# CPJKU/beat_this

Hardware: AMD Instinct MI355X
Metric: audio-seconds processed/sec (higher is better)
Workload: dtype f32 activations, f16x3 products (3 x f16 MFMA on hi+lo operand halves, f32 accumulate); main-layer attention P.V: 2 x, probabilities as fp16 hi parts

## Files before the change

### beat_this_amd/csrc/attn2.hip

```cpp
#include <cstdlib>

#include "common.h"
#include "kernels.h"

namespace {

constexpr int KB = 4;
constexpr int BLK_BYTES = 2048;
constexpr int TILE_BYTES = KB * BLK_BYTES;
constexpr int SMEM_BYTES = 2 * 2 * TILE_BYTES + 16;

typedef const __attribute__((address_space(1))) void* gptr_t;
typedef __attribute__((address_space(3))) void* lptr_t;

DEVI int lane_id_fresh() {
  int z;
  asm volatile("s_mov_b32 %0, 0" : "=s"(z));
  return __builtin_amdgcn_mbcnt_hi(~0u, __builtin_amdgcn_mbcnt_lo(~0u, z));
}
DEVI unsigned pk2(float a, float b) {
  const hfx2 t = {(hf)a, (hf)b};
  return __builtin_bit_cast(unsigned, t);
}
DEVI void zero16(f32x16& a) {
// ... 613 lines not shown
    const float scale = okq ? gatev / l_tot[j] : 0.f;
#pragma unroll
    for (int k = 0; k < 2; ++k) {
      const unsigned x0 = pk2(st[j].acc[8 * k] * scale, st[j].acc[8 * k + 1] * scale);
      const unsigned x1 = pk2(st[j].acc[8 * k + 2] * scale, st[j].acc[8 * k + 3] * scale);
      const unsigned y0 = pk2(st[j].acc[8 * k + 4] * scale, st[j].acc[8 * k + 5] * scale);
      const unsigned y1 = pk2(st[j].acc[8 * k + 6] * scale, st[j].acc[8 * k + 7] * scale);
      auto r0 = __builtin_amdgcn_permlane32_swap(x0, y0, false, false);
      auto r1 = __builtin_amdgcn_permlane32_swap(x1, y1, false, false);
      if (okq) *reinterpret_cast<u32x4*>(op + 16 * k) = u32x4{r0[0], r1[0], r0[1], r1[1]};
    }
  }
}
#endif


constexpr int BLKX_BYTES = 2 * BLK_BYTES;
constexpr float P_SHIFT_X = 3.f;

struct QStateX {
  hfx8 q0, q1, q0l, q1l;
  f32x16 acc;
  float l;
  f32x4 l4;
  float m;
  f32x16 negm;
};
struct KFragX { hfx8 k0, k1, k0l, k1l; };
struct VFragX { hfx8 v0, v1, v0l, v1l; };
DEVI KFragX ld_kx(const char* kb, int g, int lr) {
  KFragX f;
  f.k0 = *reinterpret_cast<const hfx8*>(kb + ((2 * g) * 32 + lr) * 16);
  f.k1 = *reinterpret_cast<const hfx8*>(kb + ((2 * g + 1) * 32 + lr) * 16);
  f.k0l = *reinterpret_cast<const hfx8*>(kb + BLK_BYTES + ((2 * g) * 32 + lr) * 16);
  f.k1l = *reinterpret_cast<const hfx8*>(kb + BLK_BYTES + ((2 * g + 1) * 32 + lr) * 16);
  return f;
}
DEVI VFragX ld_vx(const char* vb, int lane) {
  VFragX f;
  f.v0 = *reinterpret_cast<const hfx8*>(vb + lane * 16);
  f.v1 = *reinterpret_cast<const hfx8*>(vb + 1024 + lane * 16);
  f.v0l = *reinterpret_cast<const hfx8*>(vb + BLK_BYTES + lane * 16);
  f.v1l = *reinterpret_cast<const hfx8*>(vb + BLK_BYTES + 1024 + lane * 16);
  return f;
}
DEVI void split8(const f32x16& p, int s, u32x4& whi, u32x4& wlo) {
  unsigned h[4], l[4];
#pragma unroll
  for (int j = 0; j < 4; j += 2)
    split_hl4(p[8 * s + 2 * j], p[8 * s + 2 * j + 1], p[8 * s + 2 * j + 2], p[8 * s + 2 * j + 3], h[j], l[j], h[j + 1], l[j + 1]);
  whi = u32x4{h[0], h[1], h[2], h[3]};
  wlo = u32x4{l[0], l[1], l[2], l[3]};
}
template <bool INIT, int QB>
DEVI void score_x(const KFragX& kf, const QStateX (&st)[QB], f32x16 (&sc)[QB]) {
#pragma unroll
  for (int j = 0; j < QB; ++j) {
    if constexpr (INIT) sc[j] = st[j].negm; else zero16(sc[j]);
    sc[j] = MFMA32_H(kf.k0l, st[j].q0, sc[j]);
  }
#pragma unroll
  for (int j = 0; j < QB; ++j) sc[j] = MFMA32_H(kf.k1l, st[j].q1, sc[j]);
#pragma unroll
  for (int j = 0; j < QB; ++j) sc[j] = MFMA32_H(kf.k0, st[j].q0l, sc[j]);
#pragma unroll
  for (int j = 0; j < QB; ++j) sc[j] = MFMA32_H(kf.k1, st[j].q1l, sc[j]);
#pragma unroll
  for (int j = 0; j < QB; ++j) sc[j] = MFMA32_H(kf.k0, st[j].q0, sc[j]);
#pragma unroll
  for (int j = 0; j < QB; ++j) sc[j] = MFMA32_H(kf.k1, st[j].q1, sc[j]);
}
DEVI unsigned cvt_pk_rn(float a, float b) {
  unsigned w;
  asm("s_nop 0\n\tv_cvt_pk_f16_f32 %0, %1, %2" : "=v"(w) : "v"(a), "v"(b));
  return w;
}
template <bool SAFE, bool MASK, int QB, bool PRESUB = (QB == 1), bool P16 = false>
DEVI void finish_x(f32x16 (&sc)[QB], const VFragX& vf, int g, QStateX (&st)[QB], int key0, int L) {
#pragma unroll
  for (int j = 0; j < QB; ++j) {
    if constexpr (SAFE) {
      if constexpr (MASK) {
#pragma unroll
        for (int r = 0; r < 16; ++r)
          if (key0 + crow(r, g) >= L) sc[j][r] = -1e30f;
      }
      float bm = sc[j][0];
#pragma unroll
      for (int r = 1; r < 16; ++r) bm = fmaxf(bm, sc[j][r]);
      bm = fmaxf(bm, __shfl_xor(bm, 32));
      const float m_new = fmaxf(st[j].m, bm);
      const float alpha = __builtin_amdgcn_exp2f(st[j].m - m_new);
      st[j].m = m_new;
      st[j].l *= alpha;
      if constexpr (P16) st[j].l4 *= alpha;
#pragma unroll
      for (int r = 0; r < 16; ++r) st[j].acc[r] *= alpha;
#pragma unroll
      for (int r = 0; r < 16; ++r) sc[j][r] = __builtin_amdgcn_exp2f(sc[j][r] - m_new);
    } else {
#pragma unroll
      for (int r = 0; r < 16; ++r) sc[j][r] = __builtin_amdgcn_exp2f(PRESUB ? sc[j][r] : sc[j][r] + st[j].negm[0]);
      if constexpr (MASK) {
#pragma unroll
        for (int r = 0; r < 16; ++r)
          if (key0 + crow(r, g) >= L) sc[j][r] = 0.f;
      }
    }
    if constexpr (!P16) {
      const float a = (sc[j][0] + sc[j][1]) + (sc[j][2] + sc[j][3]), b = (sc[j][4] + sc[j][5]) + (sc[j][6] + sc[j][7]);
      const float c = (sc[j][8] + sc[j][9]) + (sc[j][10] + sc[j][11]), d = (sc[j][12] + sc[j][13]) + (sc[j][14] + sc[j][15]);
      st[j].l += (a + b) + (c + d);
    }
  }
  if constexpr (P16) {
    u32x4 w0[QB], w1[QB];
#pragma unroll
    for (int j = 0; j < QB; ++j) {
#pragma unroll
      for (int i = 0; i < 4; ++i) {
        w0[j][i] = cvt_pk_rn(sc[j][2 * i], sc[j][2 * i + 1]);
        w1[j][i] = cvt_pk_rn(sc[j][8 + 2 * i], sc[j][8 + 2 * i + 1]);
      }
      rowsum8(st[j].l4, w0[j]);
      rowsum8(st[j].l4, w1[j]);
    }
#pragma unroll
    for (int j = 0; j < QB; ++j) st[j].acc = MFMA32_H(vf.v0l, __builtin_bit_cast(hfx8, w0[j]), st[j].acc);
#pragma unroll
    for (int j = 0; j < QB; ++j) st[j].acc = MFMA32_H(vf.v1l, __builtin_bit_cast(hfx8, w1[j]), st[j].acc);
#pragma unroll
    for (int j = 0; j < QB; ++j) st[j].acc = MFMA32_H(vf.v0, __builtin_bit_cast(hfx8, w0[j]), st[j].acc);
#pragma unroll
    for (int j = 0; j < QB; ++j) st[j].acc = MFMA32_H(vf.v1, __builtin_bit_cast(hfx8, w1[j]), st[j].acc);
    return;
  }
  u32x4 h0[QB], l0[QB], h1[QB], l1[QB];
#pragma unroll
  for (int j = 0; j < QB; ++j) {
    split8(sc[j], 0, h0[j], l0[j]);
    split8(sc[j], 1, h1[j], l1[j]);
  }
#pragma unroll
  for (int j = 0; j < QB; ++j) st[j].acc = MFMA32_H(vf.v0l, __builtin_bit_cast(hfx8, h0[j]), st[j].acc);
#pragma unroll
  for (int j = 0; j < QB; ++j) st[j].acc = MFMA32_H(vf.v1l, __builtin_bit_cast(hfx8, h1[j]), st[j].acc);
#pragma unroll
  for (int j = 0; j < QB; ++j) st[j].acc = MFMA32_H(vf.v0, __builtin_bit_cast(hfx8, l0[j]), st[j].acc);
#pragma unroll
  for (int j = 0; j < QB; ++j) st[j].acc = MFMA32_H(vf.v1, __builtin_bit_cast(hfx8, l1[j]), st[j].acc);
#pragma unroll
  for (int j = 0; j < QB; ++j) st[j].acc = MFMA32_H(vf.v0, __builtin_bit_cast(hfx8, h0[j]), st[j].acc);
#pragma unroll
  for (int j = 0; j < QB; ++j) st[j].acc = MFMA32_H(vf.v1, __builtin_bit_cast(hfx8, h1[j]), st[j].acc);
}

template <int KBX>
DEVI void stage_tile_x(rsrc_t rk, rsrc_t rv, int tile, char* smem, int buf, int tid, int wave) {
  constexpr int TILEX_BYTES = KBX * BLKX_BYTES;
  char* kd = smem + buf * 2 * TILEX_BYTES + wave * 1024;
  char* vd = kd + TILEX_BYTES;
  const int so = tile * TILEX_BYTES;
  static_assert(TILEX_BYTES % 4096 == 0, "stage_tile_x copies 4 KB pieces");
#pragma unroll
  for (int i = 0; i < KBX; ++i) __builtin_amdgcn_raw_ptr_buffer_load_lds(rk, (lptr_t)(kd + i * 4096), 16, tid * 16, so + i * 4096, 0, 0);
#pragma unroll
  for (int i = 0; i < KBX; ++i) __builtin_amdgcn_raw_ptr_buffer_load_lds(rv, (lptr_t)(vd + i * 4096), 16, tid * 16, so + i * 4096, 0, 0);
}

template <bool SAFE, int QB, int KBX, bool P16 = false>
DEVI void attn_tiles_x(rsrc_t rk, rsrc_t rv, char* smem, int tid, int wave, int lane, int g, int lr, QStateX (&st)[QB], int L,
                       int nblk, int t0, bool next_staged) {
  constexpr int TILEX_BYTES = KBX * BLKX_BYTES;
  const int ntiles = (nblk + KBX - 1) / KBX;
  const bool partial = (L & 31) != 0;
  for (int t = t0; t < ntiles; ++t) {
    if (t + 1 < ntiles && !(t == t0 && next_staged)) stage_tile_x<KBX>(rk, rv, t + 1, smem, (t + 1) & 1, tid, wave);
    const char* kb = smem + (t & 1) * 2 * TILEX_BYTES;
    const char* vb = kb + TILEX_BYTES;
    const int nb = min(KBX, nblk - t * KBX);
    for (int c = 0; c < nb; ++c) {
      const int blk = t * KBX + c;
      const KFragX kf = ld_kx(kb + c * BLKX_BYTES, g, lr);
      const VFragX vf = ld_vx(vb + c * BLKX_BYTES, lane);
      f32x16 sc[QB];
      score_x<!SAFE && QB == 1, QB>(kf, st, sc);
      if (partial && blk == nblk - 1) finish_x<SAFE, true, QB, (QB == 1), P16>(sc, vf, g, st, blk * 32, L);
      else finish_x<SAFE, false, QB, (QB == 1), P16>(sc, vf, g, st, blk * 32, L);
    }
    __syncthreads();
  }
}

template <int QB>
DEVI void diag_max_x(const char* kseq, const int (&qblk)[QB], int g, int lr, const QStateX (&st)[QB], int L, float (&dmax)[QB]) {
  KFragX kd[QB];
#pragma unroll
  for (int j = 0; j < QB; ++j) kd[j] = ld_kx(kseq + (long)qblk[j] * BLKX_BYTES, g, lr);
  asm volatile("s_waitcnt vmcnt(0)" ::: "memory");
  __builtin_amdgcn_sched_barrier(0);
#pragma unroll
  for (int j = 0; j < QB; ++j) {
    f32x16 sd;
    zero16(sd);
    sd = MFMA32_H(kd[j].k0l, st[j].q0, sd);
    sd = MFMA32_H(kd[j].k1l, st[j].q1, sd);
    sd = MFMA32_H(kd[j].k0, st[j].q0l, sd);
    sd = MFMA32_H(kd[j].k1, st[j].q1l, sd);
    sd = MFMA32_H(kd[j].k0, st[j].q0, sd);
    sd = MFMA32_H(kd[j].k1, st[j].q1, sd);
    float m = -1e30f;
#pragma unroll
    for (int r = 0; r < 16; ++r) m = fmaxf(m, (32 * qblk[j] + crow(r, g) < L) ? sd[r] : -1e30f);
    dmax[j] = m;
  }
}
template <int QB>
DEVI void ref_max_x(const char* smem, int g, int lr, QStateX (&st)[QB], int L, int nblk, const float (&dmax)[QB]) {
  float bm[QB];
#pragma unroll
  for (int j = 0; j < QB; ++j) bm[j] = dmax[j];
  const int nref = min(2, nblk);
  for (int c = 0; c < nref; ++c) {
    const KFragX kf = ld_kx(smem + c * BLKX_BYTES, g, lr);
    f32x16 s0[QB];
    score_x<false, QB>(kf, st, s0);
#pragma unroll
    for (int j = 0; j < QB; ++j)
#pragma unroll
      for (int r = 0; r < 16; ++r) bm[j] = fmaxf(bm[j], (32 * c + crow(r, g) < L) ? s0[j][r] : -1e30f);
  }
#pragma unroll
  for (int j = 0; j < QB; ++j) {
    const float m = ceilf(fmaxf(bm[j], __shfl_xor(bm[j], 32)));
#pragma unroll
    for (int r = 0; r < 16; ++r) st[j].negm[r] = -m - P_SHIFT_X;
  }
}

template <int QB, int KBX, bool P16 = false>
DEVI void attn_fast_x(rsrc_t rk, rsrc_t rv, char* smem, int tid, int wave, int lane, int g, int lr, QStateX (&st)[QB], int L,
                      int nblk, const float (&dmax)[QB]) {
  constexpr int TILEX_BYTES = KBX * BLKX_BYTES;
  static_assert(KBX % 2 == 0, "two score buffers alternate over the blocks of a tile");
  const int ntiles = (nblk + KBX - 1) / KBX;
  const bool partial = (L & 31) != 0;
  int nfull = nblk / KBX;
  if (partial && nfull * KBX == nblk) --nfull;
  stage_tile_x<KBX>(rk, rv, 0, smem, 0, tid, wave);
  __syncthreads();
  if (ntiles > 1) stage_tile_x<KBX>(rk, rv, 1, smem, 1, tid, wave);
#pragma unroll
  for (int j = 0; j < QB; ++j) {
    zero16(st[j].acc);
    st[j].l = 0.f;
    st[j].l4 = f32x4{0.f, 0.f, 0.f, 0.f};
    st[j].m = -1e30f;
  }
  constexpr bool PIPE = QB == 1;
  f32x16 s2[PIPE ? 2 : 1][QB];
  ref_max_x<QB>(smem, g, lr, st, L, nblk, dmax);
  KFragX kf = ld_kx(smem, g, lr);
  if (QB == 1 && nfull > 0) score_x<true, QB>(kf, st, s2[0]);
  else if (QB != 1) score_x<false, QB>(kf, st, s2[0]);
  for (int t = 0; t < nfull; ++t) {
    const char* kb = smem + (t & 1) * 2 * TILEX_BYTES;
    const char* vb = kb + TILEX_BYTES;
    const char* kb_next = smem + ((t + 1) & 1) * 2 * TILEX_BYTES;
#pragma unroll
    for (int c = 0; c < KBX; ++c) {
      const VFragX vf = ld_vx(vb + c * BLKX_BYTES, lane);
      const int cur = PIPE ? (c & 1) : 0, nxt = PIPE ? ((c + 1) & 1) : 0;
      bool have_next = true;
      if (c + 1 < KBX) {
        kf = ld_kx(kb + (c + 1) * BLKX_BYTES, g, lr);
      } else {
        __syncthreads();
        if (t + 2 < ntiles) stage_tile_x<KBX>(rk, rv, t + 2, smem, t & 1, tid, wave);
        have_next = t + 1 < nfull;
        if (have_next) kf = ld_kx(kb_next, g, lr);
      }
      if (PIPE && have_next) score_x<true, QB>(kf, st, s2[nxt]);
      finish_x<false, false, QB, (QB == 1), P16>(s2[cur], vf, g, st, 0, L);
      if (!PIPE && have_next) score_x<false, QB>(kf, st, s2[0]);
    }
  }
// ... 90 lines not shown
  const unsigned seq_bytes = (unsigned)p.nbp * BLKX_BYTES;
  const rsrc_t rk = __builtin_amdgcn_make_buffer_rsrc(const_cast<char*>(kseq), 0, seq_bytes, 0x00020000);
  const rsrc_t rv = __builtin_amdgcn_make_buffer_rsrc(const_cast<char*>(vseq), 0, seq_bytes, 0x00020000);
  float dmax[QB];
  diag_max_x<QB>(kseq, qbi, g, lr, st, L, dmax);
  attn_fast_x<QB, KBX, P16>(rk, rv, smem, tid, wave, lane, g, lr, st, L, nblk, dmax);
  auto lane_sum = [&](int j) { return P16 ? st[j].l4[0] : st[j].l; };
  float l_tot[QB];
  bool bad[QB];
#pragma unroll
  for (int j = 0; j < QB; ++j) {
    l_tot[j] = lane_sum(j) + __shfl_xor(lane_sum(j), 32);
    const bool valid = qb0 + j < nblk && (qb0 + j) * 32 + lr < L;
    bad[j] = valid && !(l_tot[j] < 65504.f);
    const unsigned long long bw = __ballot(bad[j]);
    if (lane == 0 && qb0 + j < nblk) p.fix_mask[(long)sh * p.nbp + qb0 + j] = (int)(unsigned)bw;
  }
#ifdef BT_DEV
  if (p.status && tid == 0) atomicAdd(p.status + 2, 1);
#endif

  float amax = 0.f;
#pragma unroll
  for (int j = 0; j < QB; ++j) {
    const int qi = (qb0 + j) * 32 + lr;
    store_rows_x<OUT>(p, st[j], l_tot[j], qi, qb0 + j < nblk && qi < L && !bad[j], sh, g, amax);
  }
  if (OUT == 0 && p.status && __any(!(amax <= (p.out_f32 == 2 ? HL8_ACT_MAX : 65504.f))) && lane == 0) atomicOr(p.status, 1);
}


#include "attn_x3_loop.inc"

template <int OUT, bool P16>
__global__ __launch_bounds__(256, 2) void attn_frag_x3q2_kernel(const AttnFragP p, int nqt, int sh_total) {
  constexpr int QB = 2, KBX = ATTN_X3Q2_KBX, NBUF = ATTN_X3Q2_NBUF;
  constexpr int TILEX_BYTES = KBX * BLKX_BYTES, BUF_BYTES = 2 * TILEX_BYTES;
  static_assert(KBX == 2 && NBUF == 4 && BUF_BYTES == 16384, "the generated loop is written for four 16 KB ring buffers");
  __shared__ __attribute__((aligned(16))) char smem[NBUF * BUF_BYTES + 16];
  const int bid = blockIdx.x;
  const int idx = bid >> 3;
  const int sh = (idx / nqt) * 8 + (bid & 7);
  const int qt = idx % nqt;
  if (sh >= sh_total) return;
  const int tid = threadIdx.x, lane = tid & 63, wave = __builtin_amdgcn_readfirstlane(tid >> 6);
  const int g = lane >> 5, lr = lane & 31;
  const int L = p.L;
  const int nblk = (L + 31) >> 5;
  const long seq_off = (long)sh * p.nbp * BLKX_BYTES;
  const char* kseq = reinterpret_cast<const char*>(p.k) + seq_off;
  const char* vseq = reinterpret_cast<const char*>(p.v) + seq_off;
  QStateX st[QB];
  const int qb0 = (qt * 4 + wave) * QB;
  auto load_q = [&]() {
    const int ln = lane_id_fresh(), gg = ln >> 5, ll = ln & 31;
#pragma unroll
    for (int j = 0; j < QB; ++j) {
      const int qbc = min(qb0 + j, nblk - 1);
      const char* qblk = reinterpret_cast<const char*>(p.q) + seq_off + (long)qbc * BLKX_BYTES;
      st[j].q0 = *reinterpret_cast<const hfx8*>(qblk + ((2 * gg) * 32 + ll) * 16);
      st[j].q1 = *reinterpret_cast<const hfx8*>(qblk + ((2 * gg + 1) * 32 + ll) * 16);
      st[j].q0l = *reinterpret_cast<const hfx8*>(qblk + BLK_BYTES + ((2 * gg) * 32 + ll) * 16);
      st[j].q1l = *reinterpret_cast<const hfx8*>(qblk + BLK_BYTES + ((2 * gg + 1) * 32 + ll) * 16);
    }
    asm volatile("s_waitcnt vmcnt(0)" ::: "memory");
    __builtin_amdgcn_sched_barrier(0);
  };
  load_q();
  float dmax[QB];
  {
    const int qbi[QB] = {min(qb0, nblk - 1), min(qb0 + 1, nblk - 1)};
    diag_max_x<QB>(kseq, qbi, g, lr, st, L, dmax);
  }
  const unsigned seq_bytes = (unsigned)p.nbp * BLKX_BYTES;
  const rsrc_t rk = __builtin_amdgcn_make_buffer_rsrc(const_cast<char*>(kseq), 0, seq_bytes, 0x00020000);
  const rsrc_t rv = __builtin_amdgcn_make_buffer_rsrc(const_cast<char*>(vseq), 0, seq_bytes, 0x00020000);
  const int ntiles = (nblk + KBX - 1) / KBX;
  const bool partial = (L & 31) != 0;
  int nfull = nblk / KBX;
  if (partial && nfull * KBX == nblk) --nfull;
  nfull = __builtin_amdgcn_readfirstlane(nfull);
  auto stage_ring = [&](int tile) {
    char* kd = smem + (tile & (NBUF - 1)) * BUF_BYTES + wave * 1024;
    const int so = tile * TILEX_BYTES;
#pragma unroll
    for (int i = 0; i < KBX; ++i) __builtin_amdgcn_raw_ptr_buffer_load_lds(rk, (lptr_t)(kd + i * 4096), 16, tid * 16, so + i * 4096, 0, 0);
#pragma unroll
    for (int i = 0; i < KBX; ++i) __builtin_amdgcn_raw_ptr_buffer_load_lds(rv, (lptr_t)(kd + TILEX_BYTES + i * 4096), 16, tid * 16, so + i * 4096, 0, 0);
  };
  auto fast_pass = [&]() {
#pragma unroll
    for (int j = 0; j < QB; ++j) {
      zero16(st[j].acc);
      st[j].l = 0.f;
      st[j].l4 = f32x4{0.f, 0.f, 0.f, 0.f};
    }
    const float nm0 = st[0].negm[0], nm1 = st[1].negm[0];
    if (nfull > 0) {
    const unsigned long long ka = (unsigned long long)kseq, va = (unsigned long long)vseq;
    const u32x4 dk = {(unsigned)__builtin_amdgcn_readfirstlane((int)(unsigned)ka), (unsigned)__builtin_amdgcn_readfirstlane((int)(unsigned)((ka >> 32) & 0xffffu)),
                      (unsigned)__builtin_amdgcn_readfirstlane((int)seq_bytes), 0x00020000u};
    const u32x4 dv = {(unsigned)__builtin_amdgcn_readfirstlane((int)(unsigned)va), (unsigned)__builtin_amdgcn_readfirstlane((int)(unsigned)((va >> 32) & 0xffffu)),
                      (unsigned)__builtin_amdgcn_readfirstlane((int)seq_bytes), 0x00020000u};
    const int ln = lane_id_fresh();
    const unsigned lds0 = (unsigned)(unsigned long long)(lptr_t)smem;
    const unsigned klane = lds0 + ((2 * (ln >> 5)) * 32 + (ln & 31)) * 16, vlane = lds0 + ln * 16, dmaoff = (wave * 64 + ln) * 16;
    const unsigned m0base = (unsigned)__builtin_amdgcn_readfirstlane((int)(lds0 + wave * 1024));
    const float m1 = -1.0f;
    int t = 0, soff = 3 * TILEX_BYTES;
    if constexpr (P16)
      asm volatile(ATTN_X3Q2P_ASM
                   : "+v"(st[0].acc), "+v"(st[1].acc), "+v"(st[0].l4), "+v"(st[1].l4), "+s"(t), "+s"(soff)
                   : "v"(st[0].q0), "v"(st[0].q1), "v"(st[0].q0l), "v"(st[0].q1l), "v"(st[1].q0), "v"(st[1].q1), "v"(st[1].q0l), "v"(st[1].q1l),
                     "v"(st[0].negm), "v"(st[1].negm), "v"(klane), "v"(vlane), "v"(dmaoff), "s"(dk), "s"(dv), "s"(m0base), "s"(m1), "s"(nfull)
                   : ATTN_X3Q2P_CLOBBERS);
    else
      asm volatile(ATTN_X3Q2_ASM
                   : "+v"(st[0].acc), "+v"(st[1].acc), "+v"(st[0].l), "+v"(st[1].l), "+s"(t), "+s"(soff)
                   : "v"(st[0].q0), "v"(st[0].q1), "v"(st[0].q0l), "v"(st[0].q1l), "v"(st[1].q0), "v"(st[1].q1), "v"(st[1].q0l), "v"(st[1].q1l),
                     "v"(st[0].negm), "v"(st[1].negm), "v"(klane), "v"(vlane), "v"(dmaoff), "s"(dk), "s"(dv), "s"(m0base), "s"(m1), "s"(nfull)
                   : ATTN_X3Q2_CLOBBERS);
    }
    asm volatile("s_waitcnt vmcnt(0)" ::: "memory");
    __syncthreads();
    if (nfull < ntiles) {
      load_q();
#pragma unroll
      for (int r = 0; r < 16; ++r) {
        st[0].negm[r] = nm0;
        st[1].negm[r] = nm1;
      }
      const int lane2 = lane_id_fresh(), g2 = lane2 >> 5, lr2 = lane2 & 31;
      const char* kb = smem + (nfull & (NBUF - 1)) * BUF_BYTES;
      const char* vb = kb + TILEX_BYTES;
      const int nb = nblk - nfull * KBX;
      for (int c = 0; c < nb; ++c) {
        const int blk = nfull * KBX + c;
        const KFragX kf = ld_kx(kb + c * BLKX_BYTES, g2, lr2);
        const VFragX vf = ld_vx(vb + c * BLKX_BYTES, lane2);
        f32x16 sc[QB];
        score_x<true, QB>(kf, st, sc);
        if (partial && blk == nblk - 1) finish_x<false, true, QB, true, P16>(sc, vf, g2, st, blk * 32, L);
        else finish_x<false, false, QB, true, P16>(sc, vf, g2, st, blk * 32, L);
      }
      __syncthreads();
    }
  };
  stage_ring(0);
  stage_ring(1);
  stage_ring(2);
  asm volatile("s_waitcnt vmcnt(8)" ::: "memory");
  __syncthreads();
  ref_max_x<QB>(smem, g, lr, st, L, nblk, dmax);
  fast_pass();
  auto lane_sum = [&](int j) { return P16 ? st[j].l4[0] : st[j].l; };
  const int laneE = lane_id_fresh(), gE = laneE >> 5, lrE = laneE & 31;
  float l_tot[QB];
  bool bad[QB];
#pragma unroll
  for (int j = 0; j < QB; ++j) {
    l_tot[j] = lane_sum(j) + __shfl_xor(lane_sum(j), 32);
    const bool valid = qb0 + j < nblk && (qb0 + j) * 32 + lrE < L;
    bad[j] = valid && !(l_tot[j] < 65504.f);
    const unsigned long long bw = __ballot(bad[j]);
    if (laneE == 0 && qb0 + j < nblk) p.fix_mask[(long)sh * p.nbp + qb0 + j] = (int)(unsigned)bw;
  }
#ifdef BT_DEV
  if (p.status && tid == 0) atomicAdd(p.status + 2, 1);
#endif

  const int seq = sh / p.heads, head = sh - seq * p.heads;
  float amax = 0.f;
#pragma unroll
  for (int j = 0; j < QB; ++j) {
    const int qi = (qb0 + j) * 32 + lrE;
    const bool okq = qb0 + j < nblk && qi < L && !bad[j];
    const float gatev = okq ? p.gates[(long)sh * p.nbp * 32 + qi] : 0.f;
    const long orow = okq ? (long)(seq / p.o_div) * p.o_outer + (long)(seq % p.o_div) * p.o_inner + (long)qi * p.o_tok : 0;
    const float scale = okq ? gatev / l_tot[j] : 0.f;
    if constexpr (OUT == 1) {
      float* op = reinterpret_cast<float*>(p.out) + orow * p.inner + head * 32 + 4 * gE;
      if (okq) {
#pragma unroll
        for (int a = 0; a < 4; ++a)
          *reinterpret_cast<f32x4*>(op + 8 * a) = f32x4{st[j].acc[4 * a] * scale, st[j].acc[4 * a + 1] * scale,
                                                         st[j].acc[4 * a + 2] * scale, st[j].acc[4 * a + 3] * scale};
      }
    } else {
      hf* op = reinterpret_cast<hf*>(p.out) + orow * 2 * p.inner + head * 64 + 8 * gE;
#pragma unroll
      for (int k = 0; k < 2; ++k) {
        unsigned xh[2], xl[2], yh[2], yl[2];
#pragma unroll
        for (int i = 0; i < 2; ++i) {
          const float a0 = st[j].acc[8 * k + 2 * i] * scale, a1 = st[j].acc[8 * k + 2 * i + 1] * scale;
          const float b0 = st[j].acc[8 * k + 4 + 2 * i] * scale, b1 = st[j].acc[8 * k + 4 + 2 * i + 1] * scale;
          split_hl4(a0, a1, b0, b1, xh[i], xl[i], yh[i], yl[i]);
          amax = fmaxf(amax, fmaxf(fmaxf(fabsf(a0), fabsf(a1)), fmaxf(fabsf(b0), fabsf(b1))));
        }
        auto h0 = __builtin_amdgcn_permlane32_swap(xh[0], yh[0], false, false);
        auto h1 = __builtin_amdgcn_permlane32_swap(xh[1], yh[1], false, false);
        if (p.out_f32 == 2) {
          const float s0 = st[j].acc[8 * k] * scale, s1 = st[j].acc[8 * k + 1] * scale, s2 = st[j].acc[8 * k + 2] * scale, s3 = st[j].acc[8 * k + 3] * scale;
          const float t0 = st[j].acc[8 * k + 4] * scale, t1 = st[j].acc[8 * k + 5] * scale, t2 = st[j].acc[8 * k + 6] * scale, t3 = st[j].acc[8 * k + 7] * scale;
          auto b8 = __builtin_amdgcn_permlane32_swap(pk4_f8(s0, s1, s2, s3), pk4_f8(t0, t1, t2, t3), false, false);
          auto c8 = __builtin_amdgcn_permlane32_swap(lo4_f8(s0, s1, s2, s3, xh[0], xh[1]), lo4_f8(t0, t1, t2, t3, yh[0], yh[1]), false, false);
          if (okq) {
            *reinterpret_cast<u32x4*>(op + 16 * k) = u32x4{h0[0], h1[0], h0[1], h1[1]};
            char* gb = reinterpret_cast<char*>(op) - 16 * gE;
            *reinterpret_cast<u32x2*>(gb + 64 + 16 * k + 8 * gE) = u32x2{b8[0], b8[1]};
            *reinterpret_cast<u32x2*>(gb + 96 + 16 * k + 8 * gE) = u32x2{c8[0], c8[1]};
          }
        } else {
        auto l0 = __builtin_amdgcn_permlane32_swap(xl[0], yl[0], false, false);
        auto l1 = __builtin_amdgcn_permlane32_swap(xl[1], yl[1], false, false);
        if (okq) {
          *reinterpret_cast<u32x4*>(op + 16 * k) = u32x4{h0[0], h1[0], h0[1], h1[1]};
          *reinterpret_cast<u32x4*>(op + 32 + 16 * k) = u32x4{l0[0], l1[0], l0[1], l1[1]};
        }
        }
      }
    }
  }
  if (OUT == 0 && p.status && __any(!(amax <= (p.out_f32 == 2 ? HL8_ACT_MAX : 65504.f))) && laneE == 0) atomicOr(p.status, 1);
}


// ... 241 lines not shown
```

### beat_this_amd/csrc/attn_x3_loop.inc

```
#ifndef BT_X3Q2_ABL
#define BT_X3Q2_ABL 0
#endif
#if BT_X3Q2_ABL == 0
#define ATTN_X3Q2_ASM \
  "s_nop 4\n\t" \
  "s_and_b32 s88, %4, 3\n\t" \
  "s_lshl_b32 s88, s88, 14\n\t" \
  "v_add_u32_e32 v121, s88, %16\n\t" \
  "ds_read_b128 v[176:179], v121 offset:0\n\t" \
  "ds_read_b128 v[180:183], v121 offset:512\n\t" \
  "ds_read_b128 v[184:187], v121 offset:2048\n\t" \
  "ds_read_b128 v[188:191], v121 offset:2560\n\t" \
  "v_add_u32_e32 v122, s88, %17\n\t" \
  "ds_read_b128 v[144:147], v122 offset:8192\n\t" \
  "ds_read_b128 v[148:151], v122 offset:9216\n\t" \
  "ds_read_b128 v[152:155], v122 offset:10240\n\t" \
  "ds_read_b128 v[156:159], v122 offset:11264\n\t" \
  "ds_read_b128 v[128:131], v122 offset:8192\n\t" \
  "ds_read_b128 v[132:135], v122 offset:9216\n\t" \
  "ds_read_b128 v[136:139], v122 offset:10240\n\t" \
  "ds_read_b128 v[140:143], v122 offset:11264\n\t" \
  "v_mov_b32_e32 v200, 0\n\t" \
  "v_mov_b32_e32 v192, 0\n\t" \
  "v_mov_b32_e32 v201, 0\n\t" \
// ... 2656 lines not shown
  "ds_read_b128 v[148:151], v124 offset:9216\n\t" \
  "v_exp_f32_e32 v232, v232\n\t" \
  "v_exp_f32_e32 v233, v233\n\t" \
  "v_exp_f32_e32 v234, v234\n\t" \
  "v_exp_f32_e32 v235, v235\n\t" \
  "ds_read_b128 v[152:155], v124 offset:10240\n\t" \
  "v_mfma_f32_32x32x16_f16 %0, v[140:143], v[220:223], %0\n\t" \
  "v_exp_f32_e32 v236, v236\n\t" \
  "v_exp_f32_e32 v237, v237\n\t" \
  "v_exp_f32_e32 v238, v238\n\t" \
  "v_exp_f32_e32 v239, v239\n\t" \
  "ds_read_b128 v[156:159], v124 offset:11264\n\t" \
  "v_mfma_f32_4x4x4_16b_f16 %2, v[126:127], v[218:219], %2\n\t" \
  "v_mfma_f32_32x32x16_f16 v[240:255], v[176:179], %8, v[240:255]\n\t" \
  "v_mfma_f32_32x32x16_f16 v[240:255], v[180:183], %9, v[240:255]\n\t" \
  "v_cvt_pk_f16_f32 v200, v224, v225\n\t" \
  "v_cvt_pk_f16_f32 v201, v226, v227\n\t" \
  "v_cvt_pk_f16_f32 v202, v228, v229\n\t" \
  "v_cvt_pk_f16_f32 v203, v230, v231\n\t" \
  "v_mfma_f32_32x32x16_f16 %0, v[128:131], v[216:219], %0\n\t" \
  "v_cvt_pk_f16_f32 v204, v232, v233\n\t" \
  "v_cvt_pk_f16_f32 v205, v234, v235\n\t" \
  "v_mfma_f32_4x4x4_16b_f16 %2, v[126:127], v[220:221], %2\n\t" \
  "v_mfma_f32_32x32x16_f16 v[240:255], v[176:179], %6, v[240:255]\n\t" \
  "v_mfma_f32_32x32x16_f16 v[240:255], v[180:183], %7, v[240:255]\n\t" \
  "v_cvt_pk_f16_f32 v206, v236, v237\n\t" \
  "v_cvt_pk_f16_f32 v207, v238, v239\n\t" \
  "v_mfma_f32_32x32x16_f16 %0, v[132:135], v[220:223], %0\n\t" \
  "v_mfma_f32_4x4x4_16b_f16 %2, v[126:127], v[222:223], %2\n\t" \
  "s_add_u32 %5, %5, 8192\n\t" \
  "s_add_u32 %4, %4, 1\n\t" \
  "s_cmp_lt_i32 %4, %23\n\t" \
  "s_cbranch_scc1 Lloop%=\n\t" \
  "v_mfma_f32_32x32x16_f16 %1, v[136:139], v[200:203], %1\n\t" \
  "v_mfma_f32_4x4x4_16b_f16 %3, v[126:127], v[200:201], %3\n\t" \
  "s_nop 7\n\t" \
  "s_nop 3\n\t" \
  "v_mfma_f32_32x32x16_f16 %1, v[140:143], v[204:207], %1\n\t" \
  "v_mfma_f32_4x4x4_16b_f16 %3, v[126:127], v[202:203], %3\n\t" \
  "s_nop 7\n\t" \
  "s_nop 3\n\t" \
  "v_mfma_f32_32x32x16_f16 %1, v[128:131], v[200:203], %1\n\t" \
  "v_mfma_f32_4x4x4_16b_f16 %3, v[126:127], v[204:205], %3\n\t" \
  "s_nop 7\n\t" \
  "s_nop 3\n\t" \
  "v_mfma_f32_32x32x16_f16 %1, v[132:135], v[204:207], %1\n\t" \
  "v_mfma_f32_4x4x4_16b_f16 %3, v[126:127], v[206:207], %3\n\t" \
  "s_nop 7\n\t" \
  "s_nop 3\n\t" \
  "s_waitcnt lgkmcnt(0)\n\t" \
  "s_nop 7\n\t" \
  "s_nop 7\n\t" \
  ""
#define ATTN_X3Q2_CLOBBERS "v116", "v117", "v118", "v119", "v120", "v121", "v122", "v123", "v124", "v128", "v129", "v130", "v131", "v132", "v133", "v134", "v135", "v136", "v137", "v138", "v139", "v140", "v141", "v142", "v143", "v144", "v145", "v146", "v147", "v148", "v149", "v150", "v151", "v152", "v153", "v154", "v155", "v156", "v157", "v158", "v159", "v160", "v161", "v162", "v163", "v164", "v165", "v166", "v167", "v168", "v169", "v170", "v171", "v172", "v173", "v174", "v175", "v176", "v177", "v178", "v179", "v180", "v181", "v182", "v183", "v184", "v185", "v186", "v187", "v188", "v189", "v190", "v191", "v192", "v193", "v194", "v195", "v196", "v197", "v198", "v199", "v200", "v201", "v202", "v203", "v204", "v205", "v206", "v207", "v208", "v209", "v210", "v211", "v212", "v213", "v214", "v215", "v216", "v217", "v218", "v219", "v220", "v221", "v222", "v223", "v224", "v225", "v226", "v227", "v228", "v229", "v230", "v231", "v232", "v233", "v234", "v235", "v236", "v237", "v238", "v239", "v240", "v241", "v242", "v243", "v244", "v245", "v246", "v247", "v248", "v249", "v250", "v251", "v252", "v253", "v254", "v255", "s88", "s89", "s90", "s91", "s92", "s93", "s94", "s95", "scc", "memory"
#define ATTN_X3Q2P_CLOBBERS "v121", "v122", "v123", "v124", "v126", "v127", "v128", "v129", "v130", "v131", "v132", "v133", "v134", "v135", "v136", "v137", "v138", "v139", "v140", "v141", "v142", "v143", "v144", "v145", "v146", "v147", "v148", "v149", "v150", "v151", "v152", "v153", "v154", "v155", "v156", "v157", "v158", "v159", "v160", "v161", "v162", "v163", "v164", "v165", "v166", "v167", "v168", "v169", "v170", "v171", "v172", "v173", "v174", "v175", "v176", "v177", "v178", "v179", "v180", "v181", "v182", "v183", "v184", "v185", "v186", "v187", "v188", "v189", "v190", "v191", "v200", "v201", "v202", "v203", "v204", "v205", "v206", "v207", "v216", "v217", "v218", "v219", "v220", "v221", "v222", "v223", "v224", "v225", "v226", "v227", "v228", "v229", "v230", "v231", "v232", "v233", "v234", "v235", "v236", "v237", "v238", "v239", "v240", "v241", "v242", "v243", "v244", "v245", "v246", "v247", "v248", "v249", "v250", "v251", "v252", "v253", "v254", "v255", "s88", "s89", "s90", "s91", "s92", "s93", "s94", "s95", "scc", "memory"
#define ATTN_X3Q2_KBX 2
#define ATTN_X3Q2_NBUF 4
```

### beat_this_amd/csrc/engine.hip

```cpp
#include <algorithm>
#include <cmath>
#include <cstddef>
#include <cstdio>
#include <cstring>
#include <mutex>
#include <string>
#include <vector>

#include "../../include/beat_this_amd.h"
#include "common.h"
#include "kernels.h"


static thread_local std::string g_err;
static int bt_set_error(int code, const std::string& msg) {
  g_err = msg;
  return code;
}
int bt_set_error_external(int code, const char* msg) { return bt_set_error(code, msg); }

namespace prof {
struct Rec { int cat; hipEvent_t a, b; };
struct State { bool on = false; std::vector<Rec> recs; };
struct Scope {
// ... 111 lines not shown
  g.W = x3 ? d.conv_w_x3[blk] : d.conv_w[blk][BT_PREC_HALF];
  g.epi = G3_RESID; g.no_resid = 1; g.gelu = 1; g.bias = d.conv_b[blk]; g.ldx = 2 * C;
  g.conv_C2 = 2 * C; g.conv_T = T; g.conv_F = F / 2; g.x3 = x3; g.status = ws.status;
  g.x = out_half ? nullptr : out; g.xb = out_half ? (void*)out : nullptr;
  return g;
}

GemmP linear_params(const bt_model_desc& d, int wp, const float* in, float* out, void* xb, float* ssq_out, int B, int T) {
  GemmP g;
  memset(&g, 0, sizeof g);
  g.A = in; g.lda = 1024; g.W = d.lin_w[wp]; g.M = B * T; g.N = d.transformer_dim; g.K = 1024;
  g.epi = GEMM_EPI_STORE; g.flags = GEMM_F_A_F32 | GEMM_F_BIAS | GEMM_F_OUT_F32;
  g.bias = d.lin_b; g.out = out; g.ldo = d.transformer_dim; g.xb = xb; g.ssq_out = ssq_out;
  return g;
}

Gemm3P linear3_params(const bt_model_desc& d, const Workspace& ws, int B, int T, bool x3, bool out_f8) {
  const int D = d.transformer_dim;
  Gemm3P g;
  memset(&g, 0, sizeof g);
  g.A = front_x(ws, 3); g.lda = 1024; g.M = B * T; g.K = 1024; g.W = x3 ? d.lin_w_x3 : d.lin_w[BT_PREC_HALF]; g.N = D;
  g.epi = G3_RESID; g.no_resid = 1; g.bias = d.lin_b; g.x = ws.xm; g.ldx = D; g.xb = ws.xmb; g.ssq_out = ws.ssq[0];
  g.x3 = x3 ? 1 | (out_f8 ? G3_X3_OUT_F8 : 0) : 0; g.status = ws.status;
  return g;
}

HeadP head_params(const bt_model_desc& d, const float* x, const float* w, int prenorm, float* beat, float* downbeat, int M,
                  int* status) {
  HeadP p;
  p.x = x; p.w = w; p.b0 = d.head_b[0]; p.b1 = d.head_b[1];
  p.beat = beat; p.downbeat = downbeat; p.M = M; p.D = d.transformer_dim; p.sum_head = d.sum_head; p.prenorm = prenorm;
  p.status = status;
  return p;
}

template <class P>
void attn_rows(P& a, int B, int T, int F) {
  a.n_seq = B * F; a.L = T; a.o_div = F; a.o_outer = (long)T * F; a.o_inner = F > 1 ? 1 : 0; a.o_tok = F;
}

struct PairRoute {
  bool ff_fused;
  bool outff;
  bool split;
  bool time_frag;
};

struct FragLayer {
  bool qkv8;
  bool out8;
  bool ff8;
  bool next8;
  bool tail;
};

enum { LAYERS_GENERIC, LAYERS_FRAG_HALF, LAYERS_FRAG_X3 };

struct Route {
  bool x3;
  int fp;
  int gp, wp;
  int x3_attn, x3_attn_front;
  bool half_shadow;
  int layers;
  struct Block { PairRoute freq, time; bool conv3; } blk[3];
  bool lin3, lin_f8;
  struct Layer { PairRoute pair; FragLayer frag; } layer[BT_MAX_LAYERS];
};

Route plan_route(const bt_engine& e, int B, int T, int prec, int first, const Workspace& ws) {
  const bt_model_desc& d = e.d;
  const int D = d.transformer_dim;
  Route r;
  r.x3 = prec == BT_PREC_F32X3;
  r.fp = r.x3 ? BT_PREC_F32 : prec;
  r.gp = prec;
  r.wp = r.x3 ? BT_PREC_HALF : prec;
  r.x3_attn = r.x3 ? 4 | ((e.x3_attn_p16 == 1 || e.x3_attn_p16 == 2) ? BT_X3_P16 : 0) : 0;
  r.x3_attn_front = r.x3 ? 4 | (e.x3_attn_p16 >= 2 ? BT_X3_P16 : 0) : 0;
  auto pair = [&](const bt_pair_weights& w) {
    PairRoute p;
    p.ff_fused = w.dim <= 128 && w.w_ff_frag[r.fp];
    p.outff = p.ff_fused && w.w_outff_frag[r.fp] && w.w_attnff_frag[r.fp];
    p.split = r.x3 && w.w_outff_frag_x3 && w.w_attnff_frag_x3;
    p.time_frag = r.x3 ? p.outff && p.split && w.w_qkv_frag_x3 : p.ff_fused && r.fp == BT_PREC_HALF && w.w_qkv_frag;
    return p;
  };

  r.half_shadow = prec == BT_PREC_HALF && D >= 128 && D % 64 == 0;
  const long wide = (long)B * T * d.ff_mult * D;
  bool frag_x3 = r.x3 && D >= 128 && D % 128 == 0 && wide * 4 < 0x7fffffffL;
  for (int l = 0; frag_x3 && l < d.n_layers; ++l)
    frag_x3 = d.layers[l].w_qkvg_x3 && d.layers[l].w_out_x3 && d.layers[l].w_ff1_x3 && d.layers[l].w_ff2_x3;
  const bool frag_half = r.half_shadow && D % 128 == 0 && wide * 2 < 0x7fffffffL;
  r.layers = frag_x3 ? LAYERS_FRAG_X3 : frag_half ? LAYERS_FRAG_HALF : LAYERS_GENERIC;

  const bool lin3_fits = (frag_half || (frag_x3 && d.lin_w_x3)) && gemm3_supported(linear3_params(d, ws, B, T, frag_x3, false));
  for (int blk = 0; blk < 3; ++blk) {
    Route::Block& rb = r.blk[blk];
    rb.freq = pair(d.front[blk][0]);
    rb.time = pair(d.front[blk][1]);
    const Gemm3P cg = conv3_params(d, ws, blk, B, T, frag_x3, blk == 2 && lin3_fits);
    rb.conv3 = d.partial_transformers && rb.time.outff && (frag_x3 ? rb.time.split : frag_half) && cg.N >= 128 && cg.W &&
               gemm3_supported(cg);
  }
  r.lin3 = lin3_fits && (!frag_x3 || r.blk[2].conv3);
  r.lin_f8 = r.lin3 && frag_x3 && e.x3_gemm_fp8 >= 2 && d.n_layers > 0 && d.layers[0].w_qkvg_f8;

  for (int l = 0; l < d.n_layers; ++l) {
    const bt_pair_weights& w = d.layers[l];
    FragLayer& f = r.layer[l].frag;
    r.layer[l].pair = pair(w);
    f.qkv8 = l == 0 ? first == 0 && r.lin_f8 : r.layer[l - 1].frag.next8;
    f.out8 = frag_x3 && e.x3_gemm_fp8 >= 2 && w.w_out_f8;
    f.ff8 = frag_x3 && e.x3_gemm_fp8 >= 1 && w.w_ff1_f8 && w.w_ff2_f8;
    f.next8 = frag_x3 && e.x3_gemm_fp8 >= 2 && l + 1 < d.n_layers && d.layers[l + 1].w_qkvg_f8 && w.w_ff2_f8;
    f.tail = frag_half && w.w_tail_frag && layer_tail_supported(D, d.ff_mult * D);
  }
  return r;
}

#define CHECK_RC(what)                                                         \
  if (_rc != 0) {                                                              \
    char buf[160];                                                             \
    snprintf(buf, sizeof buf, "%s failed (code %d: %s)", what, _rc,            \
             _rc > 0 ? hipGetErrorString((hipError_t)_rc) : "bad arguments");  \
    return bt_set_error(_rc > 0 ? BT_ERR_HIP : BT_ERR_ARG, buf);               \
  }
#define LAUNCH(expr, what) \
  do { int _rc = (expr); CHECK_RC(what) } while (0)
#define LAUNCH_CAT(cat, st, expr, what) \
  do { int _rc; { prof::Scope _ps(pf, cat, st); _rc = (expr); } CHECK_RC(what) } while (0)


int check_rows(long M) {
  return M > 0x7fffffffL ? bt_set_error(BT_ERR_ARG, "batch too large for one forward call") : BT_OK;
}

int out_proj(prof::State* pf, const bt_pair_weights& pw, const Route& r, float* x, void* xs, const Workspace& ws, long M,
             hipStream_t s) {
  const int C = pw.dim;
  GemmP g;
  memset(&g, 0, sizeof g);
  g.A = ws.ao; g.lda = C; g.W = pw.w_out[r.wp]; g.M = (int)M; g.N = C; g.K = C;
  g.epi = GEMM_EPI_RESID; g.flags = 0; g.x = x; g.ldx = C; g.xb = xs;
  LAUNCH_CAT(CAT_OUT, s, launch_gemm(g, r.gp, s), "out-proj gemm");
  return BT_OK;
}

int qkv_attn(prof::State* pf, const bt_pair_weights& pw, const Route& r, const float* rope, float* x, void* xs,
             const Workspace& ws, int B, int T, int F, hipStream_t s) {
  const int C = pw.dim, H = pw.heads;
  GemmP g;
  memset(&g, 0, sizeof g);
  g.A = xs ? xs : (const void*)x; g.lda = C; g.W = pw.w_qkvg[r.wp]; g.M = B * T * F; g.N = 3 * C + H; g.K = C;
  g.epi = GEMM_EPI_QKV; g.flags = GEMM_F_RMS | (xs ? 0 : GEMM_F_A_F32) | (F > 1 ? GEMM_F_ROWMAP : 0);
  g.bias = pw.b_gates; g.out = ws.qkv; g.ldo = 3 * C; g.gates = ws.gates; g.inner = C; g.heads = H;
  g.rope = rope; g.map_T = T; g.map_F = F; g.pdiv = F; g.pmod = T;
  LAUNCH_CAT(CAT_QKV, s, launch_gemm(g, r.gp, s), "qkv gemm");
  AttnP a;
  memset(&a, 0, sizeof a);
  a.qkv = ws.qkv; a.ld = 3 * C; a.gates = ws.gates; a.out = ws.ao; a.heads = H; a.inner = C;
  attn_rows(a, B, T, F);
  LAUNCH_CAT(CAT_ATTN_FLASH, s, launch_attn_flash(a, r.gp, s), F > 1 ? "time attention" : "attention");
  return BT_OK;
}

int ff_half(prof::State* pf, const bt_pair_weights& pw, const PairRoute& pr, const Route& r, float* x, void* xs,
            const Workspace& ws, long M, int ff_mult, hipStream_t s) {
  const int C = pw.dim, HID = ff_mult * C;
  if (pr.ff_fused) {
    FusedFFP ff;
    ff.x = x; ff.M = M; ff.C = C; ff.wfrag = pw.w_ff_frag[r.fp]; ff.b1 = pw.b_ff1; ff.b2 = pw.b_ff2; ff.xb = xs;
    LAUNCH_CAT(CAT_FF_FUSED, s, launch_ff_fused(ff, r.fp, s), "fused feed-forward");
    return BT_OK;
  }
  GemmP g;
  memset(&g, 0, sizeof g);
  g.A = xs ? xs : (const void*)x; g.lda = C; g.W = pw.w_ff1[r.wp]; g.M = (int)M; g.N = HID; g.K = C;
  g.epi = GEMM_EPI_STORE; g.flags = GEMM_F_RMS | (xs ? 0 : GEMM_F_A_F32) | GEMM_F_BIAS | GEMM_F_GELU;
  g.bias = pw.b_ff1; g.out = ws.hid; g.ldo = HID;
  LAUNCH_CAT(CAT_FF1, s, launch_gemm(g, r.gp, s), "ff1 gemm");
  memset(&g, 0, sizeof g);
  g.A = ws.hid; g.lda = HID; g.W = pw.w_ff2[r.wp]; g.M = (int)M; g.N = C; g.K = HID;
  g.epi = GEMM_EPI_RESID; g.flags = GEMM_F_BIAS; g.bias = pw.b_ff2; g.x = x; g.ldx = C; g.xb = xs;
  LAUNCH_CAT(CAT_FF2, s, launch_gemm(g, r.gp, s), "ff2 gemm");
  return BT_OK;
}

int generic_layer(prof::State* pf, const bt_pair_weights& pw, const PairRoute& pr, const Route& r, const float* rope, float* x,
                  void* xs, const Workspace& ws, int B, int T, int ff_mult, bool attn, bool ff, hipStream_t s) {
  const long M = (long)B * T;
  if (int rc = check_rows(M)) return rc;
  if (attn) {
    if (int rc = qkv_attn(pf, pw, r, rope, x, xs, ws, B, T, 1, s)) return rc;
    if (int rc = out_proj(pf, pw, r, x, xs, ws, M, s)) return rc;
  }
  return ff ? ff_half(pf, pw, pr, r, x, xs, ws, M, ff_mult, s) : BT_OK;
}

int freq_half(prof::State* pf, const bt_pair_weights& pw, const PairRoute& pr, const Route& r, const float* rope, float* x,
              int B, int T, int F, hipStream_t s) {
  const long M = (long)B * T * F;
  if (int rc = check_rows(M)) return rc;
  if (!pr.outff) return bt_set_error(BT_ERR_ARG, "frequency-direction half needs bt_pair_weights.w_attnff_frag");
  FusedAttnFFP f;
  f.x = x; f.M = M; f.C = pw.dim; f.b_gates = pw.b_gates; f.rope = rope;
  f.wfrag = pr.split ? pw.w_attnff_frag_x3 : pw.w_attnff_frag[r.fp]; f.b1 = pw.b_ff1; f.b2 = pw.b_ff2;
  LAUNCH_CAT(CAT_ATTN_FREQ_FUSED, s, launch_attnff_fused(f, pr.split ? BT_PREC_F32X3 : r.fp, s),
             "fused frequency attention + feed-forward");
  return BT_OK;
}

int time_half(prof::State* pf, const bt_pair_weights& pw, const PairRoute& pr, const Route& r, const float* rope, float* x,
              const Workspace& ws, int B, int T, int F, void* shadow, hipStream_t s) {
  const long M = (long)B * T * F;
  if (int rc = check_rows(M)) return rc;
  if (pr.time_frag) {
    QkvFrontP qp;
    memset(&qp, 0, sizeof qp);
    qp.x = x; qp.B = B; qp.T = T; qp.F = F; qp.C = pw.dim; qp.wfrag = r.x3 ? pw.w_qkv_frag_x3 : pw.w_qkv_frag;
    qp.b_gates = pw.b_gates; qp.rope = rope;
    qp.q = ws.qf; qp.k = ws.kf; qp.v = ws.vf; qp.gates = ws.gates_h; qp.nbp = ws.nbp;
    qp.x3 = r.x3; qp.status = ws.status;
    LAUNCH_CAT(CAT_QKV, s, launch_qkv_front(qp, s), "frontend qkv projection");
    AttnFragP a;
    memset(&a, 0, sizeof a);
    a.q = ws.qf; a.k = ws.kf; a.v = ws.vf; a.gates = ws.gates_h; a.out = ws.ao; a.heads = pw.heads; a.inner = pw.dim;
    a.nbp = ws.nbp; attn_rows(a, B, T, F);
    a.x3 = r.x3_attn_front; a.out_f32 = 1; a.status = ws.status; a.fix_mask = ws.fix_mask;
    LAUNCH_CAT(CAT_ATTN_FLASH, s, launch_attn_frag(a, s), "time attention");
  } else if (int rc = qkv_attn(pf, pw, r, rope, x, nullptr, ws, B, T, F, s)) {
    return rc;
  }
  if (pr.outff) {
    FusedOutFFP f;
    f.x = x; f.M = M; f.C = pw.dim; f.ao = ws.ao; f.wfrag = pr.split ? pw.w_outff_frag_x3 : pw.w_outff_frag[r.fp];
    f.b1 = pw.b_ff1; f.b2 = pw.b_ff2; f.xb = shadow; f.abl = 0;
    LAUNCH_CAT(CAT_FF_FUSED, s, launch_outff_fused(f, pr.split ? BT_PREC_F32X3 : r.fp, s), "fused out-projection + feed-forward");
    return BT_OK;
  }
  if (int rc = out_proj(pf, pw, r, x, nullptr, ws, M, s)) return rc;
  return ff_half(pf, pw, pr, r, x, nullptr, ws, M, 4, s);
}

int frag_layer(prof::State* pf, const bt_pair_weights& pw, const FragLayer& f, const Route& r, const float* rope,
               const Workspace& ws, int B, int T, int ff_mult, hipStream_t s) {
  const int D = pw.dim, H = pw.heads, HID = ff_mult * D;
  const int M = B * T;
  const int parts = D / 64;
  int* status = r.x3 ? ws.status : nullptr;
  auto w = [&](const void* const* half, const void* hl32, const void* hl8, bool f8) { return !r.x3 ? half[BT_PREC_HALF] : f8 ? hl8 : hl32; };
  Gemm3P g;
  memset(&g, 0, sizeof g);
  g.A = ws.xmb; g.lda = D; g.M = M; g.K = D; g.W = w(pw.w_qkvg, pw.w_qkvg_x3, pw.w_qkvg_f8, f.qkv8); g.N = 3 * D + H; g.epi = G3_QKV;
  g.ssq_in = ws.ssq[0]; g.ssq_parts = parts; g.x3 = r.x3 | (f.qkv8 ? G3_X3_F8 : 0); g.status = status;
  g.n_seq = B; g.L = T; g.nblk = (T + 31) / 32; g.nbp = ws.nbp; g.heads = H; g.inner = D; g.rope = rope;
  g.qf = ws.qf; g.kf = ws.kf; g.vf = ws.vf; g.gates = ws.gates_h; g.b_gates = pw.b_gates;
  LAUNCH_CAT(CAT_QKV, s, launch_gemm3(g, s), r.x3 ? "qkv gemm (hi + lo)" : "qkv gemm");
  AttnFragP a;
  memset(&a, 0, sizeof a);
  a.q = ws.qf; a.k = ws.kf; a.v = ws.vf; a.gates = ws.gates_h; a.out = ws.ao; a.heads = H; a.inner = D; a.nbp = ws.nbp;
  attn_rows(a, B, T, 1);
  a.x3 = r.x3_attn; a.out_f32 = f.out8 ? 2 : 0; a.status = status; a.fix_mask = ws.fix_mask;
  LAUNCH_CAT(CAT_ATTN_FLASH, s, launch_attn_frag(a, s), r.x3 ? "attention (hi + lo)" : "attention");
  if (f.tail) {
    LayerTailP t;
    t.x = ws.xm; t.M = M; t.C = D; t.hidden = HID; t.ao = ws.ao; t.wfrag = pw.w_tail_frag; t.b1 = pw.b_ff1; t.b2 = pw.b_ff2;
    t.xb = ws.xmb; t.ssq_out = ws.ssq[0];
    LAUNCH_CAT(CAT_LAYER_TAIL, s, launch_layer_tail(t, s), "layer tail (out-projection + feed-forward)");
    return BT_OK;
  }
  memset(&g, 0, sizeof g);
  g.A = ws.ao; g.lda = D; g.M = M; g.K = D; g.W = w(pw.w_out, pw.w_out_x3, pw.w_out_f8, f.out8); g.N = D; g.epi = G3_RESID;
  g.x3 = r.x3 | (f.out8 ? G3_X3_F8 : 0) | (f.ff8 ? G3_X3_OUT_F8 : 0); g.status = status;
  g.x = ws.xm; g.ldx = D; g.xb = ws.xmb; g.ssq_out = ws.ssq[1];
  LAUNCH_CAT(CAT_OUT, s, launch_gemm3(g, s), r.x3 ? "out-proj gemm (hi + lo)" : "out-proj gemm");
  memset(&g, 0, sizeof g);
  g.A = ws.xmb; g.lda = D; g.M = M; g.K = D; g.W = w(pw.w_ff1, pw.w_ff1_x3, pw.w_ff1_f8, f.ff8); g.N = HID; g.epi = G3_FF1;
  g.x3 = r.x3 | (f.ff8 ? G3_X3_F8 | G3_X3_OUT_F8 : 0); g.status = status;
  g.bias = pw.b_ff1; g.ssq_in = ws.ssq[1]; g.ssq_parts = parts; g.out = ws.hid; g.ldo = HID;
  LAUNCH_CAT(CAT_FF1, s, launch_gemm3(g, s), r.x3 ? "ff1 gemm (hi + lo)" : "ff1 gemm");
  memset(&g, 0, sizeof g);
  g.A = ws.hid; g.lda = HID; g.M = M; g.K = HID; g.W = w(pw.w_ff2, pw.w_ff2_x3, pw.w_ff2_f8, f.ff8); g.N = D; g.epi = G3_RESID;
  g.x3 = r.x3 | (f.ff8 ? G3_X3_F8 : 0) | (f.next8 ? G3_X3_OUT_F8 : 0); g.status = status;
  g.bias = pw.b_ff2; g.x = ws.xm; g.ldx = D; g.xb = ws.xmb; g.ssq_out = ws.ssq[0];
  LAUNCH_CAT(CAT_FF2, s, launch_gemm3(g, s), r.x3 ? "ff2 gemm (hi + lo)" : "ff2 gemm");
  return BT_OK;
}

int frontend(prof::State* pf, const bt_model_desc& d, const Route& r, const float* spect, const Workspace& ws, int B, int T,
             hipStream_t s) {
  const StemP sp = stem_params(d, spect, front_x(ws, 0), B, T);
  LAUNCH_CAT(CAT_STEM, s, launch_stem(sp, s), "stem");
  for (int blk = 0; blk < 3; ++blk) {
    const Route::Block& rb = r.blk[blk];
    float* x = front_x(ws, blk);
    if (d.partial_transformers) {
      if (int rc = freq_half(pf, d.front[blk][0], rb.freq, r, d.rope, x, B, T, 32 >> blk, s)) return rc;
      if (int rc = time_half(pf, d.front[blk][1], rb.time, r, d.rope, x, ws, B, T, 32 >> blk, rb.conv3 ? ws.hid : nullptr, s))
        return rc;
    }
    if (rb.conv3) {
      const Gemm3P g = conv3_params(d, ws, blk, B, T, r.layers == LAYERS_FRAG_X3, blk == 2 && r.lin3);
      LAUNCH_CAT(CAT_CONV, s, launch_gemm3(g, s), "frontend conv gemm");
    } else {
      const GemmP g = conv_params(d, blk, r.wp, x, front_x(ws, blk + 1), B, T, !(blk == 2 && r.lin3));
      LAUNCH_CAT(CAT_CONV, s, launch_gemm(g, r.gp, s), "frontend conv gemm");
    }
  }
  if (r.lin3) {
    const Gemm3P g = linear3_params(d, ws, B, T, r.layers == LAYERS_FRAG_X3, r.lin_f8);
    LAUNCH_CAT(CAT_LINEAR, s, launch_gemm3(g, s), "frontend linear gemm");
    return BT_OK;
  }
  const GemmP g = linear_params(d, r.wp, front_x(ws, 3), ws.xm, r.half_shadow ? ws.xmb : nullptr,
                                r.layers == LAYERS_FRAG_HALF ? ws.ssq[0] : nullptr, B, T);
  LAUNCH_CAT(CAT_LINEAR, s, launch_gemm(g, r.gp, s), "frontend linear gemm");
  if (r.layers == LAYERS_FRAG_X3)
    LAUNCH_CAT(CAT_LINEAR, s, launch_shadow_ssq(ws.xm, ws.xmb, ws.ssq[0], (long)B * T, d.transformer_dim, s, 1), "hl32 shadow of the residual stream");
  return BT_OK;
}

}

extern "C" {

const char* bt_last_error(void) { return g_err.c_str(); }
int bt_version(void) { return BT_ABI_VERSION; }
int bt_half_is_bf16(void) { return BT_HALF_IS_BF16; }
void bt_struct_sizes(int32_t* out) {
  out[0] = (int32_t)sizeof(bt_pair_weights); out[1] = (int32_t)sizeof(bt_model_desc);
  out[2] = (int32_t)sizeof(bt_logmel_tables); out[3] = (int32_t)sizeof(bt_gemm_args);
  out[4] = (int32_t)sizeof(bt_attn_args); out[5] = (int32_t)offsetof(bt_model_desc, layers);
  out[6] = (int32_t)offsetof(bt_model_desc, rope);
  out[7] = (int32_t)sizeof(bt_attn_frag_args);
  out[8] = (int32_t)sizeof(bt_gemm3_args);
}

int bt_engine_create(const bt_model_desc* desc, bt_engine** out) {
  if (!desc || !out) return bt_set_error(BT_ERR_ARG, "null argument");
  if (desc->transformer_dim % 32 || desc->transformer_dim < 32 || desc->transformer_dim > 1024 ||
      desc->n_layers < 0 || desc->n_layers > BT_MAX_LAYERS || desc->ff_mult < 1 || desc->ff_mult > 16)
    return bt_set_error(BT_ERR_ARG, "unsupported transformer_dim / n_layers / ff_mult");
  bt_engine* e = new bt_engine;
  e->d = *desc;
  *out = e;
  return BT_OK;
}
static void drop_graphs(bt_engine* e) {
  for (auto& g : e->graphs) (void)hipGraphExecDestroy(g.exec);
  e->graphs.clear();
  e->warm.clear();
// ... 8 lines not shown

int bt_engine_set_option(bt_engine* e, int option, int value) {
  if (!e) return bt_set_error(BT_ERR_ARG, "null argument");
  std::lock_guard<std::mutex> lock(e->mu);
  if (option == BT_OPT_X3_ATTN_P16 && value >= 0 && value <= 3) { if (e->x3_attn_p16 != value) drop_graphs(e); e->x3_attn_p16 = value; return BT_OK; }
  if (option == BT_OPT_X3_GEMM_FP8 && value >= 0 && value <= 2) { if (e->x3_gemm_fp8 != value) drop_graphs(e); e->x3_gemm_fp8 = value; return BT_OK; }
  if (option == BT_OPT_WS_GUARD && value >= 0 && value % 256 == 0) { if (e->ws_guard != value) drop_graphs(e); e->ws_guard = value; return BT_OK; }
  return bt_set_error(BT_ERR_ARG, "unknown engine option / value");
}
int bt_engine_get_option(const bt_engine* e, int option, int* value) {
  if (!e || !value) return bt_set_error(BT_ERR_ARG, "null argument");
  if (option == BT_OPT_X3_ATTN_P16) { *value = e->x3_attn_p16; return BT_OK; }
  if (option == BT_OPT_X3_GEMM_FP8) { *value = e->x3_gemm_fp8; return BT_OK; }
  if (option == BT_OPT_WS_GUARD) { *value = e->ws_guard; return BT_OK; }
  return bt_set_error(BT_ERR_ARG, "unknown engine option");
}

size_t bt_workspace_bytes(const bt_engine* e, int B, int T, int prec) {
  if (!e || B <= 0 || T <= 0) return 0;
  return carve(nullptr, B, T, e->d.transformer_dim, e->d.ff_mult, prec, (size_t)e->ws_guard).total;
}

int bt_workspace_regions(const bt_engine* e, int B, int T, int prec, int64_t* begin_end, int max) {
  if (!e || B <= 0 || T <= 0 || max < 0 || (max > 0 && !begin_end)) return bt_set_error(BT_ERR_ARG, "bad argument to bt_workspace_regions");
  if (prec != BT_PREC_F32 && prec != BT_PREC_HALF && prec != BT_PREC_F32X3) return bt_set_error(BT_ERR_ARG, "unknown precision");
  std::vector<int64_t> r;
  carve(nullptr, B, T, e->d.transformer_dim, e->d.ff_mult, prec, (size_t)e->ws_guard, &r);
  const int n = (int)(r.size() / 2);
  for (int i = 0; i < std::min(n, max); ++i) { begin_end[2 * i] = r[2 * i]; begin_end[2 * i + 1] = r[2 * i + 1]; }
  return n;
}

int bt_forward(bt_engine* e, void* stream, int prec, const float* d_spect, int B, int T, void* d_ws, size_t ws_bytes,
               float* d_beat, float* d_downbeat) {
  return bt_forward_stages(e, stream, prec, 0, 2, d_spect, B, T, d_ws, ws_bytes, nullptr, d_beat, d_downbeat);
}

int bt_forward_stages(bt_engine* e, void* stream, int prec, int first, int last, const float* d_spect, int B, int T, void* d_ws,
                      size_t ws_bytes, float* d_out, float* d_beat, float* d_downbeat) {
  if (!e || !d_spect || !d_ws) return bt_set_error(BT_ERR_ARG, "null argument");
  if (first < 0 || last > 2 || first > last) return bt_set_error(BT_ERR_ARG, "stages: need 0 <= first <= last <= 2");
  if (last == 2 ? (!d_beat || !d_downbeat) : !d_out) return bt_set_error(BT_ERR_ARG, "null output");
  const int max_T = e->d.rope_len > 0 ? e->d.rope_len : 1536;
  if (B <= 0 || T <= 0 || T > max_T)
    return bt_set_error(BT_ERR_ARG, "need B >= 1 and 1 <= T <= " + std::to_string(max_T) + " (bt_model_desc.rope_len: rows of the rotary table)");
  if (prec != BT_PREC_F32 && prec != BT_PREC_HALF && prec != BT_PREC_F32X3)
    return bt_set_error(BT_ERR_ARG, "unknown precision");
  const bt_model_desc& d = e->d;
  prof::State* pf = &e->prof;
  const int D = d.transformer_dim;
  const Workspace ws = carve((char*)d_ws, B, T, D, d.ff_mult, prec, (size_t)e->ws_guard);
  if (ws.total > ws_bytes) return bt_set_error(BT_ERR_WORKSPACE, "workspace too small");
  if (prec == BT_PREC_F32X3 && BT_HALF_IS_BF16) return bt_set_error(BT_ERR_ARG, "BT_PREC_F32X3 needs an IEEE fp16 build");
  const Route r = plan_route(*e, B, T, prec, first, ws);
  hipStream_t s = (hipStream_t)stream;
  if (r.x3) LAUNCH(launch_clear_words(ws.status, 1, s), "clearing the range flag");
  int* status = r.x3 ? ws.status : nullptr;

  const size_t xm_bytes = (size_t)B * T * D * 4;
  if (first == 2) {
    if (!d.head_w_raw) return bt_set_error(BT_ERR_ARG, "stage entry at task_heads needs head_w_raw");
    const HeadP hp = head_params(d, d_spect, d.head_w_raw, 1, d_beat, d_downbeat, B * T, nullptr);
    LAUNCH_CAT(CAT_HEAD, s, launch_head(hp, s), "head");
    return BT_OK;
  }
  if (first == 1) {
    if (hipMemcpyAsync(ws.xm, d_spect, xm_bytes, hipMemcpyDeviceToDevice, s) != hipSuccess)
      return bt_set_error(BT_ERR_HIP, "copy of the stage input");
    if (r.half_shadow)
      LAUNCH_CAT(CAT_LINEAR, s, launch_shadow_ssq(ws.xm, ws.xmb, r.layers == LAYERS_FRAG_HALF ? ws.ssq[0] : nullptr, (long)B * T, D, s), "stage entry");
    if (r.layers == LAYERS_FRAG_X3) LAUNCH_CAT(CAT_LINEAR, s, launch_shadow_ssq(ws.xm, ws.xmb, ws.ssq[0], (long)B * T, D, s, 1), "stage entry");
  }
  if (first == 0)
    if (int rc = frontend(pf, d, r, d_spect, ws, B, T, s)) return rc;
  if (last == 0) {
    if (hipMemcpyAsync(d_out, ws.xm, xm_bytes, hipMemcpyDeviceToDevice, s) != hipSuccess)
      return bt_set_error(BT_ERR_HIP, "copy of the stage output");
    if (r.x3) LAUNCH_CAT(CAT_HEAD, s, launch_finite_rows(ws.xm, (long)B * T, D, ws.status, s), "range check of the stage output");
    return BT_OK;
  }
  for (int l = 0; l < d.n_layers; ++l) {
    const Route::Layer& rl = r.layer[l];
    const int rc = r.layers == LAYERS_GENERIC
                       ? generic_layer(pf, d.layers[l], rl.pair, r, d.rope, ws.xm, r.half_shadow ? ws.xmb : nullptr, ws, B, T,
                                       d.ff_mult, true, true, s)
                       : frag_layer(pf, d.layers[l], rl.frag, r, d.rope, ws, B, T, d.ff_mult, s);
    if (rc) return rc;
  }
  if (last == 1) {
    if (!d.norm_out_g) return bt_set_error(BT_ERR_ARG, "stage exit after transformer_blocks needs norm_out_g");
    LAUNCH_CAT(CAT_HEAD, s, launch_norm_out(ws.xm, d.norm_out_g, d_out, (long)B * T, D, s, status), "final norm");
    return BT_OK;
  }
  const HeadP hp = head_params(d, ws.xm, d.head_w, 0, d_beat, d_downbeat, B * T, status);
  LAUNCH_CAT(CAT_HEAD, s, launch_head(hp, s), "head");
  return BT_OK;
}

int bt_forward_unit(bt_engine* e, void* stream, int prec, int unit, int index, const float* d_in, float* d_out, int B, int T,
                    void* d_ws, size_t ws_bytes) {
  if (!e || !d_in || !d_out || !d_ws) return bt_set_error(BT_ERR_ARG, "null argument");
  const bt_model_desc& d = e->d;
  const int max_T = d.rope_len > 0 ? d.rope_len : 1536;
  if (B <= 0 || T <= 0 || T > max_T) return bt_set_error(BT_ERR_ARG, "need B >= 1 and 1 <= T <= bt_model_desc.rope_len");
  if (prec == BT_PREC_F32X3) prec = BT_PREC_F32;
  if (prec != BT_PREC_F32 && prec != BT_PREC_HALF) return bt_set_error(BT_ERR_ARG, "unknown precision");
  prof::State* pf = &e->prof;
  const int D = d.transformer_dim;
  const Workspace ws = carve((char*)d_ws, B, T, D, d.ff_mult, prec, (size_t)e->ws_guard);
  if (ws.total > ws_bytes) return bt_set_error(BT_ERR_WORKSPACE, "workspace too small");
  const Route r = plan_route(*e, B, T, prec, 0, ws);
  hipStream_t s = (hipStream_t)stream;
  const bool block_unit = unit == BT_UNIT_PARTIAL || unit == BT_UNIT_CONV;
  const bool layer_unit = unit == BT_UNIT_ATTN || unit == BT_UNIT_FF;
  const bool leaf_unit = unit == BT_UNIT_FRONT_ATTN || unit == BT_UNIT_FRONT_FF;
  if (leaf_unit && (index < 0 || index > 5 || !d.partial_transformers)) return bt_set_error(BT_ERR_ARG, "partial-transformer leaf index out of range");
  if (block_unit && (index < 0 || index > 2)) return bt_set_error(BT_ERR_ARG, "frontend block index out of range");
  if (layer_unit && (index < 0 || index >= d.n_layers)) return bt_set_error(BT_ERR_ARG, "layer index out of range");
  auto copy_in = [&](size_t bytes) -> int {
    if (d_in != d_out && hipMemcpyAsync(d_out, d_in, bytes, hipMemcpyDeviceToDevice, s) != hipSuccess)
      return bt_set_error(BT_ERR_HIP, "copy of the unit's input");
    return BT_OK;
  };
  switch (unit) {
    case BT_UNIT_STEM: {
      const StemP sp = stem_params(d, d_in, d_out, B, T);
      LAUNCH_CAT(CAT_STEM, s, launch_stem(sp, s), "stem");
      return BT_OK;
    }
    case BT_UNIT_PARTIAL: {
      if (!d.partial_transformers) return bt_set_error(BT_ERR_ARG, "this model has no partial transformers");
      const Route::Block& rb = r.blk[index];
      if (int rc = copy_in((size_t)B * T * 1024 * 4)) return rc;
      if (int rc = freq_half(pf, d.front[index][0], rb.freq, r, d.rope, d_out, B, T, 32 >> index, s)) return rc;
      return time_half(pf, d.front[index][1], rb.time, r, d.rope, d_out, ws, B, T, 32 >> index, nullptr, s);
    }
    case BT_UNIT_CONV: {
      const GemmP g = conv_params(d, index, r.wp, d_in, d_out, B, T, true);
      LAUNCH_CAT(CAT_CONV, s, launch_gemm(g, r.gp, s), "frontend conv gemm");
      return BT_OK;
    }
    case BT_UNIT_LINEAR: {
      const GemmP g = linear_params(d, r.wp, d_in, d_out, nullptr, nullptr, B, T);
      LAUNCH_CAT(CAT_LINEAR, s, launch_gemm(g, r.gp, s), "frontend linear gemm");
      return BT_OK;
    }
    case BT_UNIT_ATTN:
    case BT_UNIT_FF: {
      if (int rc = copy_in((size_t)B * T * D * 4)) return rc;
      return generic_layer(pf, d.layers[index], r.layer[index].pair, r, d.rope, d_out, nullptr, ws, B, T, d.ff_mult,
                           unit == BT_UNIT_ATTN, unit == BT_UNIT_FF, s);
    }
    case BT_UNIT_FRONT_ATTN:
    case BT_UNIT_FRONT_FF: {
      const bt_pair_weights& pw = d.front[index >> 1][index & 1];
      const Route::Block& rb = r.blk[index >> 1];
      if (int rc = copy_in((size_t)B * T * pw.dim * 4)) return rc;
      return generic_layer(pf, pw, index & 1 ? rb.time : rb.freq, r, d.rope, d_out, nullptr, ws, B, T, 4,
                           unit == BT_UNIT_FRONT_ATTN, unit == BT_UNIT_FRONT_FF, s);
    }
    case BT_UNIT_NORM:
      if (!d.norm_out_g) return bt_set_error(BT_ERR_ARG, "bt_model_desc.norm_out_g is not set");
      LAUNCH_CAT(CAT_HEAD, s, launch_norm_out(d_in, d.norm_out_g, d_out, (long)B * T, D, s), "final norm");
      return BT_OK;
    default:
      return bt_set_error(BT_ERR_ARG, "unknown unit");
  }
}

int bt_split_chunks(void* stream, const float* d_spect, int64_t n_frames, const int32_t* d_starts, int B, int T,
                    float* d_chunks) {
  if (!d_spect || !d_starts || !d_chunks || B <= 0 || T <= 0 || n_frames <= 0)
    return bt_set_error(BT_ERR_ARG, "bad argument to bt_split_chunks");
  LAUNCH(launch_split(d_spect, n_frames, d_starts, nullptr, B, T, d_chunks, (hipStream_t)stream), "split");
  return BT_OK;
}

int bt_split_chunks_batch(void* stream, const float* d_spect, const int32_t* d_chunk_table, int B, int T, float* d_chunks) {
  if (!d_spect || !d_chunk_table || !d_chunks || B <= 0 || T <= 0)
    return bt_set_error(BT_ERR_ARG, "bad argument to bt_split_chunks_batch");
  LAUNCH(launch_split(d_spect, 0, nullptr, d_chunk_table, B, T, d_chunks, (hipStream_t)stream), "split (batch)");
  return BT_OK;
}

int bt_aggregate(void* stream, const float* cb, const float* cd, const int32_t* d_starts, int B, int T, int border,
                 int64_t n_frames, float* d_beat, float* d_downbeat) {
  if (!cb || !cd || !d_starts || !d_beat || !d_downbeat || B <= 0 || T <= 0 || n_frames <= 0 || border < 0)
    return bt_set_error(BT_ERR_ARG, "bad argument to bt_aggregate");
// ... 268 lines not shown
  for (int i = 0; i < n_categories; ++i) { ms_by_category[i] = 0.0; launches_by_category[i] = 0; }
  for (auto& r : e->prof.recs) {
    hipError_t e = hipEventSynchronize(r.b);
    float ms = 0.f;
    if (e == hipSuccess) e = hipEventElapsedTime(&ms, r.a, r.b);
    if (e != hipSuccess) return bt_set_error(BT_ERR_HIP, hipGetErrorString(e));
    ms_by_category[r.cat] += ms;
    launches_by_category[r.cat] += 1;
    (void)hipEventDestroy(r.a); (void)hipEventDestroy(r.b);
  }
  e->prof.recs.clear();
  return BT_OK;
}

int bt_ff_fused(void* stream, int prec, const bt_pair_weights* w, float* d_x, int64_t M) {
  if (!w || !d_x || M <= 0 || w->dim > 128 || !w->w_ff_frag[prec]) return bt_set_error(BT_ERR_ARG, "bad argument to bt_ff_fused");
  FusedFFP ff;
  ff.x = d_x; ff.M = M; ff.C = w->dim; ff.wfrag = w->w_ff_frag[prec]; ff.b1 = w->b_ff1; ff.b2 = w->b_ff2;
  ff.xb = nullptr;
  LAUNCH(launch_ff_fused(ff, prec, (hipStream_t)stream), "fused feed-forward");
  return BT_OK;
}

int bt_gemm(void* stream, int prec, const bt_gemm_args* a) {
  if (!a) return bt_set_error(BT_ERR_ARG, "null argument");
  GemmP g;
  memset(&g, 0, sizeof g);
  g.A = a->A; g.lda = a->lda; g.W = a->W; g.M = a->M; g.N = a->N; g.K = a->K; g.epi = a->epi; g.flags = a->flags;
  g.bias = a->bias; g.out = a->out; g.ldo = a->ldo; g.x = a->x; g.ldx = a->ldx;
  g.conv_C2 = a->conv_C2; g.conv_T = a->conv_T; g.conv_F = a->conv_F;
  g.gates = a->gates; g.inner = a->inner; g.heads = a->heads; g.rope = a->rope;
  g.pdiv = a->pdiv; g.pmod = a->pmod; g.map_T = a->map_T; g.map_F = a->map_F;
  LAUNCH(launch_gemm(g, prec, (hipStream_t)stream), "gemm");
  return BT_OK;
}

int bt_attention(void* stream, int prec, const bt_attn_args* a) {
  if (!a) return bt_set_error(BT_ERR_ARG, "null argument");
  AttnP p;
  memset(&p, 0, sizeof p);
  p.qkv = a->qkv; p.ld = a->ld; p.gates = a->gates; p.out = a->out; p.n_seq = a->n_seq; p.L = a->L;
  p.heads = a->heads; p.inner = a->inner; p.o_div = a->o_div; p.o_outer = a->o_outer; p.o_inner = a->o_inner;
  p.o_tok = a->o_tok;
  LAUNCH(launch_attn_flash(p, prec, (hipStream_t)stream), "attention (flash)");
  return BT_OK;
}

int bt_outff_fused(void* stream, int prec, const bt_pair_weights* w, const void* d_ao, float* d_x, int64_t M, void* d_xb) {
  if (prec != BT_PREC_F32 && prec != BT_PREC_HALF && prec != BT_PREC_F32X3) return bt_set_error(BT_ERR_ARG, "unknown precision");
  const void* wf = !w ? nullptr : prec == BT_PREC_F32X3 ? w->w_outff_frag_x3 : w->w_outff_frag[prec];
  if (!w || !d_ao || !d_x || M <= 0 || w->dim > 128 || !wf) return bt_set_error(BT_ERR_ARG, "bad argument to bt_outff_fused");
  FusedOutFFP f;
  f.x = d_x; f.M = M; f.C = w->dim; f.ao = d_ao; f.wfrag = wf; f.b1 = w->b_ff1; f.b2 = w->b_ff2;
  f.xb = prec == BT_PREC_F32 ? nullptr : d_xb; f.abl = 0;
  LAUNCH(launch_outff_fused(f, prec, (hipStream_t)stream), "fused out-projection + feed-forward");
  return BT_OK;
}

int bt_attnff_fused(void* stream, int prec, const bt_pair_weights* w, const float* d_rope, float* d_x, int64_t M) {
  if (prec != BT_PREC_F32 && prec != BT_PREC_HALF && prec != BT_PREC_F32X3) return bt_set_error(BT_ERR_ARG, "unknown precision");
  const void* wf = !w ? nullptr : prec == BT_PREC_F32X3 ? w->w_attnff_frag_x3 : w->w_attnff_frag[prec];
  if (!w || !d_x || !d_rope || M <= 0 || w->dim > 128 || !wf) return bt_set_error(BT_ERR_ARG, "bad argument to bt_attnff_fused");
  FusedAttnFFP f;
  f.x = d_x; f.M = M; f.C = w->dim; f.b_gates = w->b_gates; f.rope = d_rope; f.wfrag = wf;
  f.b1 = w->b_ff1; f.b2 = w->b_ff2;
  LAUNCH(launch_attnff_fused(f, prec, (hipStream_t)stream), "fused frequency attention + feed-forward");
  return BT_OK;
}

int bt_layer_tail(void* stream, const bt_pair_weights* w, int hidden, const void* d_ao, float* d_x, int64_t M, void* d_xb,
                  float* d_ssq_out) {
  if (!w || !w->w_tail_frag || !d_ao || !d_x || M <= 0 || !layer_tail_supported(w->dim, hidden))
    return bt_set_error(BT_ERR_ARG, "bad argument to bt_layer_tail");
  LayerTailP t;
  t.x = d_x; t.M = M; t.C = w->dim; t.hidden = hidden; t.ao = d_ao; t.wfrag = w->w_tail_frag; t.b1 = w->b_ff1;
  t.b2 = w->b_ff2; t.xb = d_xb; t.ssq_out = d_ssq_out;
  LAUNCH(launch_layer_tail(t, (hipStream_t)stream), "layer tail");
  return BT_OK;
}

int bt_gemm3(void* stream, const bt_gemm3_args* a) {
  if (!a || !a->A || !a->W) return bt_set_error(BT_ERR_ARG, "null argument");
  Gemm3P g;
  memset(&g, 0, sizeof g);
  g.A = a->A; g.lda = a->lda; g.M = a->M; g.K = a->K; g.W = a->W; g.N = a->N; g.epi = a->epi; g.bias = a->bias;
  g.ssq_in = a->ssq_in; g.ssq_parts = a->ssq_parts; g.out = a->out; g.ldo = a->ldo; g.x = a->x; g.ldx = a->ldx;
  g.xb = a->xb; g.ssq_out = a->ssq_out; g.n_seq = a->n_seq; g.L = a->L; g.nblk = (a->L + 31) / 32; g.nbp = a->nbp;
  g.heads = a->heads; g.inner = a->heads * 32; g.rope = a->rope; g.qf = a->qf; g.kf = a->kf; g.vf = a->vf;
  g.gates = a->gates; g.b_gates = a->b_gates;
  g.x3 = a->x3; g.status = a->status;
  g.no_resid = a->no_resid; g.gelu = a->gelu; g.conv_C2 = a->conv_C2; g.conv_T = a->conv_T; g.conv_F = a->conv_F;
  if (!gemm3_supported(g)) return bt_set_error(BT_ERR_ARG, "shape not supported by bt_gemm3");
  LAUNCH(launch_gemm3(g, (hipStream_t)stream), "gemm3");
  return BT_OK;
}

int bt_gemm_mx8(void* stream, const void* d_A, const void* d_SA, const void* d_W, const void* d_SW, float* d_out, int M, int N, int K,
                int64_t ldo) {
  GemmMx8P g;
  g.A = d_A; g.SA = d_SA; g.W = d_W; g.SW = d_SW; g.out = d_out; g.ldo = (long)ldo; g.M = M; g.N = N; g.K = K;
  if (!d_A || !d_SA || !d_W || !d_SW || !d_out || !gemm_mx8_supported(g)) return bt_set_error(BT_ERR_ARG, "bad argument to bt_gemm_mx8");
  LAUNCH(launch_gemm_mx8(g, (hipStream_t)stream), "MX e4m3 gemm");
  return BT_OK;
}

int bt_attn_frag_blocks(int L) { return L > 0 ? attn_frag_blocks(L) : 0; }

// ... 30 lines not shown
```

### beat_this_amd/csrc/fused2.hip

```cpp
#include <cstdlib>
#include <type_traits>

#include "chain.h"
#include "kernels.h"

namespace {


typedef __amdgpu_buffer_rsrc_t rsrc_t;
typedef __attribute__((address_space(3))) void* lptr_t;
DEVI unsigned pk2_hf(float a, float b) {
  const hfx2 t = {(hf)a, (hf)b};
  return __builtin_bit_cast(unsigned, t);
}

#ifdef BT_DEV
__device__ long long* g_f2_dbg = nullptr;
#define F2_DBG g_f2_dbg
#define F2_ABL(p) ((p).abl)
#else
#define F2_DBG ((long long*)nullptr)
#define F2_ABL(p) 0
#endif

template <typename T, int C>
struct WRing {
  static constexpr int KT = C / 32;
  static constexpr int TILE_B = 32 * 32 * (int)sizeof(T);
  static constexpr int STEP_B = 2 * KT * TILE_B;
#ifndef BT_F2_NST_HL128
#define BT_F2_NST_HL128 2
#endif
#ifndef BT_F2_NST_HL64
#define BT_F2_NST_HL64 2
#endif
  static constexpr bool HL = sizeof(T) == 4 && !std::is_same<T, float>::value;
  static constexpr int NST = C == 128 ? (HL ? BT_F2_NST_HL128 : 3) : (HL && C == 64 ? BT_F2_NST_HL64 : 4);
  static constexpr int CH = STEP_B / 4096;
  rsrc_t rs;
  char* lds;
  int tid, wave, total;
  long long t_wait = 0, t_bar = 0;
  bool timing = false;
  DEVI void issue(int s) {
    if (s >= total) return;
    char* dst = lds + (s % NST) * STEP_B + wave * 1024;
#pragma unroll
    for (int i = 0; i < CH; ++i)
      __builtin_amdgcn_raw_ptr_buffer_load_lds(rs, (lptr_t)(dst + i * 4096), 16, tid * 16, s * STEP_B + i * 4096, 0, 0);
  }
  DEVI void prologue() {
#pragma unroll
    for (int s = 0; s < NST - 1; ++s) issue(s);
  }
  DEVI const char* acquire(int s) {
    const int ahead = min(NST - 2, total - 1 - s);
    long long q0 = 0, q1 = 0;
    if (timing) q0 = clock64();
    if (ahead >= 2) asm volatile("s_waitcnt vmcnt(%0) lgkmcnt(0)" ::"n"(2 * CH) : "memory");
    else if (ahead == 1) asm volatile("s_waitcnt vmcnt(%0) lgkmcnt(0)" ::"n"(CH) : "memory");
    else asm volatile("s_waitcnt vmcnt(0) lgkmcnt(0)" ::: "memory");
    if (timing) q1 = clock64();
    __builtin_amdgcn_s_barrier();
    if (timing) { const long long q2 = clock64(); t_wait += q1 - q0; t_bar += q2 - q1; }
    issue(s + NST - 1);
    return lds + (s % NST) * STEP_B;
  }
};

template <typename T, int C>
DEVI void ff_tail(WRing<T, C>& ws, int step0, float (&xn)[C / 32][16], const float* b1s, const float* b2,
                  float* xrow, hf* xbrow, bool ok, int lane, int g) {
  constexpr int KT = C / 32, HB = 4 * C / 32;
  constexpr int TILE_B = WRing<T, C>::TILE_B;
  float ss = 0.f;
#pragma unroll
  for (int kt = 0; kt < KT; ++kt)
#pragma unroll
    for (int r = 0; r < 16; ++r) ss = fmaf(xn[kt][r], xn[kt][r], ss);
  ss += __shfl_xor(ss, 32);
  constexpr float PW = OpScale<T>::PW;
  const float scale = sqrtf((float)C) / fmaxf(sqrtf(ss), 1e-12f) * PW;
  Frag<T> xf[KT];
#pragma unroll
  for (int kt = 0; kt < KT; ++kt) xf[kt] = pack_frag<T>(xn[kt]);
  f32x16 acc2[KT];
#pragma unroll
  for (int mt = 0; mt < KT; ++mt)
#pragma unroll
    for (int r = 0; r < 16; ++r) acc2[mt][r] = xn[mt][r] * (1.f / PW);
#pragma unroll 1
  for (int hb = 0; hb < HB; ++hb) {
    const char* wb = ws.acquire(step0 + hb);
    f32x16 acc1;
    zero16(acc1);
#pragma unroll
    for (int kt = 0; kt < KT; ++kt) mma32(acc1, lds_frag<T>(wb + kt * TILE_B, lane), xf[kt]);
    float h[16];
#pragma unroll
    for (int a = 0; a < 4; ++a) {
      const f32x4 b = *reinterpret_cast<const f32x4*>(b1s + hb * 32 + 8 * a + 4 * g);
#pragma unroll
      for (int j = 0; j < 4; ++j) h[4 * a + j] = gelu_t<T>(fmaf(acc1[4 * a + j], scale, b[j]));
    }
    const Frag<T> hf = pack_frag<T>(h);
#pragma unroll
    for (int mt = 0; mt < KT; ++mt) mma32(acc2[mt], lds_frag<T>(wb + (KT + mt) * TILE_B, lane), hf);
  }
#pragma unroll
  for (int mt = 0; mt < KT; ++mt) {
    f32x4 v[4];
#pragma unroll
    for (int a = 0; a < 4; ++a) {
      const int f0 = mt * 32 + 8 * a + 4 * g;
      const f32x4 b = *reinterpret_cast<const f32x4*>(b2 + f0);
#pragma unroll
      for (int j = 0; j < 4; ++j) v[a][j] = fmaf(acc2[mt][4 * a + j], PW, b[j]);
      if (ok) *reinterpret_cast<f32x4*>(xrow + f0) = v[a];
    }
    if (xbrow) {
      typedef __attribute__((ext_vector_type(4))) unsigned int u32x4;
      if constexpr (std::is_same<T, hl>::value) {
#pragma unroll
        for (int k = 0; k < 2; ++k) {
          unsigned xh[2], xl[2], yh[2], yl[2];
#pragma unroll
          for (int i = 0; i < 2; ++i) {
            split_hl4(v[2 * k][2 * i], v[2 * k][2 * i + 1], v[2 * k + 1][2 * i], v[2 * k + 1][2 * i + 1], xh[i], xl[i], yh[i], yl[i]);
          }
          auto h0 = __builtin_amdgcn_permlane32_swap(xh[0], yh[0], false, false);
          auto h1 = __builtin_amdgcn_permlane32_swap(xh[1], yh[1], false, false);
          auto l0 = __builtin_amdgcn_permlane32_swap(xl[0], yl[0], false, false);
          auto l1 = __builtin_amdgcn_permlane32_swap(xl[1], yl[1], false, false);
          if (ok) {
            *reinterpret_cast<u32x4*>(xbrow + mt * 64 + 16 * k + 8 * g) = u32x4{h0[0], h1[0], h0[1], h1[1]};
            *reinterpret_cast<u32x4*>(xbrow + mt * 64 + 32 + 16 * k + 8 * g) = u32x4{l0[0], l1[0], l0[1], l1[1]};
          }
        }
      } else {
#pragma unroll
      for (int k = 0; k < 2; ++k) {
        const unsigned x0 = pk2_hf(v[2 * k][0], v[2 * k][1]), x1 = pk2_hf(v[2 * k][2], v[2 * k][3]);
        const unsigned y0 = pk2_hf(v[2 * k + 1][0], v[2 * k + 1][1]), y1 = pk2_hf(v[2 * k + 1][2], v[2 * k + 1][3]);
        auto r0 = __builtin_amdgcn_permlane32_swap(x0, y0, false, false);
        auto r1 = __builtin_amdgcn_permlane32_swap(x1, y1, false, false);
        if (ok) *reinterpret_cast<u32x4*>(xbrow + mt * 32 + 16 * k + 8 * g) = u32x4{r0[0], r1[0], r0[1], r1[1]};
      }
      }
    }
  }
}

template <typename T, int C>
__global__ __launch_bounds__(256) void outff_fused_kernel(const FusedOutFFP p) {
  constexpr int KT = C / 32, HB = 4 * C / 32;
  constexpr int TILE_B = WRing<T, C>::TILE_B, STEP_B = WRing<T, C>::STEP_B, NST = WRing<T, C>::NST;
  __shared__ __attribute__((aligned(16))) char wl[NST * STEP_B + 4 * C * 4];
  float* b1s = reinterpret_cast<float*>(wl + NST * STEP_B);
  const int tid = threadIdx.x, lane = tid & 63, wave = __builtin_amdgcn_readfirstlane(tid >> 6);
  const int g = lane >> 5, lr = lane & 31;
  const long tok = ((long)blockIdx.x * 4 + wave) * 32 + lr;
  const bool ok_st = tok < p.M && !(F2_ABL(p) & 2);
  const bool ok = tok < p.M && !(F2_ABL(p) & 1);
  float* xrow = p.x + (tok < p.M ? tok : 0) * C;
  for (int i = tid; i < 4 * C; i += 256) b1s[i] = p.b1[i];

  const T* arow = reinterpret_cast<const T*>(p.ao) + (ok ? tok : 0) * C;
  Frag<T> af[KT];
#pragma unroll
  for (int kt = 0; kt < KT; ++kt) af[kt] = ldg_frag<T>(arow + kt * 32 + 16 * g);
  float xn[KT][16];
#pragma unroll
  for (int mt = 0; mt < KT; ++mt)
#pragma unroll
    for (int a = 0; a < 4; ++a) {
      const f32x4 v = ok ? *reinterpret_cast<const f32x4*>(xrow + mt * 32 + 8 * a + 4 * g) : f32x4{0.f, 0.f, 0.f, 0.f};
#pragma unroll
      for (int j = 0; j < 4; ++j) xn[mt][4 * a + j] = v[j];
    }
  WRing<T, C> ws;
  ws.rs = __builtin_amdgcn_make_buffer_rsrc(const_cast<void*>(p.wfrag), 0, (unsigned)((KT + HB) * STEP_B), 0x00020000);
  ws.lds = wl; ws.tid = tid; ws.wave = wave; ws.total = KT + HB;
  __syncthreads();
  asm volatile("s_waitcnt vmcnt(0)" ::: "memory");
  ws.prologue();
#pragma unroll
  for (int mt = 0; mt < KT; ++mt) {
    const char* wb = ws.acquire(mt);
    f32x16 acc;
    zero16(acc);
#pragma unroll
    for (int kt = 0; kt < KT; ++kt) mma32(acc, lds_frag<T>(wb + kt * TILE_B, lane), af[kt]);
#pragma unroll
    for (int r = 0; r < 16; ++r) xn[mt][r] = fmaf(acc[r], OpScale<T>::PW, xn[mt][r]);
  }
  hf* xbrow = p.xb ? reinterpret_cast<hf*>(p.xb) + tok * C * (std::is_same<T, hl>::value ? 2 : 1) : nullptr;
  ff_tail<T, C>(ws, KT, xn, b1s, p.b2, xrow, xbrow, ok_st, lane, g);
}

template <typename T, int C>
__global__ __launch_bounds__(256) void attnff_fused_kernel(const FusedAttnFFP p) {
  constexpr int KT = C / 32;
  constexpr int H = C / 32;
  constexpr int F = 1024 / C;
  constexpr int HB = 4 * C / 32;
  constexpr int TILE_B = WRing<T, C>::TILE_B, STEP_B = WRing<T, C>::STEP_B, NST = WRing<T, C>::NST;
  __shared__ __attribute__((aligned(16))) char wl[NST * STEP_B + 4 * C * 4];
  float* b1s = reinterpret_cast<float*>(wl + NST * STEP_B);
  const int tid = threadIdx.x, lane = tid & 63, wave = __builtin_amdgcn_readfirstlane(tid >> 6);
  const int g = lane >> 5, lr = lane & 31;
  const long tok = ((long)blockIdx.x * 4 + wave) * 32 + lr;
  const bool ok = tok < p.M;
  float* xrow = p.x + (ok ? tok : 0) * C;
  long long* dbg = F2_DBG;
  const long long t_in = dbg ? clock64() : 0;
  for (int i = tid; i < 4 * C; i += 256) b1s[i] = p.b1[i];

  float ss = 0.f;
  Frag<T> xf[KT];
#pragma unroll
  for (int kt = 0; kt < KT; ++kt) xf[kt] = ldx_frag<T>(xrow + kt * 32 + 16 * g, ok, ss);
  ss += __shfl_xor(ss, 32);
  constexpr float PW = OpScale<T>::PW, PA = OpScale<T>::PA;
  const float scale = sqrtf((float)C) / fmaxf(sqrtf(ss), 1e-12f) * PW;
  float sk[16];
#pragma unroll
  for (int r = 0; r < 16; ++r) sk[r] = __shfl(scale, crow(r, g));
  const int pos = (int)(tok & (F - 1));
  f32x2 cs[8];
#pragma unroll
  for (int a = 0; a < 4; ++a)
#pragma unroll
    for (int b = 0; b < 2; ++b)
      cs[2 * a + b] = *reinterpret_cast<const f32x2*>(p.rope + ((long)pos * 16 + 4 * a + 2 * g + b) * 2);
  float bg[H];
#pragma unroll
  for (int hd = 0; hd < H; ++hd) bg[hd] = p.b_gates[hd];
  WRing<T, C> ws;
  ws.rs = __builtin_amdgcn_make_buffer_rsrc(const_cast<void*>(p.wfrag), 0, (unsigned)((1 + 2 * H + HB) * STEP_B), 0x00020000);
  ws.lds = wl; ws.tid = tid; ws.wave = wave; ws.total = 1 + 2 * H + HB;
  __syncthreads();
  asm volatile("s_waitcnt vmcnt(0)" ::: "memory");
  ws.timing = dbg != nullptr;
  const long long t_ring = dbg ? clock64() : 0;
  ws.prologue();

  float gate[H];
  {
    const char* wb = ws.acquire(0);
    f32x16 ag;
// ... 51 lines not shown
      }
      l += __shfl_xor(l, 32);
    }
    {
      const char* wb = ws.acquire(2 + 2 * hd);
      f32x16 av;
      zero16(av);
#pragma unroll
      for (int kt = 0; kt < KT; ++kt) mma32(av, xf[kt], lds_frag<T>(wb + kt * TILE_B, lane));
      float v[16];
#pragma unroll
      for (int r = 0; r < 16; ++r) v[r] = av[r] * sk[r];
      f32x16 ao;
      zero16(ao);
      mma32(ao, pack_frag<T>(v), pack_frag<T>(pr));
      float gsel = gate[0];
#pragma unroll
      for (int k = 1; k < H; ++k) gsel = hd == k ? gate[k] : gsel;
      const float fin = gsel / l * PA;
      float o[16];
#pragma unroll
      for (int r = 0; r < 16; ++r) o[r] = ao[r] * fin;
      const Frag<T> of = pack_frag<T>(o);
#pragma unroll
      for (int mt = 0; mt < KT; ++mt) mma32(acco[mt], lds_frag<T>(wb + (KT + mt) * TILE_B, lane), of);
    }
  }
  f32x4 xv[KT][4];
#pragma unroll
  for (int mt = 0; mt < KT; ++mt)
#pragma unroll
    for (int a = 0; a < 4; ++a)
      xv[mt][a] = ok ? *reinterpret_cast<const f32x4*>(xrow + mt * 32 + 8 * a + 4 * g) : f32x4{0.f, 0.f, 0.f, 0.f};
  asm volatile("s_waitcnt vmcnt(0)" ::: "memory");
  __builtin_amdgcn_sched_barrier(0);
  float xn[KT][16];
#pragma unroll
  for (int mt = 0; mt < KT; ++mt)
#pragma unroll
    for (int a = 0; a < 4; ++a)
#pragma unroll
      for (int j = 0; j < 4; ++j) xn[mt][4 * a + j] = fmaf(acco[mt][4 * a + j], PW, xv[mt][a][j]);
  const long long t_ff = dbg ? clock64() : 0;
  ff_tail<T, C>(ws, 1 + 2 * H, xn, b1s, p.b2, xrow, nullptr, ok, lane, g);
  if (dbg && lane == 0) {
    long long* d = dbg + ((long)blockIdx.x * 4 + wave) * 6;
    d[0] = t_ring - t_in; d[1] = t_ff - t_ring; d[2] = clock64() - t_ff; d[3] = ws.t_wait; d[4] = ws.t_bar; d[5] = 0;
  }
}

template <typename T>
int launch_outff_t(const FusedOutFFP& p, hipStream_t s) {
  dim3 grid((unsigned)((p.M + 127) / 128)), block(256);
  switch (p.C) {
    case 32: hipLaunchKernelGGL((outff_fused_kernel<T, 32>), grid, block, 0, s, p); break;
    case 64: hipLaunchKernelGGL((outff_fused_kernel<T, 64>), grid, block, 0, s, p); break;
    case 128: hipLaunchKernelGGL((outff_fused_kernel<T, 128>), grid, block, 0, s, p); break;
    default: return -2;
  }
  return (int)hipGetLastError();
}
template <typename T>
int launch_attnff_t(const FusedAttnFFP& p, hipStream_t s) {
  dim3 grid((unsigned)((p.M + 127) / 128)), block(256);
  switch (p.C) {
    case 32: hipLaunchKernelGGL((attnff_fused_kernel<T, 32>), grid, block, 0, s, p); break;
    case 64: hipLaunchKernelGGL((attnff_fused_kernel<T, 64>), grid, block, 0, s, p); break;
    case 128: hipLaunchKernelGGL((attnff_fused_kernel<T, 128>), grid, block, 0, s, p); break;
    default: return -2;
  }
  return (int)hipGetLastError();
}

}

#ifdef BT_DEV
extern "C" int bt_debug_fused2_buffer(void* buf) {
  return (int)hipMemcpyToSymbol(HIP_SYMBOL(g_f2_dbg), &buf, sizeof buf);
}
#endif

int launch_outff_fused(const FusedOutFFP& p0, int prec, hipStream_t s) {
  if (p0.M <= 0) return -2;
  FusedOutFFP p = p0;
  p.abl = 0;
#ifdef BT_DEV
  static const int abl = getenv("BT_F2_ABL") ? atoi(getenv("BT_F2_ABL")) : 0;
  p.abl = abl;
#endif
  if (prec == BT_PREC_F32X3) return BT_HALF_IS_BF16 ? -2 : launch_outff_t<hl>(p, s);
  return prec == BT_PREC_F32 ? launch_outff_t<float>(p, s) : launch_outff_t<hf>(p, s);
}
int launch_attnff_fused(const FusedAttnFFP& p, int prec, hipStream_t s) {
  if (p.M <= 0) return -2;
  if (prec == BT_PREC_F32X3) return BT_HALF_IS_BF16 ? -2 : launch_attnff_t<hl>(p, s);
  return prec == BT_PREC_F32 ? launch_attnff_t<float>(p, s) : launch_attnff_t<hf>(p, s);
}
```

### beat_this_amd/csrc/gemm3.hip

```cpp
#include <cstdlib>

#include "common.h"
#include "kernels.h"

struct G3CfgS { static constexpr int BM = 128, BN = 128, BK = 32, WGM = 2, WGN = 2, NST = 3, OCC = 3; };
struct G3CfgB { static constexpr int BM = 256, BN = 256, BK = 64, WGM = 2, WGN = 4, NST = 2, OCC = 1; };
struct G3CfgT { static constexpr int BM = 192, BN = 256, BK = 64, WGM = 2, WGN = 4, NST = 2, OCC = 1; };
struct G3CfgSX { static constexpr int BM = 128, BN = 128, BK = 64, WGM = 2, WGN = 2, NST = 2, OCC = 2; };
struct G3CfgBX { static constexpr int BM = 256, BN = 256, BK = 64, WGM = 2, WGN = 4, NST = 2, OCC = 1; };
struct G3CfgTX { static constexpr int BM = 192, BN = 256, BK = 64, WGM = 2, WGN = 4, NST = 2, OCC = 1; };
struct G3CfgMX { static constexpr int BM = 256, BN = 128, BK = 32, WGM = 2, WGN = 2, NST = 3, OCC = 2; };
struct G3CfgHX { static constexpr int BM = 64, BN = 128, BK = 64, WGM = 2, WGN = 2, NST = 3, OCC = 2; };

#ifndef X3_NSPLIT
#define X3_NSPLIT 2
#endif

namespace {

typedef G3CfgS CfgS;
typedef G3CfgB CfgB;

constexpr unsigned OOB = 0x80000000u;

// ... 20 lines not shown
#pragma unroll
  for (int k = 0; k < 2; ++k) {
    unsigned x0 = pk2(v[8 * k], v[8 * k + 1]), x1 = pk2(v[8 * k + 2], v[8 * k + 3]);
    unsigned y0 = pk2(v[8 * k + 4], v[8 * k + 5]), y1 = pk2(v[8 * k + 6], v[8 * k + 7]);
    auto r0 = __builtin_amdgcn_permlane32_swap(x0, y0, false, false);
    auto r1 = __builtin_amdgcn_permlane32_swap(x1, y1, false, false);
    piece[k] = u32x4{r0[0], r1[0], r0[1], r1[1]};
  }
}

DEVI void split2(float a, float b, unsigned& whi, unsigned& wlo, float& amax) {
  split_hl(a, b, whi, wlo);
  amax = fmaxf(amax, fmaxf(fabsf(a), fabsf(b)));
}
DEVI void pack_row_hl(const float (&v)[16], u32x4 (&hi)[2], u32x4 (&lo)[2], float& amax) {
#pragma unroll
  for (int k = 0; k < 2; ++k) {
    unsigned xh[2], xl[2], yh[2], yl[2];
    split2(v[8 * k], v[8 * k + 1], xh[0], xl[0], amax);
    split2(v[8 * k + 2], v[8 * k + 3], xh[1], xl[1], amax);
    split2(v[8 * k + 4], v[8 * k + 5], yh[0], yl[0], amax);
    split2(v[8 * k + 6], v[8 * k + 7], yh[1], yl[1], amax);
    auto h0 = __builtin_amdgcn_permlane32_swap(xh[0], yh[0], false, false);
    auto h1 = __builtin_amdgcn_permlane32_swap(xh[1], yh[1], false, false);
    auto l0 = __builtin_amdgcn_permlane32_swap(xl[0], yl[0], false, false);
    auto l1 = __builtin_amdgcn_permlane32_swap(xl[1], yl[1], false, false);
    hi[k] = u32x4{h0[0], h1[0], h0[1], h1[1]};
    lo[k] = u32x4{l0[0], l1[0], l0[1], l1[1]};
  }
}
DEVI void pack_row_f8(const float (&v)[16], u32x4 (&hi)[2], u32x2 (&h8)[2], u32x2 (&l8)[2], float& amax) {
#pragma unroll
  for (int k = 0; k < 2; ++k) {
    unsigned xh[2], xl[2], yh[2], yl[2];
    split2(v[8 * k], v[8 * k + 1], xh[0], xl[0], amax);
    split2(v[8 * k + 2], v[8 * k + 3], xh[1], xl[1], amax);
    split2(v[8 * k + 4], v[8 * k + 5], yh[0], yl[0], amax);
    split2(v[8 * k + 6], v[8 * k + 7], yh[1], yl[1], amax);
    const unsigned x8 = pk4_f8(v[8 * k], v[8 * k + 1], v[8 * k + 2], v[8 * k + 3]);
    const unsigned y8 = pk4_f8(v[8 * k + 4], v[8 * k + 5], v[8 * k + 6], v[8 * k + 7]);
    const unsigned xl8 = lo4_f8(v[8 * k], v[8 * k + 1], v[8 * k + 2], v[8 * k + 3], xh[0], xh[1]);
    const unsigned yl8 = lo4_f8(v[8 * k + 4], v[8 * k + 5], v[8 * k + 6], v[8 * k + 7], yh[0], yh[1]);
    auto h0 = __builtin_amdgcn_permlane32_swap(xh[0], yh[0], false, false);
    auto h1 = __builtin_amdgcn_permlane32_swap(xh[1], yh[1], false, false);
    auto b8 = __builtin_amdgcn_permlane32_swap(x8, y8, false, false);
    auto c8 = __builtin_amdgcn_permlane32_swap(xl8, yl8, false, false);
    hi[k] = u32x4{h0[0], h1[0], h0[1], h1[1]};
    h8[k] = u32x2{b8[0], b8[1]};
    l8[k] = u32x2{c8[0], c8[1]};
  }
}
DEVI void flag_range(int* status, float amax, float limit = 65504.f) {
  if (status && __any(!(amax <= limit)) && (threadIdx.x & 63) == 0) atomicOr(status, 1);
}

template <int EPI, typename CFG, int X3 = 0, int ABL = 0>
__global__ __launch_bounds__(64 * CFG::WGM * CFG::WGN, (CFG::OCC * CFG::WGM * CFG::WGN + 3) / 4)
void gemm3_kernel(const Gemm3P p, int n_tiles, int total_tiles, int per_xcd, int nsplit) {
  constexpr int BM = CFG::BM, BN = CFG::BN, BK = CFG::BK, NST = CFG::NST;
  constexpr int NW = CFG::WGM * CFG::WGN, NT = 64 * NW;
  constexpr int TB = BM / CFG::WGM / 32;
  constexpr int FB = BN / CFG::WGN / 32;
  constexpr int ROWB = BK * 2;
  constexpr int KR = X3 ? BK / 2 : BK;
  constexpr bool HL16 = X3 && BK == 32;
  constexpr int EB = X3 ? 4 : 2;
  constexpr int CPR = ROWB / 16;
  constexpr int RPI = 64 / CPR;
  constexpr int A_BYTES = BM * ROWB, W_BYTES = BN * ROWB, ST_BYTES = A_BYTES + W_BYTES;
  constexpr int APC = A_BYTES / (NT * 16), WPC = W_BYTES / (NT * 16);
  static_assert(EPI != G3_QKV || TB == FB, "the V columns swap the operand roles: square wave tile needed");
  static_assert(BN / CFG::WGN == 64, "ssq partials are per 64 columns = one wave");
  static_assert(!X3 || ROWB == 128 || ROWB == 64, "hl32: a k-step is a whole group (128 B per row) or half of one (64 B)");
  static_assert(X3 != 2 || ROWB == 128, "hl8: a k-step is a whole 32-column group");
  static_assert(NST * ST_BYTES >= NW * 8192, "the epilogues stage 8 KB per wave in the ring's LDS");
  __shared__ __attribute__((aligned(16))) char smem[NST * ST_BYTES];
  const int bid = blockIdx.x;
  int m_tile, n_tile;
  if (nsplit <= 1) {
    const int tile = (bid & 7) * per_xcd + (bid >> 3);
    if (tile >= total_tiles) return;
    m_tile = tile / n_tiles;
    n_tile = tile - m_tile * n_tiles;
  } else {
    const int xcd = bid & 7, slot = bid >> 3;
    const int g = xcd % nsplit, j = xcd / nsplit, per_m = 8 / nsplit, nt = n_tiles / nsplit;
    const int m_local = slot / nt;
    m_tile = m_local * per_m + j;
    n_tile = g * nt + (slot - m_local * nt);
    if ((long)m_tile * n_tiles >= total_tiles) return;
  }
  const int m0 = m_tile * BM, n0 = n_tile * BN;
  const int tid = threadIdx.x, lane = tid & 63, wave = __builtin_amdgcn_readfirstlane(tid >> 6);
  const int g = lane >> 5, lr = lane & 31;
  const int wm = wave / CFG::WGN, wn = wave % CFG::WGN;
  const int nk = p.K / KR;
  auto swz = [](int r) { return ROWB == 64 ? (r >> 2) & 3 : (r >> 1) & 7; };
  const int Lv = p.nblk * 32;

  int kind = 0;
  if constexpr (EPI == G3_QKV) kind = n0 < 3 * p.inner ? n0 / p.inner : 3;
  const bool normal = EPI == G3_QKV && kind == 2;

  const unsigned a_bytes = (unsigned)((long)p.M * p.lda * EB), w_bytes = (unsigned)((long)n_tiles * BN * p.K * EB);
  static_assert(APC >= 1 && WPC >= 1, "tile too small for the workgroup");
  static_assert(APC <= 4 && WPC <= 4, "voffA / voffW hold at most 4 pieces");
  unsigned voffA[4], voffW[4];
  int tapmask[4] = {0, 0, 0, 0};
#pragma unroll
  for (int i = 0; i < APC; ++i) {
    const int r = (i * NW + wave) * RPI + lane / CPR;
    const int c = (lane % CPR) ^ swz(r);
    long row = (long)m0 + r;
    bool ok = row < p.M;
    if constexpr (EPI == G3_QKV) {
      const int seq = (int)(row / Lv), t = (int)(row - (long)seq * Lv);
      ok = seq < p.n_seq && t < p.L;
      row = (long)seq * p.L + t;
    }
#ifdef BT_ABL_HID_WRAP
    if (EPI == G3_RESID && X3 && p.K >= 1024 && p.conv_C2 == 0) row &= BT_ABL_HID_WRAP - 1;
#endif
    voffA[i] = ok ? (unsigned)(row * p.lda * EB + (HL16 ? (c >> 1) * 64 + (c & 1) * 16 : c * 16)) : OOB;
    if constexpr (EPI == G3_RESID) {
      const int t = p.conv_C2 > 0 ? (int)((row / p.conv_F) % p.conv_T) : 1;
      tapmask[i] = ok ? ((t >= 1 ? 1 : 0) | 2 | (t + 1 < p.conv_T ? 4 : 0)) : 0;
    }
  }
#pragma unroll
  for (int i = 0; i < WPC; ++i) {
    const int r = (i * NW + wave) * RPI + lane / CPR;
    const int c = (lane % CPR) ^ swz(r);
    voffW[i] = (unsigned)((long)(n0 + r) * p.K * EB + (HL16 ? (c >> 1) * 64 + (c & 1) * 16 : c * 16));
  }
  const bool conv = EPI == G3_RESID && p.conv_C2 > 0;
  const unsigned tap_bytes = conv ? (unsigned)(p.conv_F * p.conv_C2 * EB) : 0u;
  const int c2_shift = conv ? __builtin_ctz((unsigned)p.conv_C2) : 0;
  const rsrc_t rA = __builtin_amdgcn_make_buffer_rsrc(const_cast<char*>(reinterpret_cast<const char*>(p.A)) - tap_bytes, 0,
                                                      a_bytes + 2 * tap_bytes, 0x00020000);
  const rsrc_t rW = __builtin_amdgcn_make_buffer_rsrc(const_cast<void*>(p.W), 0, w_bytes, 0x00020000);
#define G3_ISSUE(kt, stage)                                                                                          \
  do {                                                                                                                \
    char* st_ = smem + (stage) * ST_BYTES + wave * 1024;                                                              \
    const int so_ = HL16 ? ((kt) >> 1) * 128 + ((kt) & 1) * 32 : (kt) * ROWB;                                         \
    if (conv) {                                                                                                       \
      const int tap_ = ((kt) * KR) >> c2_shift;                                                                       \
      const int kin_ = ((kt) * KR) & (p.conv_C2 - 1);                                                                 \
      const int soa_ = tap_ * (int)tap_bytes + (HL16 ? (kin_ >> 5) * 128 + ((kin_ >> 4) & 1) * 32 : kin_ * EB);      \
      _Pragma("unroll") for (int i_ = 0; i_ < APC; ++i_)                                                              \
          __builtin_amdgcn_raw_ptr_buffer_load_lds(rA, (lptr_t)(st_ + i_ * NW * 1024), 16,                            \
                                                   ((tapmask[i_] >> tap_) & 1) ? voffA[i_] : OOB, soa_, 0, 0);        \
    } else {                                                                                                          \
      _Pragma("unroll") for (int i_ = 0; i_ < APC; ++i_)                                                              \
          __builtin_amdgcn_raw_ptr_buffer_load_lds(rA, (lptr_t)(st_ + i_ * NW * 1024), 16, voffA[i_], so_, 0, 0);     \
    }                                                                                                                 \
// ... 277 lines not shown
    if (p.gelu) {
#pragma unroll
      for (int a = 0; a < FB; ++a)
#pragma unroll
        for (int b = 0; b < TB; ++b)
#pragma unroll
          for (int r = 0; r < 16; ++r) acc[a][b][r] = X3 ? gelu_erf(acc[a][b][r]) : gelu_tanh(acc[a][b][r]);
    }
#pragma unroll
    for (int b = 0; b < TB; ++b) {
      f32x4 xv[8];
#pragma unroll
      for (int ps = 0; ps < 8; ++ps) {
        const unsigned off = off_lane + (unsigned)(32 * b + 4 * ps) * ldx + colq[ps & 3];
        xv[ps] = (32 * b + 4 * ps < rows_left && !p.no_resid && p.x) ? *reinterpret_cast<const f32x4*>(p.x + off)
                                                               : f32x4{0.f, 0.f, 0.f, 0.f};
      }
#pragma unroll
      for (int a = 0; a < FB; ++a)
#pragma unroll
        for (int q = 0; q < 4; ++q)
          *reinterpret_cast<f32x4*>(wst + lr * 256 + (((8 * a + 2 * q + g) ^ (lr & 15)) << 4)) =
              f32x4{acc[a][b][4 * q], acc[a][b][4 * q + 1], acc[a][b][4 * q + 2], acc[a][b][4 * q + 3]};
#pragma unroll
      for (int ps = 0; ps < 8; ++ps) {
        const int r = ps * 4 + r4;
        const unsigned off = off_lane + (unsigned)(32 * b + 4 * ps) * ldx + colq[ps & 3];
        const bool ok = 32 * b + 4 * ps < rows_left;
        f32x4 v = *reinterpret_cast<const f32x4*>(wst + r * 256 + (cp << 4));
#pragma unroll
        for (int i = 0; i < 4; ++i) v[i] += xv[ps][i];
        if (ok) {
          if (p.x) *reinterpret_cast<f32x4*>(p.x + off) = v;
          if constexpr (X3) {
            if (xb) {
              const unsigned f = (unsigned)nb0 + colq[ps & 3];
              unsigned wh[2], wl[2];
              split2(v[0], v[1], wh[0], wl[0], amax);
              split2(v[2], v[3], wh[1], wl[1], amax);
              hf* d = xb + (2u * off - (f & 31u));
              *reinterpret_cast<u32x2*>(d) = u32x2{wh[0], wh[1]};
              if (p.x3 & G3_X3_OUT_F8) {
                char* gb = reinterpret_cast<char*>(d) - (f & 31u);
                *reinterpret_cast<unsigned*>(gb + 64) = pk4_f8(v[0], v[1], v[2], v[3]);
                *reinterpret_cast<unsigned*>(gb + 96) = lo4_f8(v[0], v[1], v[2], v[3], wh[0], wh[1]);
              } else {
                *reinterpret_cast<u32x2*>(d + 32) = u32x2{wl[0], wl[1]};
              }
            }
          } else {
            if (xb) *reinterpret_cast<u32x2*>(xb + off) = u32x2{pk2(v[0], v[1]), pk2(v[2], v[3])};
          }
        }
        float ssq = ok ? fmaf(v[0], v[0], fmaf(v[1], v[1], fmaf(v[2], v[2], v[3] * v[3]))) : 0.f;
#pragma unroll
        for (int o = 8; o > 0; o >>= 1) ssq += __shfl_xor(ssq, o);
        if (p.ssq_out && ok && cp == 0) p.ssq_out[(unsigned)(n0 / 64 + wn) * (unsigned)p.M + (unsigned)(row0 + 32 * b + r)] = ssq;
      }
    }
    }
  } else {
    constexpr int BLK_E = X3 ? 2048 : 1024;
    if (kind < 2) {
      hf* dst = reinterpret_cast<hf*>(kind == 0 ? p.qf : p.kf);
#pragma unroll
      for (int b = 0; b < TB; ++b) {
        if (tseq[b] >= p.n_seq) continue;
        const f32x4 (&cs)[4] = csv[b];
#pragma unroll
        for (int a = 0; a < FB; ++a) {
          const int head = (n0 - kind * p.inner + wn * 64 + a * 32) >> 5;
          hf* blk = dst + (((long)tseq[b] * p.heads + head) * p.nbp + tblk[b]) * BLK_E;
#pragma unroll
          for (int q = 0; q < 4; ++q) {
            const float e0 = acc[a][b][4 * q] * rs[b], o0 = acc[a][b][4 * q + 1] * rs[b];
            const float e1 = acc[a][b][4 * q + 2] * rs[b], o1 = acc[a][b][4 * q + 3] * rs[b];
            const float r0 = e0 * cs[q][0] - o0 * cs[q][1], r1 = o0 * cs[q][0] + e0 * cs[q][1];
            const float r2 = e1 * cs[q][2] - o1 * cs[q][3], r3 = o1 * cs[q][2] + e1 * cs[q][3];
            if constexpr (X3) {
              unsigned wh[2], wl[2];
              split2(r0, r1, wh[0], wl[0], amax);
              split2(r2, r3, wh[1], wl[1], amax);
              ST_STREAM(reinterpret_cast<u32x2*>(blk + (q * 32 + lr) * 8 + 4 * g), (u32x2{wh[0], wh[1]}));
              ST_STREAM(reinterpret_cast<u32x2*>(blk + 1024 + (q * 32 + lr) * 8 + 4 * g), (u32x2{wl[0], wl[1]}));
            } else {
              *reinterpret_cast<u32x2*>(blk + (q * 32 + lr) * 8 + 4 * g) = u32x2{pk2(r0, r1), pk2(r2, r3)};
            }
          }
        }
      }
    } else if (kind == 2) {
      hf* dst = reinterpret_cast<hf*>(p.vf);
#pragma unroll
      for (int a = 0; a < TB; ++a) {
        if (tseq[a] >= p.n_seq) continue;
        float sk[16];
#pragma unroll
        for (int r = 0; r < 16; ++r) sk[r] = __shfl(rs[a], crow(r, g));
#pragma unroll
        for (int b = 0; b < FB; ++b) {
          const int head = (n0 - 2 * p.inner + wn * 64 + b * 32) >> 5;
          hf* blk = dst + (((long)tseq[a] * p.heads + head) * p.nbp + tblk[a]) * BLK_E;
#pragma unroll
          for (int s = 0; s < 2; ++s) {
            unsigned w[4], wl[4] = {0, 0, 0, 0};
#pragma unroll
            for (int i = 0; i < 4; ++i) {
              const float v0 = acc[a][b][8 * s + 2 * i] * sk[8 * s + 2 * i], v1 = acc[a][b][8 * s + 2 * i + 1] * sk[8 * s + 2 * i + 1];
              if constexpr (X3) split2(v0, v1, w[i], wl[i], amax);
              else w[i] = pk2(v0, v1);
// ... 167 lines not shown
```

### beat_this_amd/csrc/kernels.h

```cpp
#pragma once
#include <hip/hip_runtime.h>
#include <stdint.h>

#ifndef BT_PREC_F32
#define BT_PREC_F32 0
#define BT_PREC_HALF 1
#endif
#ifndef BT_PREC_F32X3
#define BT_PREC_F32X3 3
#endif

enum {
  GEMM_EPI_STORE = 0,
  GEMM_EPI_RESID = 1,
  GEMM_EPI_QKV = 2
};
enum {
  GEMM_F_RMS = 1,
  GEMM_F_BIAS = 2,
  GEMM_F_GELU = 4,
  GEMM_F_OUT_F32 = 8,
  GEMM_F_A_F32 = 16,
  GEMM_F_CONV = 32,
  GEMM_F_ROWMAP = 64
// ... 57 lines not shown
  const void* qkv;
  long ld;
  const float* gates;
  void* out;
  int n_seq, L, heads, inner;
  int o_div;
  long o_outer, o_inner, o_tok;
};
int launch_attn_flash(const AttnP& p, int prec, hipStream_t s);

struct AttnFragP {
  const void* q; const void* k; const void* v;
  const float* gates;
  void* out;
  int n_seq, L, heads, inner, nbp;
  int o_div;
  long o_outer, o_inner, o_tok;
  int x3, out_f32;
  int* status;
  int* fix_mask;
};
int attn_frag_blocks(int L);
int launch_attn_frag(const AttnFragP& p, hipStream_t s);

struct QkvFrontP {
  const float* x;
  int B, T, F, C;
  const void* wfrag;
  const float* b_gates;
  const float* rope;
  void* q; void* k; void* v;
  float* gates;
  int nbp;
  int x3;
  int* status;
};
int launch_qkv_front(const QkvFrontP& p, hipStream_t s);

struct FusedFFP {
  float* x; long M; int C;
  const void* wfrag;
  const float* b1; const float* b2;
  void* xb;
};
int launch_ff_fused(const FusedFFP& p, int prec, hipStream_t s);

struct FusedOutFFP {
  float* x; long M; int C;
  const void* ao;
  const void* wfrag;
  const float* b1; const float* b2;
  void* xb;
  int abl;
};
int launch_outff_fused(const FusedOutFFP& p, int prec, hipStream_t s);
struct FusedAttnFFP {
  float* x; long M; int C;
  const float* b_gates; const float* rope;
  const void* wfrag;
  const float* b1; const float* b2;
};
int launch_attnff_fused(const FusedAttnFFP& p, int prec, hipStream_t s);

struct LayerTailP {
  float* x; long M; int C; int hidden;
  const void* ao;
  const void* wfrag;
  const float* b1; const float* b2;
  void* xb;
  float* ssq_out;
};
bool layer_tail_supported(int C, int hidden);
int launch_layer_tail(const LayerTailP& p, hipStream_t s);

struct StemP {
  const float* spect;
  float* x;
  const float* bn1_scale; const float* bn1_shift;
  const float* w;
  const float* bias;
  int B, T;
};
int launch_stem(const StemP& p, hipStream_t s);

struct HeadP {
  const float* x;
  const float* w;
  float b0, b1;
  float* beat; float* downbeat;
  int M, D, sum_head;
  int prenorm;
  int* status;
};
int launch_head(const HeadP& p, hipStream_t s);
int launch_clear_words(int* w, int n, hipStream_t s);
int launch_norm_out(const float* x, const float* gamma, float* y, long M, int D, hipStream_t s, int* status = nullptr);
int launch_finite_rows(const float* x, long M, int D, int* status, hipStream_t s);
int launch_shadow_ssq(const float* x, void* xb, float* ssq, long M, int D, hipStream_t s, int hl32 = 0);

struct bt_span_t { const float* data; long n; long out_off; long n_out; };

int launch_split(const float* spect, long n_frames, const int* starts, const int* table, int B, int T, float* chunks,
                 hipStream_t s, int border = 0);
int launch_aggregate(const float* cb, const float* cd, const int* starts, const int* table, const int* pieces, int n_pieces,
                     int B, int T, int border, long n_frames, float* beat, float* downbeat, hipStream_t s);
int launch_resample(const bt_span_t& one, const bt_span_t* tracks, int n_tracks, long max_n_out, int up, int down,
// ... 16 lines not shown
```

Measured before the change: 63370.

## Skip dead second query block in attention, add gate-tile QKV path and shadow-only outff

When a wave's second query block lies past the sequence end, the attention kernel now runs a one-block variant of the hand-written asm loop and the C++ tail, instead of computing a clamped duplicate block. The QKV GEMM gets a dedicated gate-column tile that computes only the sigmoid gates with f16x3 products. The fused out/FF kernel gains a shadow-only mode that skips the f32 residual store. The GEMM epilogue also skips the sum-of-squares reduction when no output buffer is given. These remove redundant MFMA work and stores, at the cost of more code paths and a large new inline-asm block.

```diff
diff --git a/beat_this_amd/csrc/attn2.hip b/beat_this_amd/csrc/attn2.hip
--- a/beat_this_amd/csrc/attn2.hip
+++ b/beat_this_amd/csrc/attn2.hip
@@ -689,33 +689,33 @@
   whi = u32x4{h[0], h[1], h[2], h[3]};
   wlo = u32x4{l[0], l[1], l[2], l[3]};
 }
-template <bool INIT, int QB>
+template <bool INIT, int QB, int NA = QB>
 DEVI void score_x(const KFragX& kf, const QStateX (&st)[QB], f32x16 (&sc)[QB]) {
 #pragma unroll
-  for (int j = 0; j < QB; ++j) {
+  for (int j = 0; j < NA; ++j) {
     if constexpr (INIT) sc[j] = st[j].negm; else zero16(sc[j]);
     sc[j] = MFMA32_H(kf.k0l, st[j].q0, sc[j]);
   }
 #pragma unroll
-  for (int j = 0; j < QB; ++j) sc[j] = MFMA32_H(kf.k1l, st[j].q1, sc[j]);
-#pragma unroll
-  for (int j = 0; j < QB; ++j) sc[j] = MFMA32_H(kf.k0, st[j].q0l, sc[j]);
-#pragma unroll
-  for (int j = 0; j < QB; ++j) sc[j] = MFMA32_H(kf.k1, st[j].q1l, sc[j]);
-#pragma unroll
-  for (int j = 0; j < QB; ++j) sc[j] = MFMA32_H(kf.k0, st[j].q0, sc[j]);
-#pragma unroll
-  for (int j = 0; j < QB; ++j) sc[j] = MFMA32_H(kf.k1, st[j].q1, sc[j]);
+  for (int j = 0; j < NA; ++j) sc[j] = MFMA32_H(kf.k1l, st[j].q1, sc[j]);
+#pragma unroll
+  for (int j = 0; j < NA; ++j) sc[j] = MFMA32_H(kf.k0, st[j].q0l, sc[j]);
+#pragma unroll
+  for (int j = 0; j < NA; ++j) sc[j] = MFMA32_H(kf.k1, st[j].q1l, sc[j]);
+#pragma unroll
+  for (int j = 0; j < NA; ++j) sc[j] = MFMA32_H(kf.k0, st[j].q0, sc[j]);
+#pragma unroll
+  for (int j = 0; j < NA; ++j) sc[j] = MFMA32_H(kf.k1, st[j].q1, sc[j]);
 }
 DEVI unsigned cvt_pk_rn(float a, float b) {
   unsigned w;
   asm("s_nop 0\n\tv_cvt_pk_f16_f32 %0, %1, %2" : "=v"(w) : "v"(a), "v"(b));
   return w;
 }
-template <bool SAFE, bool MASK, int QB, bool PRESUB = (QB == 1), bool P16 = false>
+template <bool SAFE, bool MASK, int QB, bool PRESUB = (QB == 1), bool P16 = false, int NA = QB>
 DEVI void finish_x(f32x16 (&sc)[QB], const VFragX& vf, int g, QStateX (&st)[QB], int key0, int L) {
 #pragma unroll
-  for (int j = 0; j < QB; ++j) {
+  for (int j = 0; j < NA; ++j) {
     if constexpr (SAFE) {
       if constexpr (MASK) {
 #pragma unroll
@@ -753,7 +753,7 @@
   if constexpr (P16) {
     u32x4 w0[QB], w1[QB];
 #pragma unroll
-    for (int j = 0; j < QB; ++j) {
+    for (int j = 0; j < NA; ++j) {
 #pragma unroll
       for (int i = 0; i < 4; ++i) {
         w0[j][i] = cvt_pk_rn(sc[j][2 * i], sc[j][2 * i + 1]);
@@ -763,33 +763,33 @@
       rowsum8(st[j].l4, w1[j]);
     }
 #pragma unroll
-    for (int j = 0; j < QB; ++j) st[j].acc = MFMA32_H(vf.v0l, __builtin_bit_cast(hfx8, w0[j]), st[j].acc);
-#pragma unroll
-    for (int j = 0; j < QB; ++j) st[j].acc = MFMA32_H(vf.v1l, __builtin_bit_cast(hfx8, w1[j]), st[j].acc);
-#pragma unroll
-    for (int j = 0; j < QB; ++j) st[j].acc = MFMA32_H(vf.v0, __builtin_bit_cast(hfx8, w0[j]), st[j].acc);
-#pragma unroll
-    for (int j = 0; j < QB; ++j) st[j].acc = MFMA32_H(vf.v1, __builtin_bit_cast(hfx8, w1[j]), st[j].acc);
+    for (int j = 0; j < NA; ++j) st[j].acc = MFMA32_H(vf.v0l, __builtin_bit_cast(hfx8, w0[j]), st[j].acc);
+#pragma unroll
+    for (int j = 0; j < NA; ++j) st[j].acc = MFMA32_H(vf.v1l, __builtin_bit_cast(hfx8, w1[j]), st[j].acc);
+#pragma unroll
+    for (int j = 0; j < NA; ++j) st[j].acc = MFMA32_H(vf.v0, __builtin_bit_cast(hfx8, w0[j]), st[j].acc);
+#pragma unroll
+    for (int j = 0; j < NA; ++j) st[j].acc = MFMA32_H(vf.v1, __builtin_bit_cast(hfx8, w1[j]), st[j].acc);
     return;
   }
   u32x4 h0[QB], l0[QB], h1[QB], l1[QB];
 #pragma unroll
-  for (int j = 0; j < QB; ++j) {
+  for (int j = 0; j < NA; ++j) {
     split8(sc[j], 0, h0[j], l0[j]);
     split8(sc[j], 1, h1[j], l1[j]);
   }
 #pragma unroll
-  for (int j = 0; j < QB; ++j) st[j].acc = MFMA32_H(vf.v0l, __builtin_bit_cast(hfx8, h0[j]), st[j].acc);
-#pragma unroll
-  for (int j = 0; j < QB; ++j) st[j].acc = MFMA32_H(vf.v1l, __builtin_bit_cast(hfx8, h1[j]), st[j].acc);
-#pragma unroll
-  for (int j = 0; j < QB; ++j) st[j].acc = MFMA32_H(vf.v0, __builtin_bit_cast(hfx8, l0[j]), st[j].acc);
-#pragma unroll
-  for (int j = 0; j < QB; ++j) st[j].acc = MFMA32_H(vf.v1, __builtin_bit_cast(hfx8, l1[j]), st[j].acc);
-#pragma unroll
-  for (int j = 0; j < QB; ++j) st[j].acc = MFMA32_H(vf.v0, __builtin_bit_cast(hfx8, h0[j]), st[j].acc);
-#pragma unroll
-  for (int j = 0; j < QB; ++j) st[j].acc = MFMA32_H(vf.v1, __builtin_bit_cast(hfx8, h1[j]), st[j].acc);
+  for (int j = 0; j < NA; ++j) st[j].acc = MFMA32_H(vf.v0l, __builtin_bit_cast(hfx8, h0[j]), st[j].acc);
+#pragma unroll
+  for (int j = 0; j < NA; ++j) st[j].acc = MFMA32_H(vf.v1l, __builtin_bit_cast(hfx8, h1[j]), st[j].acc);
+#pragma unroll
+  for (int j = 0; j < NA; ++j) st[j].acc = MFMA32_H(vf.v0, __builtin_bit_cast(hfx8, l0[j]), st[j].acc);
+#pragma unroll
+  for (int j = 0; j < NA; ++j) st[j].acc = MFMA32_H(vf.v1, __builtin_bit_cast(hfx8, l1[j]), st[j].acc);
+#pragma unroll
+  for (int j = 0; j < NA; ++j) st[j].acc = MFMA32_H(vf.v0, __builtin_bit_cast(hfx8, h0[j]), st[j].acc);
+#pragma unroll
+  for (int j = 0; j < NA; ++j) st[j].acc = MFMA32_H(vf.v1, __builtin_bit_cast(hfx8, h1[j]), st[j].acc);
 }
 
 template <int KBX>
@@ -829,15 +829,15 @@
   }
 }
 
-template <int QB>
+template <int QB, int NA = QB>
 DEVI void diag_max_x(const char* kseq, const int (&qblk)[QB], int g, int lr, const QStateX (&st)[QB], int L, float (&dmax)[QB]) {
   KFragX kd[QB];
 #pragma unroll
-  for (int j = 0; j < QB; ++j) kd[j] = ld_kx(kseq + (long)qblk[j] * BLKX_BYTES, g, lr);
+  for (int j = 0; j < NA; ++j) kd[j] = ld_kx(kseq + (long)qblk[j] * BLKX_BYTES, g, lr);
   asm volatile("s_waitcnt vmcnt(0)" ::: "memory");
   __builtin_amdgcn_sched_barrier(0);
 #pragma unroll
-  for (int j = 0; j < QB; ++j) {
+  for (int j = 0; j < NA; ++j) {
     f32x16 sd;
     zero16(sd);
     sd = MFMA32_H(kd[j].k0l, st[j].q0, sd);
@@ -852,23 +852,23 @@
     dmax[j] = m;
   }
 }
-template <int QB>
+template <int QB, int NA = QB>
 DEVI void ref_max_x(const char* smem, int g, int lr, QStateX (&st)[QB], int L, int nblk, const float (&dmax)[QB]) {
   float bm[QB];
 #pragma unroll
-  for (int j = 0; j < QB; ++j) bm[j] = dmax[j];
+  for (int j = 0; j < NA; ++j) bm[j] = dmax[j];
   const int nref = min(2, nblk);
   for (int c = 0; c < nref; ++c) {
     const KFragX kf = ld_kx(smem + c * BLKX_BYTES, g, lr);
     f32x16 s0[QB];
-    score_x<false, QB>(kf, st, s0);
-#pragma unroll
-    for (int j = 0; j < QB; ++j)
+    score_x<false, QB, NA>(kf, st, s0);
+#pragma unroll
+    for (int j = 0; j < NA; ++j)
 #pragma unroll
       for (int r = 0; r < 16; ++r) bm[j] = fmaxf(bm[j], (32 * c + crow(r, g) < L) ? s0[j][r] : -1e30f);
   }
 #pragma unroll
-  for (int j = 0; j < QB; ++j) {
+  for (int j = 0; j < NA; ++j) {
     const float m = ceilf(fmaxf(bm[j], __shfl_xor(bm[j], 32)));
 #pragma unroll
     for (int r = 0; r < 16; ++r) st[j].negm[r] = -m - P_SHIFT_X;
@@ -1065,10 +1065,18 @@
   const char* vseq = reinterpret_cast<const char*>(p.v) + seq_off;
   QStateX st[QB];
   const int qb0 = (qt * 4 + wave) * QB;
+#ifndef BT_X3Q2_ONE
+#define BT_X3Q2_ONE 1
+#endif
+  const bool one = BT_X3Q2_ONE && __builtin_amdgcn_readfirstlane((int)(qb0 + 1 >= nblk)) != 0;
   auto load_q = [&]() {
     const int ln = lane_id_fresh(), gg = ln >> 5, ll = ln & 31;
 #pragma unroll
     for (int j = 0; j < QB; ++j) {
+      if (j == 1 && one) {
+        st[j].q0 = st[j].q1 = st[j].q0l = st[j].q1l = hfx8{0, 0, 0, 0, 0, 0, 0, 0};
+        continue;
+      }
       const int qbc = min(qb0 + j, nblk - 1);
       const char* qblk = reinterpret_cast<const char*>(p.q) + seq_off + (long)qbc * BLKX_BYTES;
       st[j].q0 = *reinterpret_cast<const hfx8*>(qblk + ((2 * gg) * 32 + ll) * 16);
@@ -1083,7 +1091,12 @@
   float dmax[QB];
   {
     const int qbi[QB] = {min(qb0, nblk - 1), min(qb0 + 1, nblk - 1)};
-    diag_max_x<QB>(kseq, qbi, g, lr, st, L, dmax);
+    if (one) {
+      diag_max_x<QB, 1>(kseq, qbi, g, lr, st, L, dmax);
+      dmax[1] = -1e30f;
+    } else {
+      diag_max_x<QB>(kseq, qbi, g, lr, st, L, dmax);
+    }
   }
   const unsigned seq_bytes = (unsigned)p.nbp * BLKX_BYTES;
   const rsrc_t rk = __builtin_amdgcn_make_buffer_rsrc(const_cast<char*>(kseq), 0, seq_bytes, 0x00020000);
@@ -1121,6 +1134,20 @@
     const unsigned m0base = (unsigned)__builtin_amdgcn_readfirstlane((int)(lds0 + wave * 1024));
     const float m1 = -1.0f;
     int t = 0, soff = 3 * TILEX_BYTES;
+    if (one) {
+    if constexpr (P16)
+      asm volatile(ATTN_X3Q2P_ONE_ASM
+                   : "+v"(st[0].acc), "+v"(st[1].acc), "+v"(st[0].l4), "+v"(st[1].l4), "+s"(t), "+s"(soff)
+                   : "v"(st[0].q0), "v"(st[0].q1), "v"(st[0].q0l), "v"(st[0].q1l), "v"(st[1].q0), "v"(st[1].q1), "v"(st[1].q0l), "v"(st[1].q1l),
+                     "v"(st[0].negm), "v"(st[1].negm), "v"(klane), "v"(vlane), "v"(dmaoff), "s"(dk), "s"(dv), "s"(m0base), "s"(m1), "s"(nfull)
+                   : ATTN_X3Q2P_CLOBBERS);
+    else
+      asm volatile(ATTN_X3Q2_ONE_ASM
+                   : "+v"(st[0].acc), "+v"(st[1].acc), "+v"(st[0].l), "+v"(st[1].l), "+s"(t), "+s"(soff)
+                   : "v"(st[0].q0), "v"(st[0].q1), "v"(st[0].q0l), "v"(st[0].q1l), "v"(st[1].q0), "v"(st[1].q1), "v"(st[1].q0l), "v"(st[1].q1l),
+                     "v"(st[0].negm), "v"(st[1].negm), "v"(klane), "v"(vlane), "v"(dmaoff), "s"(dk), "s"(dv), "s"(m0base), "s"(m1), "s"(nfull)
+                   : ATTN_X3Q2_CLOBBERS);
+    } else {
     if constexpr (P16)
       asm volatile(ATTN_X3Q2P_ASM
                    : "+v"(st[0].acc), "+v"(st[1].acc), "+v"(st[0].l4), "+v"(st[1].l4), "+s"(t), "+s"(soff)
@@ -1134,6 +1161,7 @@
                      "v"(st[0].negm), "v"(st[1].negm), "v"(klane), "v"(vlane), "v"(dmaoff), "s"(dk), "s"(dv), "s"(m0base), "s"(m1), "s"(nfull)
                    : ATTN_X3Q2_CLOBBERS);
     }
+    }
     asm volatile("s_waitcnt vmcnt(0)" ::: "memory");
     __syncthreads();
     if (nfull < ntiles) {
@@ -1152,9 +1180,15 @@
         const KFragX kf = ld_kx(kb + c * BLKX_BYTES, g2, lr2);
         const VFragX vf = ld_vx(vb + c * BLKX_BYTES, lane2);
         f32x16 sc[QB];
-        score_x<true, QB>(kf, st, sc);
-        if (partial && blk == nblk - 1) finish_x<false, true, QB, true, P16>(sc, vf, g2, st, blk * 32, L);
-        else finish_x<false, false, QB, true, P16>(sc, vf, g2, st, blk * 32, L);
+        if (one) {
+          score_x<true, QB, 1>(kf, st, sc);
+          if (partial && blk == nblk - 1) finish_x<false, true, QB, true, P16, 1>(sc, vf, g2, st, blk * 32, L);
+          else finish_x<false, false, QB, true, P16, 1>(sc, vf, g2, st, blk * 32, L);
+        } else {
+          score_x<true, QB>(kf, st, sc);
+          if (partial && blk == nblk - 1) finish_x<false, true, QB, true, P16>(sc, vf, g2, st, blk * 32, L);
+          else finish_x<false, false, QB, true, P16>(sc, vf, g2, st, blk * 32, L);
+        }
       }
       __syncthreads();
     }
@@ -1164,7 +1198,12 @@
   stage_ring(2);
   asm volatile("s_waitcnt vmcnt(8)" ::: "memory");
   __syncthreads();
-  ref_max_x<QB>(smem, g, lr, st, L, nblk, dmax);
+  if (one) {
+    ref_max_x<QB, 1>(smem, g, lr, st, L, nblk, dmax);
+    zero16(st[1].negm);
+  } else {
+    ref_max_x<QB>(smem, g, lr, st, L, nblk, dmax);
+  }
   fast_pass();
   auto lane_sum = [&](int j) { return P16 ? st[j].l4[0] : st[j].l; };
   const int laneE = lane_id_fresh(), gE = laneE >> 5, lrE = laneE & 31;
@@ -1186,6 +1225,7 @@
   float amax = 0.f;
 #pragma unroll
   for (int j = 0; j < QB; ++j) {
+    if (j == 1 && one) continue;
     const int qi = (qb0 + j) * 32 + lrE;
     const bool okq = qb0 + j < nblk && qi < L && !bad[j];
     const float gatev = okq ? p.gates[(long)sh * p.nbp * 32 + qi] : 0.f;
diff --git a/beat_this_amd/csrc/attn_x3_loop.inc b/beat_this_amd/csrc/attn_x3_loop.inc
--- a/beat_this_amd/csrc/attn_x3_loop.inc
+++ b/beat_this_amd/csrc/attn_x3_loop.inc
@@ -2732,6 +2732,418 @@
   "s_nop 7\n\t" \
   "s_nop 7\n\t" \
   ""
+#define ATTN_X3Q2_ONE_ASM \
+  "s_nop 4\n\t" \
+  "s_and_b32 s88, %4, 3\n\t" \
+  "s_lshl_b32 s88, s88, 14\n\t" \
+  "v_add_u32_e32 v121, s88, %16\n\t" \
+  "ds_read_b128 v[176:179], v121 offset:0\n\t" \
+  "ds_read_b128 v[180:183], v121 offset:512\n\t" \
+  "ds_read_b128 v[184:187], v121 offset:2048\n\t" \
+  "ds_read_b128 v[188:191], v121 offset:2560\n\t" \
+  "v_add_u32_e32 v122, s88, %17\n\t" \
+  "ds_read_b128 v[144:147], v122 offset:8192\n\t" \
+  "ds_read_b128 v[148:151], v122 offset:9216\n\t" \
+  "ds_read_b128 v[152:155], v122 offset:10240\n\t" \
+  "ds_read_b128 v[156:159], v122 offset:11264\n\t" \
+  "ds_read_b128 v[128:131], v122 offset:8192\n\t" \
+  "ds_read_b128 v[132:135], v122 offset:9216\n\t" \
+  "ds_read_b128 v[136:139], v122 offset:10240\n\t" \
+  "ds_read_b128 v[140:143], v122 offset:11264\n\t" \
+  "v_mov_b32_e32 v200, 0\n\t" \
+  "v_mov_b32_e32 v192, 0\n\t" \
+  "v_mov_b32_e32 v201, 0\n\t" \
+  "v_mov_b32_e32 v193, 0\n\t" \
+  "v_mov_b32_e32 v202, 0\n\t" \
+  "v_mov_b32_e32 v194, 0\n\t" \
+  "v_mov_b32_e32 v203, 0\n\t" \
+  "v_mov_b32_e32 v195, 0\n\t" \
+  "v_mov_b32_e32 v204, 0\n\t" \
+  "v_mov_b32_e32 v196, 0\n\t" \
+  "v_mov_b32_e32 v205, 0\n\t" \
+  "v_mov_b32_e32 v197, 0\n\t" \
+  "v_mov_b32_e32 v206, 0\n\t" \
+  "v_mov_b32_e32 v198, 0\n\t" \
+  "v_mov_b32_e32 v207, 0\n\t" \
+  "v_mov_b32_e32 v199, 0\n\t" \
+  "s_waitcnt lgkmcnt(0)\n\t" \
+  "v_mfma_f32_32x32x16_f16 v[240:255], v[184:187], %6, %14\n\t" \
+  "v_mfma_f32_32x32x16_f16 v[240:255], v[188:191], %7, v[240:255]\n\t" \
+  "v_mfma_f32_32x32x16_f16 v[240:255], v[176:179], %8, v[240:255]\n\t" \
+  "v_mfma_f32_32x32x16_f16 v[240:255], v[180:183], %9, v[240:255]\n\t" \
+  "v_mfma_f32_32x32x16_f16 v[240:255], v[176:179], %6, v[240:255]\n\t" \
+  "v_mfma_f32_32x32x16_f16 v[240:255], v[180:183], %7, v[240:255]\n\t" \
+  "s_nop 7\n\t" \
+  "s_nop 7\n\t" \
+  "Lloop%=:\n\t" \
+  "s_and_b32 s88, %4, 3\n\t" \
+  "s_lshl_b32 s88, s88, 14\n\t" \
+  "s_add_u32 s89, %4, 1\n\t" \
+  "s_and_b32 s89, s89, 3\n\t" \
+  "s_lshl_b32 s89, s89, 14\n\t" \
+  "v_add_u32_e32 v121, s88, %16\n\t" \
+  "v_add_u32_e32 v123, s88, %17\n\t" \
+  "v_add_u32_e32 v122, s89, %16\n\t" \
+  "v_add_u32_e32 v124, s89, %17\n\t" \
+  "v_exp_f32_e32 v240, v240\n\t" \
+  "v_exp_f32_e32 v241, v241\n\t" \
+  "v_exp_f32_e32 v242, v242\n\t" \
+  "v_exp_f32_e32 v243, v243\n\t" \
+  "ds_read_b128 v[160:163], v121 offset:4096\n\t" \
+  "v_exp_f32_e32 v244, v244\n\t" \
+  "v_exp_f32_e32 v245, v245\n\t" \
+  "v_exp_f32_e32 v246, v246\n\t" \
+  "v_exp_f32_e32 v247, v247\n\t" \
+  "ds_read_b128 v[164:167], v121 offset:4608\n\t" \
+  "v_exp_f32_e32 v248, v248\n\t" \
+  "v_exp_f32_e32 v249, v249\n\t" \
+  "v_exp_f32_e32 v250, v250\n\t" \
+  "v_exp_f32_e32 v251, v251\n\t" \
+  "ds_read_b128 v[168:171], v121 offset:6144\n\t" \
+  "v_exp_f32_e32 v252, v252\n\t" \
+  "v_exp_f32_e32 v253, v253\n\t" \
+  "v_exp_f32_e32 v254, v254\n\t" \
+  "v_exp_f32_e32 v255, v255\n\t" \
+  "ds_read_b128 v[172:175], v121 offset:6656\n\t" \
+  "v_cvt_pk_f16_f32 v216, v240, v241\n\t" \
+  "v_cvt_pk_f16_f32 v217, v242, v243\n\t" \
+  "v_add_f32_e32 v116, v240, v241\n\t" \
+  "v_add_f32_e32 v117, v242, v243\n\t" \
+  "v_fma_mixlo_f16 v208, v216, %22, v240 op_sel:[0,0,0] op_sel_hi:[1,0,0]\n\t" \
+  "v_fma_mixlo_f16 v209, v217, %22, v242 op_sel:[0,0,0] op_sel_hi:[1,0,0]\n\t" \
+  "v_fma_mixhi_f16 v208, v216, %22, v241 op_sel:[1,0,0] op_sel_hi:[1,0,0]\n\t" \
+  "v_fma_mixhi_f16 v209, v217, %22, v243 op_sel:[1,0,0] op_sel_hi:[1,0,0]\n\t" \
+  "v_cvt_pk_f16_f32 v218, v244, v245\n\t" \
+  "v_cvt_pk_f16_f32 v219, v246, v247\n\t" \
+  "v_add_f32_e32 v116, v116, v117\n\t" \
+  "v_add_f32_e32 v118, v244, v245\n\t" \
+  "v_add_f32_e32 v119, v246, v247\n\t" \
+  "v_fma_mixlo_f16 v210, v218, %22, v244 op_sel:[0,0,0] op_sel_hi:[1,0,0]\n\t" \
+  "v_fma_mixlo_f16 v211, v219, %22, v246 op_sel:[0,0,0] op_sel_hi:[1,0,0]\n\t" \
+  "v_fma_mixhi_f16 v210, v218, %22, v245 op_sel:[1,0,0] op_sel_hi:[1,0,0]\n\t" \
+  "v_fma_mixhi_f16 v211, v219, %22, v247 op_sel:[1,0,0] op_sel_hi:[1,0,0]\n\t" \
+  "v_add_f32_e32 v118, v118, v119\n\t" \
+  "v_add_f32_e32 v116, v116, v118\n\t" \
+  "v_cvt_pk_f16_f32 v220, v248, v249\n\t" \
+  "v_cvt_pk_f16_f32 v221, v250, v251\n\t" \
+  "v_add_f32_e32 v120, v248, v249\n\t" \
+  "v_add_f32_e32 v117, v250, v251\n\t" \
+  "v_fma_mixlo_f16 v212, v220, %22, v248 op_sel:[0,0,0] op_sel_hi:[1,0,0]\n\t" \
+  "v_fma_mixlo_f16 v213, v221, %22, v250 op_sel:[0,0,0] op_sel_hi:[1,0,0]\n\t" \
+  "v_fma_mixhi_f16 v212, v220, %22, v249 op_sel:[1,0,0] op_sel_hi:[1,0,0]\n\t" \
+  "v_fma_mixhi_f16 v213, v221, %22, v251 op_sel:[1,0,0] op_sel_hi:[1,0,0]\n\t" \
+  "v_add_f32_e32 v120, v120, v117\n\t" \
+  "v_cvt_pk_f16_f32 v222, v252, v253\n\t" \
+  "v_cvt_pk_f16_f32 v223, v254, v255\n\t" \
+  "v_add_f32_e32 v118, v252, v253\n\t" \
+  "v_add_f32_e32 v119, v254, v255\n\t" \
+  "v_fma_mixlo_f16 v214, v222, %22, v252 op_sel:[0,0,0] op_sel_hi:[1,0,0]\n\t" \
+  "v_fma_mixlo_f16 v215, v223, %22, v254 op_sel:[0,0,0] op_sel_hi:[1,0,0]\n\t" \
+  "v_fma_mixhi_f16 v214, v222, %22, v253 op_sel:[1,0,0] op_sel_hi:[1,0,0]\n\t" \
+  "v_fma_mixhi_f16 v215, v223, %22, v255 op_sel:[1,0,0] op_sel_hi:[1,0,0]\n\t" \
+  "v_add_f32_e32 v118, v118, v119\n\t" \
+  "v_add_f32_e32 v120, v120, v118\n\t" \
+  "v_add_f32_e32 v116, v116, v120\n\t" \
+  "v_add_f32_e32 %2, %2, v116\n\t" \
+  "s_nop 3\n\t" \
+  "s_waitcnt lgkmcnt(0)\n\t" \
+  "v_mfma_f32_32x32x16_f16 v[240:255], v[168:171], %6, %14\n\t" \
+  "ds_read_b128 v[128:131], v123 offset:12288\n\t" \
+  "v_mfma_f32_32x32x16_f16 %0, v[152:155], v[216:219], %0\n\t" \
+  "ds_read_b128 v[132:135], v123 offset:13312\n\t" \
+  "v_mfma_f32_32x32x16_f16 v[240:255], v[172:175], %7, v[240:255]\n\t" \
+  "ds_read_b128 v[136:139], v123 offset:14336\n\t" \
+  "v_mfma_f32_32x32x16_f16 %0, v[156:159], v[220:223], %0\n\t" \
+  "ds_read_b128 v[140:143], v123 offset:15360\n\t" \
+  "v_mfma_f32_32x32x16_f16 v[240:255], v[160:163], %8, v[240:255]\n\t" \
+  "v_mfma_f32_32x32x16_f16 %0, v[144:147], v[208:211], %0\n\t" \
+  "v_mfma_f32_32x32x16_f16 v[240:255], v[164:167], %9, v[240:255]\n\t" \
+  "v_mfma_f32_32x32x16_f16 %0, v[148:151], v[212:215], %0\n\t" \
+  "v_mfma_f32_32x32x16_f16 v[240:255], v[160:163], %6, v[240:255]\n\t" \
+  "v_mfma_f32_32x32x16_f16 %0, v[144:147], v[216:219], %0\n\t" \
+  "v_mfma_f32_32x32x16_f16 v[240:255], v[164:167], %7, v[240:255]\n\t" \
+  "v_mfma_f32_32x32x16_f16 %0, v[148:151], v[220:223], %0\n\t" \
+  "s_nop 7\n\t" \
+  "s_nop 3\n\t" \
+  "s_waitcnt vmcnt(4) lgkmcnt(0)\n\t" \
+  "s_barrier\n\t" \
+  "v_exp_f32_e32 v240, v240\n\t" \
+  "v_exp_f32_e32 v241, v241\n\t" \
+  "v_exp_f32_e32 v242, v242\n\t" \
+  "v_exp_f32_e32 v243, v243\n\t" \
+  "ds_read_b128 v[176:179], v122 offset:0\n\t" \
+  "v_exp_f32_e32 v244, v244\n\t" \
+  "v_exp_f32_e32 v245, v245\n\t" \
+  "v_exp_f32_e32 v246, v246\n\t" \
+  "v_exp_f32_e32 v247, v247\n\t" \
+  "ds_read_b128 v[180:183], v122 offset:512\n\t" \
+  "v_exp_f32_e32 v248, v248\n\t" \
+  "v_exp_f32_e32 v249, v249\n\t" \
+  "v_exp_f32_e32 v250, v250\n\t" \
+  "v_exp_f32_e32 v251, v251\n\t" \
+  "ds_read_b128 v[184:187], v122 offset:2048\n\t" \
+  "v_exp_f32_e32 v252, v252\n\t" \
+  "v_exp_f32_e32 v253, v253\n\t" \
+  "v_exp_f32_e32 v254, v254\n\t" \
+  "v_exp_f32_e32 v255, v255\n\t" \
+  "ds_read_b128 v[188:191], v122 offset:2560\n\t" \
+  "v_cvt_pk_f16_f32 v216, v240, v241\n\t" \
+  "v_cvt_pk_f16_f32 v217, v242, v243\n\t" \
+  "v_add_f32_e32 v116, v240, v241\n\t" \
+  "v_add_f32_e32 v117, v242, v243\n\t" \
+  "v_fma_mixlo_f16 v208, v216, %22, v240 op_sel:[0,0,0] op_sel_hi:[1,0,0]\n\t" \
+  "s_add_u32 s91, %4, 3\n\t" \
+  "s_and_b32 s91, s91, 3\n\t" \
+  "s_lshl_b32 s91, s91, 14\n\t" \
+  "s_add_u32 s91, s91, %21\n\t" \
+  "v_fma_mixlo_f16 v209, v217, %22, v242 op_sel:[0,0,0] op_sel_hi:[1,0,0]\n\t" \
+  "v_fma_mixhi_f16 v208, v216, %22, v241 op_sel:[1,0,0] op_sel_hi:[1,0,0]\n\t" \
+  "v_fma_mixhi_f16 v209, v217, %22, v243 op_sel:[1,0,0] op_sel_hi:[1,0,0]\n\t" \
+  "v_cvt_pk_f16_f32 v218, v244, v245\n\t" \
+  "v_cvt_pk_f16_f32 v219, v246, v247\n\t" \
+  "s_add_u32 m0, s91, 0\n\t" \
+  "s_add_u32 s90, %5, 0\n\t" \
+  "buffer_load_dwordx4 %18, %19, s90 offen lds\n\t" \
+  "v_add_f32_e32 v116, v116, v117\n\t" \
+  "v_add_f32_e32 v118, v244, v245\n\t" \
+  "v_add_f32_e32 v119, v246, v247\n\t" \
+  "v_fma_mixlo_f16 v210, v218, %22, v244 op_sel:[0,0,0] op_sel_hi:[1,0,0]\n\t" \
+  "v_fma_mixlo_f16 v211, v219, %22, v246 op_sel:[0,0,0] op_sel_hi:[1,0,0]\n\t" \
+  "s_add_u32 m0, s91, 4096\n\t" \
+  "s_add_u32 s90, %5, 4096\n\t" \
+  "buffer_load_dwordx4 %18, %19, s90 offen lds\n\t" \
+  "v_fma_mixhi_f16 v210, v218, %22, v245 op_sel:[1,0,0] op_sel_hi:[1,0,0]\n\t" \
+  "v_fma_mixhi_f16 v211, v219, %22, v247 op_sel:[1,0,0] op_sel_hi:[1,0,0]\n\t" \
+  "v_add_f32_e32 v118, v118, v119\n\t" \
+  "v_add_f32_e32 v116, v116, v118\n\t" \
+  "v_cvt_pk_f16_f32 v220, v248, v249\n\t" \
+  "s_add_u32 m0, s91, 8192\n\t" \
+  "s_add_u32 s90, %5, 0\n\t" \
+  "buffer_load_dwordx4 %18, %20, s90 offen lds\n\t" \
+  "v_cvt_pk_f16_f32 v221, v250, v251\n\t" \
+  "v_add_f32_e32 v120, v248, v249\n\t" \
+  "v_add_f32_e32 v117, v250, v251\n\t" \
+  "v_fma_mixlo_f16 v212, v220, %22, v248 op_sel:[0,0,0] op_sel_hi:[1,0,0]\n\t" \
+  "v_fma_mixlo_f16 v213, v221, %22, v250 op_sel:[0,0,0] op_sel_hi:[1,0,0]\n\t" \
+  "s_add_u32 m0, s91, 12288\n\t" \
+  "s_add_u32 s90, %5, 4096\n\t" \
+  "buffer_load_dwordx4 %18, %20, s90 offen lds\n\t" \
+  "v_fma_mixhi_f16 v212, v220, %22, v249 op_sel:[1,0,0] op_sel_hi:[1,0,0]\n\t" \
+  "v_fma_mixhi_f16 v213, v221, %22, v251 op_sel:[1,0,0] op_sel_hi:[1,0,0]\n\t" \
+  "v_add_f32_e32 v120, v120, v117\n\t" \
+  "v_cvt_pk_f16_f32 v222, v252, v253\n\t" \
+  "v_cvt_pk_f16_f32 v223, v254, v255\n\t" \
+  "v_add_f32_e32 v118, v252, v253\n\t" \
+  "v_add_f32_e32 v119, v254, v255\n\t" \
+  "v_fma_mixlo_f16 v214, v222, %22, v252 op_sel:[0,0,0] op_sel_hi:[1,0,0]\n\t" \
+  "v_fma_mixlo_f16 v215, v223, %22, v254 op_sel:[0,0,0] op_sel_hi:[1,0,0]\n\t" \
+  "v_fma_mixhi_f16 v214, v222, %22, v253 op_sel:[1,0,0] op_sel_hi:[1,0,0]\n\t" \
+  "v_fma_mixhi_f16 v215, v223, %22, v255 op_sel:[1,0,0] op_sel_hi:[1,0,0]\n\t" \
+  "v_add_f32_e32 v118, v118, v119\n\t" \
+  "v_add_f32_e32 v120, v120, v118\n\t" \
+  "v_add_f32_e32 v116, v116, v120\n\t" \
+  "v_add_f32_e32 %2, %2, v116\n\t" \
+  "s_nop 3\n\t" \
+  "s_waitcnt lgkmcnt(0)\n\t" \
+  "v_mfma_f32_32x32x16_f16 v[240:255], v[184:187], %6, %14\n\t" \
+  "ds_read_b128 v[144:147], v124 offset:8192\n\t" \
+  "v_mfma_f32_32x32x16_f16 %0, v[136:139], v[216:219], %0\n\t" \
+  "ds_read_b128 v[148:151], v124 offset:9216\n\t" \
+  "v_mfma_f32_32x32x16_f16 v[240:255], v[188:191], %7, v[240:255]\n\t" \
+  "ds_read_b128 v[152:155], v124 offset:10240\n\t" \
+  "v_mfma_f32_32x32x16_f16 %0, v[140:143], v[220:223], %0\n\t" \
+  "ds_read_b128 v[156:159], v124 offset:11264\n\t" \
+  "v_mfma_f32_32x32x16_f16 v[240:255], v[176:179], %8, v[240:255]\n\t" \
+  "v_mfma_f32_32x32x16_f16 %0, v[128:131], v[208:211], %0\n\t" \
+  "v_mfma_f32_32x32x16_f16 v[240:255], v[180:183], %9, v[240:255]\n\t" \
+  "v_mfma_f32_32x32x16_f16 %0, v[132:135], v[212:215], %0\n\t" \
+  "v_mfma_f32_32x32x16_f16 v[240:255], v[176:179], %6, v[240:255]\n\t" \
+  "v_mfma_f32_32x32x16_f16 %0, v[128:131], v[216:219], %0\n\t" \
+  "v_mfma_f32_32x32x16_f16 v[240:255], v[180:183], %7, v[240:255]\n\t" \
+  "v_mfma_f32_32x32x16_f16 %0, v[132:135], v[220:223], %0\n\t" \
+  "s_nop 7\n\t" \
+  "s_nop 3\n\t" \
+  "s_add_u32 %5, %5, 8192\n\t" \
+  "s_add_u32 %4, %4, 1\n\t" \
+  "s_cmp_lt_i32 %4, %23\n\t" \
+  "s_cbranch_scc1 Lloop%=\n\t" \
+  "s_waitcnt lgkmcnt(0)\n\t" \
+  "s_nop 7\n\t" \
+  "s_nop 7\n\t" \
+  ""
+#define ATTN_X3Q2P_ONE_ASM \
+  "s_nop 4\n\t" \
+  "v_mov_b32_e32 v126, 0x3c003c00\n\t" \
+  "v_mov_b32_e32 v127, 0x3c003c00\n\t" \
+  "s_and_b32 s88, %4, 3\n\t" \
+  "s_lshl_b32 s88, s88, 14\n\t" \
+  "v_add_u32_e32 v121, s88, %16\n\t" \
+  "ds_read_b128 v[176:179], v121 offset:0\n\t" \
+  "ds_read_b128 v[180:183], v121 offset:512\n\t" \
+  "ds_read_b128 v[184:187], v121 offset:2048\n\t" \
+  "ds_read_b128 v[188:191], v121 offset:2560\n\t" \
+  "v_add_u32_e32 v122, s88, %17\n\t" \
+  "ds_read_b128 v[144:147], v122 offset:8192\n\t" \
+  "ds_read_b128 v[148:151], v122 offset:9216\n\t" \
+  "ds_read_b128 v[152:155], v122 offset:10240\n\t" \
+  "ds_read_b128 v[156:159], v122 offset:11264\n\t" \
+  "ds_read_b128 v[128:131], v122 offset:8192\n\t" \
+  "ds_read_b128 v[132:135], v122 offset:9216\n\t" \
+  "ds_read_b128 v[136:139], v122 offset:10240\n\t" \
+  "ds_read_b128 v[140:143], v122 offset:11264\n\t" \
+  "v_mov_b32_e32 v200, 0\n\t" \
+  "v_mov_b32_e32 v201, 0\n\t" \
+  "v_mov_b32_e32 v202, 0\n\t" \
+  "v_mov_b32_e32 v203, 0\n\t" \
+  "v_mov_b32_e32 v204, 0\n\t" \
+  "v_mov_b32_e32 v205, 0\n\t" \
+  "v_mov_b32_e32 v206, 0\n\t" \
+  "v_mov_b32_e32 v207, 0\n\t" \
+  "s_waitcnt lgkmcnt(0)\n\t" \
+  "v_mfma_f32_32x32x16_f16 v[240:255], v[184:187], %6, %14\n\t" \
+  "v_mfma_f32_32x32x16_f16 v[240:255], v[188:191], %7, v[240:255]\n\t" \
+  "v_mfma_f32_32x32x16_f16 v[240:255], v[176:179], %8, v[240:255]\n\t" \
+  "v_mfma_f32_32x32x16_f16 v[240:255], v[180:183], %9, v[240:255]\n\t" \
+  "v_mfma_f32_32x32x16_f16 v[240:255], v[176:179], %6, v[240:255]\n\t" \
+  "v_mfma_f32_32x32x16_f16 v[240:255], v[180:183], %7, v[240:255]\n\t" \
+  "s_nop 7\n\t" \
+  "s_nop 7\n\t" \
+  "Lloop%=:\n\t" \
+  "s_and_b32 s88, %4, 3\n\t" \
+  "s_lshl_b32 s88, s88, 14\n\t" \
+  "s_add_u32 s89, %4, 1\n\t" \
+  "s_and_b32 s89, s89, 3\n\t" \
+  "s_lshl_b32 s89, s89, 14\n\t" \
+  "v_add_u32_e32 v121, s88, %16\n\t" \
+  "v_add_u32_e32 v123, s88, %17\n\t" \
+  "v_add_u32_e32 v122, s89, %16\n\t" \
+  "v_add_u32_e32 v124, s89, %17\n\t" \
+  "v_exp_f32_e32 v240, v240\n\t" \
+  "v_exp_f32_e32 v241, v241\n\t" \
+  "v_exp_f32_e32 v242, v242\n\t" \
+  "v_exp_f32_e32 v243, v243\n\t" \
+  "ds_read_b128 v[160:163], v121 offset:4096\n\t" \
+  "v_exp_f32_e32 v244, v244\n\t" \
+  "v_exp_f32_e32 v245, v245\n\t" \
+  "v_exp_f32_e32 v246, v246\n\t" \
+  "v_exp_f32_e32 v247, v247\n\t" \
+  "ds_read_b128 v[164:167], v121 offset:4608\n\t" \
+  "v_exp_f32_e32 v248, v248\n\t" \
+  "v_exp_f32_e32 v249, v249\n\t" \
+  "v_exp_f32_e32 v250, v250\n\t" \
+  "v_exp_f32_e32 v251, v251\n\t" \
+  "ds_read_b128 v[168:171], v121 offset:6144\n\t" \
+  "v_exp_f32_e32 v252, v252\n\t" \
+  "v_exp_f32_e32 v253, v253\n\t" \
+  "v_exp_f32_e32 v254, v254\n\t" \
+  "v_exp_f32_e32 v255, v255\n\t" \
+  "ds_read_b128 v[172:175], v121 offset:6656\n\t" \
+  "v_cvt_pk_f16_f32 v216, v240, v241\n\t" \
+  "v_cvt_pk_f16_f32 v217, v242, v243\n\t" \
+  "v_cvt_pk_f16_f32 v218, v244, v245\n\t" \
+  "v_cvt_pk_f16_f32 v219, v246, v247\n\t" \
+  "v_cvt_pk_f16_f32 v220, v248, v249\n\t" \
+  "v_cvt_pk_f16_f32 v221, v250, v251\n\t" \
+  "v_cvt_pk_f16_f32 v222, v252, v253\n\t" \
+  "v_cvt_pk_f16_f32 v223, v254, v255\n\t" \
+  "s_nop 3\n\t" \
+  "s_waitcnt lgkmcnt(0)\n\t" \
+  "v_mfma_f32_32x32x16_f16 %0, v[152:155], v[216:219], %0\n\t" \
+  "ds_read_b128 v[128:131], v123 offset:12288\n\t" \
+  "v_mfma_f32_4x4x4_16b_f16 %2, v[126:127], v[216:217], %2\n\t" \
+  "v_mfma_f32_32x32x16_f16 v[240:255], v[168:171], %6, %14\n\t" \
+  "v_mfma_f32_32x32x16_f16 v[240:255], v[172:175], %7, v[240:255]\n\t" \
+  "ds_read_b128 v[132:135], v123 offset:13312\n\t" \
+  "ds_read_b128 v[136:139], v123 offset:14336\n\t" \
+  "v_mfma_f32_32x32x16_f16 %0, v[156:159], v[220:223], %0\n\t" \
+  "ds_read_b128 v[140:143], v123 offset:15360\n\t" \
+  "v_mfma_f32_4x4x4_16b_f16 %2, v[126:127], v[218:219], %2\n\t" \
+  "v_mfma_f32_32x32x16_f16 v[240:255], v[160:163], %8, v[240:255]\n\t" \
+  "v_mfma_f32_32x32x16_f16 v[240:255], v[164:167], %9, v[240:255]\n\t" \
+  "v_mfma_f32_32x32x16_f16 %0, v[144:147], v[216:219], %0\n\t" \
+  "v_mfma_f32_4x4x4_16b_f16 %2, v[126:127], v[220:221], %2\n\t" \
+  "v_mfma_f32_32x32x16_f16 v[240:255], v[160:163], %6, v[240:255]\n\t" \
+  "v_mfma_f32_32x32x16_f16 v[240:255], v[164:167], %7, v[240:255]\n\t" \
+  "v_mfma_f32_32x32x16_f16 %0, v[148:151], v[220:223], %0\n\t" \
+  "v_mfma_f32_4x4x4_16b_f16 %2, v[126:127], v[222:223], %2\n\t" \
+  "s_nop 7\n\t" \
+  "s_nop 3\n\t" \
+  "s_waitcnt vmcnt(4) lgkmcnt(0)\n\t" \
+  "s_barrier\n\t" \
+  "v_exp_f32_e32 v240, v240\n\t" \
+  "v_exp_f32_e32 v241, v241\n\t" \
+  "v_exp_f32_e32 v242, v242\n\t" \
+  "v_exp_f32_e32 v243, v243\n\t" \
+  "ds_read_b128 v[176:179], v122 offset:0\n\t" \
+  "v_exp_f32_e32 v244, v244\n\t" \
+  "v_exp_f32_e32 v245, v245\n\t" \
+  "v_exp_f32_e32 v246, v246\n\t" \
+  "v_exp_f32_e32 v247, v247\n\t" \
+  "ds_read_b128 v[180:183], v122 offset:512\n\t" \
+  "v_exp_f32_e32 v248, v248\n\t" \
+  "v_exp_f32_e32 v249, v249\n\t" \
+  "v_exp_f32_e32 v250, v250\n\t" \
+  "v_exp_f32_e32 v251, v251\n\t" \
+  "ds_read_b128 v[184:187], v122 offset:2048\n\t" \
+  "v_exp_f32_e32 v252, v252\n\t" \
+  "v_exp_f32_e32 v253, v253\n\t" \
+  "v_exp_f32_e32 v254, v254\n\t" \
+  "v_exp_f32_e32 v255, v255\n\t" \
+  "ds_read_b128 v[188:191], v122 offset:2560\n\t" \
+  "s_add_u32 s91, %4, 3\n\t" \
+  "s_and_b32 s91, s91, 3\n\t" \
+  "s_lshl_b32 s91, s91, 14\n\t" \
+  "s_add_u32 s91, s91, %21\n\t" \
+  "v_cvt_pk_f16_f32 v216, v240, v241\n\t" \
+  "v_cvt_pk_f16_f32 v217, v242, v243\n\t" \
+  "v_cvt_pk_f16_f32 v218, v244, v245\n\t" \
+  "v_cvt_pk_f16_f32 v219, v246, v247\n\t" \
+  "s_add_u32 m0, s91, 0\n\t" \
+  "s_add_u32 s90, %5, 0\n\t" \
+  "buffer_load_dwordx4 %18, %19, s90 offen lds\n\t" \
+  "v_cvt_pk_f16_f32 v220, v248, v249\n\t" \
+  "v_cvt_pk_f16_f32 v221, v250, v251\n\t" \
+  "s_add_u32 m0, s91, 4096\n\t" \
+  "s_add_u32 s90, %5, 4096\n\t" \
+  "buffer_load_dwordx4 %18, %19, s90 offen lds\n\t" \
+  "v_cvt_pk_f16_f32 v222, v252, v253\n\t" \
+  "v_cvt_pk_f16_f32 v223, v254, v255\n\t" \
+  "s_add_u32 m0, s91, 8192\n\t" \
+  "s_add_u32 s90, %5, 0\n\t" \
+  "buffer_load_dwordx4 %18, %20, s90 offen lds\n\t" \
+  "s_add_u32 m0, s91, 12288\n\t" \
+  "s_add_u32 s90, %5, 4096\n\t" \
+  "buffer_load_dwordx4 %18, %20, s90 offen lds\n\t" \
+  "s_nop 3\n\t" \
+  "s_waitcnt lgkmcnt(0)\n\t" \
+  "v_mfma_f32_32x32x16_f16 %0, v[136:139], v[216:219], %0\n\t" \
+  "ds_read_b128 v[144:147], v124 offset:8192\n\t" \
+  "v_mfma_f32_4x4x4_16b_f16 %2, v[126:127], v[216:217], %2\n\t" \
+  "v_mfma_f32_32x32x16_f16 v[240:255], v[184:187], %6, %14\n\t" \
+  "v_mfma_f32_32x32x16_f16 v[240:255], v[188:191], %7, v[240:255]\n\t" \
+  "ds_read_b128 v[148:151], v124 offset:9216\n\t" \
+  "ds_read_b128 v[152:155], v124 offset:10240\n\t" \
+  "v_mfma_f32_32x32x16_f16 %0, v[140:143], v[220:223], %0\n\t" \
+  "ds_read_b128 v[156:159], v124 offset:11264\n\t" \
+  "v_mfma_f32_4x4x4_16b_f16 %2, v[126:127], v[218:219], %2\n\t" \
+  "v_mfma_f32_32x32x16_f16 v[240:255], v[176:179], %8, v[240:255]\n\t" \
+  "v_mfma_f32_32x32x16_f16 v[240:255], v[180:183], %9, v[240:255]\n\t" \
+  "v_mfma_f32_32x32x16_f16 %0, v[128:131], v[216:219], %0\n\t" \
+  "v_mfma_f32_4x4x4_16b_f16 %2, v[126:127], v[220:221], %2\n\t" \
+  "v_mfma_f32_32x32x16_f16 v[240:255], v[176:179], %6, v[240:255]\n\t" \
+  "v_mfma_f32_32x32x16_f16 v[240:255], v[180:183], %7, v[240:255]\n\t" \
+  "v_mfma_f32_32x32x16_f16 %0, v[132:135], v[220:223], %0\n\t" \
+  "v_mfma_f32_4x4x4_16b_f16 %2, v[126:127], v[222:223], %2\n\t" \
+  "s_nop 7\n\t" \
+  "s_nop 3\n\t" \
+  "s_add_u32 %5, %5, 8192\n\t" \
+  "s_add_u32 %4, %4, 1\n\t" \
+  "s_cmp_lt_i32 %4, %23\n\t" \
+  "s_cbranch_scc1 Lloop%=\n\t" \
+  "s_waitcnt lgkmcnt(0)\n\t" \
+  "s_nop 7\n\t" \
+  "s_nop 7\n\t" \
+  ""
 #define ATTN_X3Q2_CLOBBERS "v116", "v117", "v118", "v119", "v120", "v121", "v122", "v123", "v124", "v128", "v129", "v130", "v131", "v132", "v133", "v134", "v135", "v136", "v137", "v138", "v139", "v140", "v141", "v142", "v143", "v144", "v145", "v146", "v147", "v148", "v149", "v150", "v151", "v152", "v153", "v154", "v155", "v156", "v157", "v158", "v159", "v160", "v161", "v162", "v163", "v164", "v165", "v166", "v167", "v168", "v169", "v170", "v171", "v172", "v173", "v174", "v175", "v176", "v177", "v178", "v179", "v180", "v181", "v182", "v183", "v184", "v185", "v186", "v187", "v188", "v189", "v190", "v191", "v192", "v193", "v194", "v195", "v196", "v197", "v198", "v199", "v200", "v201", "v202", "v203", "v204", "v205", "v206", "v207", "v208", "v209", "v210", "v211", "v212", "v213", "v214", "v215", "v216", "v217", "v218", "v219", "v220", "v221", "v222", "v223", "v224", "v225", "v226", "v227", "v228", "v229", "v230", "v231", "v232", "v233", "v234", "v235", "v236", "v237", "v238", "v239", "v240", "v241", "v242", "v243", "v244", "v245", "v246", "v247", "v248", "v249", "v250", "v251", "v252", "v253", "v254", "v255", "s88", "s89", "s90", "s91", "s92", "s93", "s94", "s95", "scc", "memory"
 #define ATTN_X3Q2P_CLOBBERS "v121", "v122", "v123", "v124", "v126", "v127", "v128", "v129", "v130", "v131", "v132", "v133", "v134", "v135", "v136", "v137", "v138", "v139", "v140", "v141", "v142", "v143", "v144", "v145", "v146", "v147", "v148", "v149", "v150", "v151", "v152", "v153", "v154", "v155", "v156", "v157", "v158", "v159", "v160", "v161", "v162", "v163", "v164", "v165", "v166", "v167", "v168", "v169", "v170", "v171", "v172", "v173", "v174", "v175", "v176", "v177", "v178", "v179", "v180", "v181", "v182", "v183", "v184", "v185", "v186", "v187", "v188", "v189", "v190", "v191", "v200", "v201", "v202", "v203", "v204", "v205", "v206", "v207", "v216", "v217", "v218", "v219", "v220", "v221", "v222", "v223", "v224", "v225", "v226", "v227", "v228", "v229", "v230", "v231", "v232", "v233", "v234", "v235", "v236", "v237", "v238", "v239", "v240", "v241", "v242", "v243", "v244", "v245", "v246", "v247", "v248", "v249", "v250", "v251", "v252", "v253", "v254", "v255", "s88", "s89", "s90", "s91", "s92", "s93", "s94", "s95", "scc", "memory"
 #define ATTN_X3Q2_KBX 2
diff --git a/beat_this_amd/csrc/engine.hip b/beat_this_amd/csrc/engine.hip
--- a/beat_this_amd/csrc/engine.hip
+++ b/beat_this_amd/csrc/engine.hip
@@ -187,6 +187,7 @@
   bool ff8;
   bool next8;
   bool tail;
+  bool shadow_dead;
 };
 
 enum { LAYERS_GENERIC, LAYERS_FRAG_HALF, LAYERS_FRAG_X3 };
@@ -198,12 +199,15 @@
   int x3_attn, x3_attn_front;
   bool half_shadow;
   int layers;
-  struct Block { PairRoute freq, time; bool conv3; } blk[3];
+  struct Block { PairRoute freq, time; bool conv3; bool x_dead; } blk[3];
   bool lin3, lin_f8;
   struct Layer { PairRoute pair; FragLayer frag; } layer[BT_MAX_LAYERS];
 };
 
-Route plan_route(const bt_engine& e, int B, int T, int prec, int first, const Workspace& ws) {
+#ifndef BT_SKIP_DEAD_STORES
+#define BT_SKIP_DEAD_STORES 1
+#endif
+Route plan_route(const bt_engine& e, int B, int T, int prec, int first, int last, const Workspace& ws) {
   const bt_model_desc& d = e.d;
   const int D = d.transformer_dim;
   Route r;
@@ -238,6 +242,7 @@
     const Gemm3P cg = conv3_params(d, ws, blk, B, T, frag_x3, blk == 2 && lin3_fits);
     rb.conv3 = d.partial_transformers && rb.time.outff && (frag_x3 ? rb.time.split : frag_half) && cg.N >= 128 && cg.W &&
                gemm3_supported(cg);
+    rb.x_dead = BT_SKIP_DEAD_STORES && rb.conv3 && frag_x3;
   }
   r.lin3 = lin3_fits && (!frag_x3 || r.blk[2].conv3);
   r.lin_f8 = r.lin3 && frag_x3 && e.x3_gemm_fp8 >= 2 && d.n_layers > 0 && d.layers[0].w_qkvg_f8;
@@ -251,6 +256,7 @@
     f.ff8 = frag_x3 && e.x3_gemm_fp8 >= 1 && w.w_ff1_f8 && w.w_ff2_f8;
     f.next8 = frag_x3 && e.x3_gemm_fp8 >= 2 && l + 1 < d.n_layers && d.layers[l + 1].w_qkvg_f8 && w.w_ff2_f8;
     f.tail = frag_half && w.w_tail_frag && layer_tail_supported(D, d.ff_mult * D);
+    f.shadow_dead = BT_SKIP_DEAD_STORES && frag_x3 && last == 2 && l == d.n_layers - 1;
   }
   return r;
 }
@@ -348,7 +354,7 @@
 }
 
 int time_half(prof::State* pf, const bt_pair_weights& pw, const PairRoute& pr, const Route& r, const float* rope, float* x,
-              const Workspace& ws, int B, int T, int F, void* shadow, hipStream_t s) {
+              const Workspace& ws, int B, int T, int F, void* shadow, bool shadow_only, hipStream_t s) {
   const long M = (long)B * T * F;
   if (int rc = check_rows(M)) return rc;
   if (pr.time_frag) {
@@ -371,7 +377,7 @@
   if (pr.outff) {
     FusedOutFFP f;
     f.x = x; f.M = M; f.C = pw.dim; f.ao = ws.ao; f.wfrag = pr.split ? pw.w_outff_frag_x3 : pw.w_outff_frag[r.fp];
-    f.b1 = pw.b_ff1; f.b2 = pw.b_ff2; f.xb = shadow; f.abl = 0;
+    f.b1 = pw.b_ff1; f.b2 = pw.b_ff2; f.xb = shadow; f.abl = 0; f.shadow_only = shadow && shadow_only && pr.split;
     LAUNCH_CAT(CAT_FF_FUSED, s, launch_outff_fused(f, pr.split ? BT_PREC_F32X3 : r.fp, s), "fused out-projection + feed-forward");
     return BT_OK;
   }
@@ -419,7 +425,7 @@
   memset(&g, 0, sizeof g);
   g.A = ws.hid; g.lda = HID; g.M = M; g.K = HID; g.W = w(pw.w_ff2, pw.w_ff2_x3, pw.w_ff2_f8, f.ff8); g.N = D; g.epi = G3_RESID;
   g.x3 = r.x3 | (f.ff8 ? G3_X3_F8 : 0) | (f.next8 ? G3_X3_OUT_F8 : 0); g.status = status;
-  g.bias = pw.b_ff2; g.x = ws.xm; g.ldx = D; g.xb = ws.xmb; g.ssq_out = ws.ssq[0];
+  g.bias = pw.b_ff2; g.x = ws.xm; g.ldx = D; g.xb = f.shadow_dead ? nullptr : ws.xmb; g.ssq_out = f.shadow_dead ? nullptr : ws.ssq[0];
   LAUNCH_CAT(CAT_FF2, s, launch_gemm3(g, s), r.x3 ? "ff2 gemm (hi + lo)" : "ff2 gemm");
   return BT_OK;
 }
@@ -433,7 +439,7 @@
     float* x = front_x(ws, blk);
     if (d.partial_transformers) {
       if (int rc = freq_half(pf, d.front[blk][0], rb.freq, r, d.rope, x, B, T, 32 >> blk, s)) return rc;
-      if (int rc = time_half(pf, d.front[blk][1], rb.time, r, d.rope, x, ws, B, T, 32 >> blk, rb.conv3 ? ws.hid : nullptr, s))
+      if (int rc = time_half(pf, d.front[blk][1], rb.time, r, d.rope, x, ws, B, T, 32 >> blk, rb.conv3 ? ws.hid : nullptr, rb.x_dead, s))
         return rc;
     }
     if (rb.conv3) {
@@ -548,7 +554,7 @@
   const Workspace ws = carve((char*)d_ws, B, T, D, d.ff_mult, prec, (size_t)e->ws_guard);
   if (ws.total > ws_bytes) return bt_set_error(BT_ERR_WORKSPACE, "workspace too small");
   if (prec == BT_PREC_F32X3 && BT_HALF_IS_BF16) return bt_set_error(BT_ERR_ARG, "BT_PREC_F32X3 needs an IEEE fp16 build");
-  const Route r = plan_route(*e, B, T, prec, first, ws);
+  const Route r = plan_route(*e, B, T, prec, first, last, ws);
   hipStream_t s = (hipStream_t)stream;
   if (r.x3) LAUNCH(launch_clear_words(ws.status, 1, s), "clearing the range flag");
   int* status = r.x3 ? ws.status : nullptr;
@@ -605,7 +611,7 @@
   const int D = d.transformer_dim;
   const Workspace ws = carve((char*)d_ws, B, T, D, d.ff_mult, prec, (size_t)e->ws_guard);
   if (ws.total > ws_bytes) return bt_set_error(BT_ERR_WORKSPACE, "workspace too small");
-  const Route r = plan_route(*e, B, T, prec, 0, ws);
+  const Route r = plan_route(*e, B, T, prec, 0, 0, ws);
   hipStream_t s = (hipStream_t)stream;
   const bool block_unit = unit == BT_UNIT_PARTIAL || unit == BT_UNIT_CONV;
   const bool layer_unit = unit == BT_UNIT_ATTN || unit == BT_UNIT_FF;
@@ -629,7 +635,7 @@
       const Route::Block& rb = r.blk[index];
       if (int rc = copy_in((size_t)B * T * 1024 * 4)) return rc;
       if (int rc = freq_half(pf, d.front[index][0], rb.freq, r, d.rope, d_out, B, T, 32 >> index, s)) return rc;
-      return time_half(pf, d.front[index][1], rb.time, r, d.rope, d_out, ws, B, T, 32 >> index, nullptr, s);
+      return time_half(pf, d.front[index][1], rb.time, r, d.rope, d_out, ws, B, T, 32 >> index, nullptr, false, s);
     }
     case BT_UNIT_CONV: {
       const GemmP g = conv_params(d, index, r.wp, d_in, d_out, B, T, true);
@@ -1004,7 +1010,7 @@
   if (!w || !d_ao || !d_x || M <= 0 || w->dim > 128 || !wf) return bt_set_error(BT_ERR_ARG, "bad argument to bt_outff_fused");
   FusedOutFFP f;
   f.x = d_x; f.M = M; f.C = w->dim; f.ao = d_ao; f.wfrag = wf; f.b1 = w->b_ff1; f.b2 = w->b_ff2;
-  f.xb = prec == BT_PREC_F32 ? nullptr : d_xb; f.abl = 0;
+  f.xb = prec == BT_PREC_F32 ? nullptr : d_xb; f.abl = 0; f.shadow_only = 0;
   LAUNCH(launch_outff_fused(f, prec, (hipStream_t)stream), "fused out-projection + feed-forward");
   return BT_OK;
 }
diff --git a/beat_this_amd/csrc/fused2.hip b/beat_this_amd/csrc/fused2.hip
--- a/beat_this_amd/csrc/fused2.hip
+++ b/beat_this_amd/csrc/fused2.hip
@@ -68,7 +68,7 @@
   }
 };
 
-template <typename T, int C>
+template <typename T, int C, bool STORE_X = true>
 DEVI void ff_tail(WRing<T, C>& ws, int step0, float (&xn)[C / 32][16], const float* b1s, const float* b2,
                   float* xrow, hf* xbrow, bool ok, int lane, int g) {
   constexpr int KT = C / 32, HB = 4 * C / 32;
@@ -116,7 +116,9 @@
       const f32x4 b = *reinterpret_cast<const f32x4*>(b2 + f0);
 #pragma unroll
       for (int j = 0; j < 4; ++j) v[a][j] = fmaf(acc2[mt][4 * a + j], PW, b[j]);
-      if (ok) *reinterpret_cast<f32x4*>(xrow + f0) = v[a];
+      if constexpr (STORE_X) {
+        if (ok) *reinterpret_cast<f32x4*>(xrow + f0) = v[a];
+      }
     }
     if (xbrow) {
       typedef __attribute__((ext_vector_type(4))) unsigned int u32x4;
@@ -151,7 +153,7 @@
   }
 }
 
-template <typename T, int C>
+template <typename T, int C, bool STORE_X = true>
 __global__ __launch_bounds__(256) void outff_fused_kernel(const FusedOutFFP p) {
   constexpr int KT = C / 32, HB = 4 * C / 32;
   constexpr int TILE_B = WRing<T, C>::TILE_B, STEP_B = WRing<T, C>::STEP_B, NST = WRing<T, C>::NST;
@@ -195,7 +197,7 @@
     for (int r = 0; r < 16; ++r) xn[mt][r] = fmaf(acc[r], OpScale<T>::PW, xn[mt][r]);
   }
   hf* xbrow = p.xb ? reinterpret_cast<hf*>(p.xb) + tok * C * (std::is_same<T, hl>::value ? 2 : 1) : nullptr;
-  ff_tail<T, C>(ws, KT, xn, b1s, p.b2, xrow, xbrow, ok_st, lane, g);
+  ff_tail<T, C, STORE_X>(ws, KT, xn, b1s, p.b2, xrow, xbrow, ok_st, lane, g);
 }
 
 template <typename T, int C>
@@ -353,6 +355,19 @@
 template <typename T>
 int launch_outff_t(const FusedOutFFP& p, hipStream_t s) {
   dim3 grid((unsigned)((p.M + 127) / 128)), block(256);
+  if constexpr (std::is_same<T, hl>::value) {
+    if (p.shadow_only) {
+      if (!p.xb) return -2;
+      switch (p.C) {
+        case 64: hipLaunchKernelGGL((outff_fused_kernel<T, 64, false>), grid, block, 0, s, p); break;
+        case 128: hipLaunchKernelGGL((outff_fused_kernel<T, 128, false>), grid, block, 0, s, p); break;
+        default: return -2;
+      }
+      return (int)hipGetLastError();
+    }
+  } else if (p.shadow_only) {
+    return -2;
+  }
   switch (p.C) {
     case 32: hipLaunchKernelGGL((outff_fused_kernel<T, 32>), grid, block, 0, s, p); break;
     case 64: hipLaunchKernelGGL((outff_fused_kernel<T, 64>), grid, block, 0, s, p); break;
diff --git a/beat_this_amd/csrc/gemm3.hip b/beat_this_amd/csrc/gemm3.hip
--- a/beat_this_amd/csrc/gemm3.hip
+++ b/beat_this_amd/csrc/gemm3.hip
@@ -96,6 +96,103 @@
 }
 DEVI void flag_range(int* status, float amax, float limit = 65504.f) {
   if (status && __any(!(amax <= limit)) && (threadIdx.x & 63) == 0) atomicOr(status, 1);
+}
+
+#ifndef BT_QKV_GATE_TILE
+#define BT_QKV_GATE_TILE 1
+#endif
+template <typename CFG>
+DEVI void qkv_gate_tile_x3(const Gemm3P& p, char* smem, int m0, int n0, int n_tiles, int lane, int wave) {
+  constexpr int BM = CFG::BM, BN = CFG::BN, ROWB = CFG::BK * 2, NST = CFG::NST, KR = CFG::BK / 2, EB = 4;
+  constexpr int NW = CFG::WGM * CFG::WGN, NT = 64 * NW;
+  constexpr int CPR = ROWB / 16, RPI = 64 / CPR;
+  constexpr int A_BYTES = BM * ROWB, ST_BYTES = A_BYTES + BN * ROWB;
+  constexpr int APC = A_BYTES / (NT * 16), LPS = APC + 1;
+  static_assert(ROWB == 128 && NW * 32 == BM && 32 * ROWB == NT * 16 && APC <= 4, "one 32-token block per wave, one W piece per thread");
+  const int g = lane >> 5, lr = lane & 31;
+  const int nk = p.K / KR;
+  const int Lv = p.nblk * 32;
+  auto swz = [](int r) { return (r >> 1) & 7; };
+  const unsigned a_bytes = (unsigned)((long)p.M * p.lda * EB), w_bytes = (unsigned)((long)n_tiles * BN * p.K * EB);
+  unsigned voffA[4];
+#pragma unroll
+  for (int i = 0; i < APC; ++i) {
+    const int r = (i * NW + wave) * RPI + lane / CPR;
+    const int c = (lane % CPR) ^ swz(r);
+    const long row = (long)m0 + r;
+    const int seq = (int)(row / Lv), t = (int)(row - (long)seq * Lv);
+    voffA[i] = (seq < p.n_seq && t < p.L) ? (unsigned)(((long)seq * p.L + t) * p.lda * EB + c * 16) : OOB;
+  }
+  unsigned voffW;
+  {
+    const int r = wave * RPI + lane / CPR;
+    voffW = (unsigned)((long)(n0 + r) * p.K * EB + ((lane % CPR) ^ swz(r)) * 16);
+  }
+  const rsrc_t rA = __builtin_amdgcn_make_buffer_rsrc(const_cast<char*>(reinterpret_cast<const char*>(p.A)), 0, a_bytes, 0x00020000);
+  const rsrc_t rW = __builtin_amdgcn_make_buffer_rsrc(const_cast<void*>(p.W), 0, w_bytes, 0x00020000);
+  auto issue = [&](int kt, int stage) {
+    char* st_ = smem + stage * ST_BYTES + wave * 1024;
+    const int so_ = kt * ROWB;
+#pragma unroll
+    for (int i_ = 0; i_ < APC; ++i_)
+      __builtin_amdgcn_raw_ptr_buffer_load_lds(rA, (lptr_t)(st_ + i_ * NW * 1024), 16, voffA[i_], so_, 0, 0);
+    __builtin_amdgcn_raw_ptr_buffer_load_lds(rW, (lptr_t)(st_ + A_BYTES), 16, voffW, so_, 0, 0);
+  };
+  const int pofs = A_BYTES + lr * ROWB;
+  const int qofs = (wave * 32 + lr) * ROWB;
+  const int sw = swz(lr);
+  int kc[4];
+#pragma unroll
+  for (int m = 0; m < 4; ++m) kc[m] = ((2 * m + g) ^ sw) * 16;
+  f32x16 acc;
+#pragma unroll
+  for (int r = 0; r < 16; ++r) acc[r] = 0.f;
+  const int vb = m0 + wave * 32;
+  const int tseq = vb / Lv, tblk = (vb - tseq * Lv) >> 5;
+  const int t = tblk * 32 + lr;
+  const long trow = (tseq < p.n_seq && t < p.L) ? (long)tseq * p.L + t : -1;
+  float part[8];
+#pragma unroll
+  for (int q = 0; q < 8; ++q) part[q] = (p.ssq_in && trow >= 0 && q < p.ssq_parts) ? p.ssq_in[(long)q * p.M + trow] : 0.f;
+#pragma unroll
+  for (int s0 = 0; s0 < NST - 1; ++s0)
+    if (s0 < nk) issue(s0, s0);
+  asm volatile("s_waitcnt vmcnt(0)" ::: "memory");
+  __builtin_amdgcn_sched_barrier(0);
+  float rs = 1.f;
+  if (p.ssq_in) {
+    float sum = 0.f;
+#pragma unroll
+    for (int q = 0; q < 8; ++q) sum += part[q];
+    for (int q = 8; q < p.ssq_parts; ++q) sum += trow >= 0 ? p.ssq_in[(long)q * p.M + trow] : 0.f;
+    rs = trow >= 0 ? sqrtf((float)p.K) / fmaxf(sqrtf(sum), 1e-12f) : 0.f;
+  }
+  int stage = 0, stage2 = NST - 1;
+  for (int kt = 0; kt < nk; ++kt) {
+    if (NST > 2 && kt + 1 < nk) asm volatile("s_waitcnt vmcnt(%0) lgkmcnt(0)" ::"n"((NST - 2) * LPS) : "memory");
+    else asm volatile("s_waitcnt vmcnt(0) lgkmcnt(0)" ::: "memory");
+    __builtin_amdgcn_s_barrier();
+    if (kt + NST - 1 < nk) issue(kt + NST - 1, stage2);
+    const char* st = smem + stage * ST_BYTES;
+#pragma unroll
+    for (int m = 0; m < 2; ++m) {
+      const hfx8 ph = *reinterpret_cast<const hfx8*>(st + pofs + kc[m]);
+      const hfx8 pl = *reinterpret_cast<const hfx8*>(st + pofs + kc[m + 2]);
+      const hfx8 qh = *reinterpret_cast<const hfx8*>(st + qofs + kc[m]);
+      const hfx8 ql = *reinterpret_cast<const hfx8*>(st + qofs + kc[m + 2]);
+      acc = MFMA32_H(pl, qh, acc);
+      acc = MFMA32_H(ph, ql, acc);
+      acc = MFMA32_H(ph, qh, acc);
+    }
+    stage = stage == NST - 1 ? 0 : stage + 1;
+    stage2 = stage2 == NST - 1 ? 0 : stage2 + 1;
+  }
+  if (tseq >= p.n_seq) return;
+#pragma unroll
+  for (int r = 0; r < 16; ++r) {
+    const int h = n0 - 3 * p.inner + crow(r, g);
+    if (h < p.heads) p.gates[((long)tseq * p.heads + h) * p.nbp * 32 + t] = sigmoidf(fmaf(acc[r], rs, p.b_gates[h]));
+  }
 }
 
 template <int EPI, typename CFG, int X3 = 0, int ABL = 0>
@@ -145,6 +242,12 @@
   int kind = 0;
   if constexpr (EPI == G3_QKV) kind = n0 < 3 * p.inner ? n0 / p.inner : 3;
   const bool normal = EPI == G3_QKV && kind == 2;
+  if constexpr (BT_QKV_GATE_TILE && EPI == G3_QKV && X3 == 1 && ABL == 0 && BM == 128 && BN == 128 && ROWB == 128 && NW == 4) {
+    if (kind == 3 && p.heads <= 32 && (p.x3 & 15) != 3) {
+      qkv_gate_tile_x3<CFG>(p, smem, m0, n0, n_tiles, lane, wave);
+      return;
+    }
+  }
 
   const unsigned a_bytes = (unsigned)((long)p.M * p.lda * EB), w_bytes = (unsigned)((long)n_tiles * BN * p.K * EB);
   static_assert(APC >= 1 && WPC >= 1, "tile too small for the workgroup");
@@ -528,10 +631,12 @@
             if (xb) *reinterpret_cast<u32x2*>(xb + off) = u32x2{pk2(v[0], v[1]), pk2(v[2], v[3])};
           }
         }
-        float ssq = ok ? fmaf(v[0], v[0], fmaf(v[1], v[1], fmaf(v[2], v[2], v[3] * v[3]))) : 0.f;
-#pragma unroll
-        for (int o = 8; o > 0; o >>= 1) ssq += __shfl_xor(ssq, o);
-        if (p.ssq_out && ok && cp == 0) p.ssq_out[(unsigned)(n0 / 64 + wn) * (unsigned)p.M + (unsigned)(row0 + 32 * b + r)] = ssq;
+        if (p.ssq_out) {
+          float ssq = ok ? fmaf(v[0], v[0], fmaf(v[1], v[1], fmaf(v[2], v[2], v[3] * v[3]))) : 0.f;
+#pragma unroll
+          for (int o = 8; o > 0; o >>= 1) ssq += __shfl_xor(ssq, o);
+          if (ok && cp == 0) p.ssq_out[(unsigned)(n0 / 64 + wn) * (unsigned)p.M + (unsigned)(row0 + 32 * b + r)] = ssq;
+        }
       }
     }
     }
diff --git a/beat_this_amd/csrc/kernels.h b/beat_this_amd/csrc/kernels.h
--- a/beat_this_amd/csrc/kernels.h
+++ b/beat_this_amd/csrc/kernels.h
@@ -133,6 +133,7 @@
   const float* b1; const float* b2;
   void* xb;
   int abl;
+  int shadow_only;
 };
 int launch_outff_fused(const FusedOutFFP& p, int prec, hipStream_t s);
 struct FusedAttnFFP {
```

Result: faster. 64300 (median of 6 runs) (+1.5%).
